# Fannovel16/stylish-tts

Hardware: AMD Instinct MI355X
Metric: utterances_per_sec (higher is better)
Workload: dtype f32

## Files before the change

### include/stylish_hip.h

```cpp
#ifndef STYLISH_HIP_H_
#define STYLISH_HIP_H_

#include <stddef.h>
#include <stdint.h>

#ifdef __cplusplus
extern "C" {
#endif

typedef struct stts_ctx stts_ctx;

typedef struct stts_model_dims {
  int32_t n_fft, win_length, hop_length, sample_rate;
  int32_t style_dim, inter_dim;
  int32_t dec_hidden, dec_residual;
  int32_t gen_input, gen_hidden, gen_inter, gen_io_kernel;
  int32_t tokens, te_hidden, te_filter, te_heads, te_layers, te_kernel;
  int32_t style_layers;
  int32_t dur_layers, dur_classes, dur_max;
  int32_t pe_inter;
} stts_model_dims;

const char* stts_last_error(void);
int stts_version(void);
// ... 113 lines not shown
int stts_rmvpe_finalize(stts_ctx* ctx, const stts_rmvpe_dims* dims);
size_t stts_rmvpe_workspace_bytes(const stts_ctx* ctx, int n_utt, const int32_t* off_host);
int stts_rmvpe_forward(stts_ctx* ctx, void* stream, int n_utt, const int32_t* off_host, const int32_t* off_dev, const float* mel_rows, int ld_mel, float thred,
                       float* hidden_out, float* f0_out, void* ws, size_t ws_bytes);
int stts_rmvpe_forward_taps(stts_ctx* ctx, void* stream, int n_utt, const int32_t* off_host, const int32_t* off_dev, const float* mel_rows, int ld_mel,
                            float thred, float* hidden_out, float* f0_out, float* taps, void* ws, size_t ws_bytes);
int64_t stts_rmvpe_tap_floats(const stts_rmvpe_dims* dims, int n_utt, const int32_t* off_host);
int stts_rmvpe_mel(stts_ctx* ctx, void* stream, int n_utt, const int32_t* sample_off_host, const int32_t* sample_off_dev, const int32_t* mel_off_host,
                   const int32_t* mel_off_dev, const float* wave, const float* mel_basis, const int32_t* band, float* mel_out, int ld_mel, float* mel_lin);
int stts_rmvpe_decode(stts_ctx* ctx, void* stream, int64_t n_rows, const float* salience, int ld, float thred, float* f0_out);
int stts_rmvpe_resample(stts_ctx* ctx, void* stream, int n_utt, const int32_t* off_in_dev, const int32_t* off_out_host, const int32_t* off_out_dev,
                        const float* f0_in, float* f0_out);

typedef struct stts_aligner_dims {
  int32_t n_mels, hidden, classes;
  int32_t n_tdnn, ffn_layers;
  int32_t tdnn_kernel[4];
} stts_aligner_dims;
int stts_aligner_finalize(stts_ctx* ctx, const stts_aligner_dims* dims);
size_t stts_aligner_workspace_bytes(const stts_ctx* ctx, int n_utt, const int32_t* off_host);
int stts_aligner_forward(stts_ctx* ctx, void* stream, int n_utt, const int32_t* off_host, const int32_t* off_dev, const float* mel_rows, int ld_mel,
                         float* log_probs, int ld_out, void* ws, size_t ws_bytes);
int stts_aligner_forward_taps(stts_ctx* ctx, void* stream, int n_utt, const int32_t* off_host, const int32_t* off_dev, const float* mel_rows, int ld_mel,
                              float* log_probs, int ld_out, float* taps, void* ws, size_t ws_bytes);
int64_t stts_aligner_tap_floats(const stts_aligner_dims* dims, int n_utt, const int32_t* off_host);
size_t stts_ctc_align_workspace_bytes(int n_utt, const int32_t* t_off_host, const int32_t* p_off_host);
int stts_ctc_align(void* stream, int n_utt, const int32_t* t_off_host, const int32_t* t_off_dev, const int32_t* p_off_host, const int32_t* p_off_dev,
                   const float* log_probs, int ld, int classes, int blank, const int32_t* targets, int path_given, int32_t* path, float* scores,
                   int32_t* durations, float* left, float* right, void* ws, size_t ws_bytes);

size_t stts_hubert_workspace_bytes(const stts_ctx* ctx, int64_t rows_T, int n_utt, int max_len);
int stts_speaker_style(stts_ctx* ctx, void* stream, int n_utt, const float* spk_emb, int ld, float* style_out, float* pe_style_out, void* ws,
                       size_t ws_bytes);
int stts_hubert_encoder_forward(stts_ctx* ctx, void* stream, int n_utt, const int32_t* off_T_host, const int32_t* off_T_dev, const float* feats,
                                int ld_feats, float* asr_out, int ld_asr, void* ws, size_t ws_bytes);
int stts_hubert_pitch_energy_forward(stts_ctx* ctx, void* stream, int n_utt, const int32_t* off_T_host, const int32_t* off_T_dev, const float* feats,
                                     int ld_feats, const float* pe_style, float* f0_out, float* energy_out, float* prosody_tap, void* ws,
                                     size_t ws_bytes);

size_t stts_mel_style_workspace_bytes(stts_ctx* ctx, int which, int64_t rows_T, int n_utt);
int stts_mel_style_forward(stts_ctx* ctx, void* stream, int which, int n_utt, const int32_t* seg_off_host, const int32_t* seg_off_dev, const float* mel,
                           int ld, float* style_out, void* ws, size_t ws_bytes);
int stts_mel_style_forward_taps(stts_ctx* ctx, void* stream, int which, int n_utt, const int32_t* seg_off_host, const int32_t* seg_off_dev,
                                const float* mel, int ld, float* style_out, float* block_taps, void* ws, size_t ws_bytes);

size_t stts_cfm_pitch_workspace_bytes(stts_ctx* ctx, int64_t rows_T, int n_utt);
int stts_cfm_pitch_forward(stts_ctx* ctx, void* stream, int n_utt, const int32_t* off_T_host, const int32_t* off_T_dev, const float* asr, int ld_asr,
                           const float* spk_style, float* out_normed, float* out_hz, float f0_log2_mean, float f0_log2_std, const float* uv, void* ws,
                           size_t ws_bytes);
int stts_cfm_pitch_forward_taps(stts_ctx* ctx, void* stream, int n_utt, const int32_t* off_T_host, const int32_t* off_T_dev, const float* asr, int ld_asr,
                                const float* spk_style, float* out_normed, float* out_hz, float f0_log2_mean, float f0_log2_std, const float* uv,
                                float* taps, void* ws, size_t ws_bytes);

int stts_log_mel_forward(stts_ctx* ctx, void* stream, int n_utt, const int32_t* sample_off_host, const int32_t* sample_off_dev,
                         const int32_t* row_off_host, const int32_t* row_off_dev, const float* wave, int n_fft, int win_length, int hop_length, int n_mels,
                         int sample_rate, double mean, double std, float* mel_rows, int ld, float* energy, float* raw_rows);
int stts_log_mel_stats(stts_ctx* ctx, void* stream, int n_utt, const int32_t* sample_off_host, const int32_t* sample_off_dev,
                       const int32_t* row_off_host, const int32_t* row_off_dev, const float* wave, int n_fft, int win_length, int hop_length, int n_mels,
                       int sample_rate, double* partials, double* stats);
int stts_log_mel_filters(int n_fft, int n_mels, int sample_rate, int32_t* band, float* weights);

int stts_to_time_major(void* stream, const float* x_bct, int B, int C, int T, float* y, int ldy);
int stts_to_channel_major(void* stream, const float* x, int ldx, int B, int C, int T, float* y_bct);

int stts_conv_stft_transform(stts_ctx* ctx, void* stream, int n_utt, const int32_t* frame_off_host, const int32_t* frame_off_dev,
                             const float* wave, int hop, float* mag, float* x, float* y, int ld);
int stts_conv_stft_inverse(stts_ctx* ctx, void* stream, int n_utt, const int32_t* frame_off_host, const int32_t* frame_off_dev,
                           const float* mag, const float* x, const float* y, int ld, int hop, float* wave_out, void* ws, size_t ws_bytes);

int stts_profile_begin(void);
int stts_profile_end(void* stream, int* launches, double* total_ms, double* total_flops);
int stts_profile_report(void* stream, char* json, size_t json_capacity);

int stts_op_mrf_block(stts_ctx* ctx, void* stream, const char* prefix, int n_utt, const int32_t* seg_off_host,
                      const int32_t* seg_off_dev, const float* x, int ldx, int channels, int kernel, const float* style, float* y,
                      int ldy, void* ws, size_t ws_bytes);

#ifdef STTS_TEST_OPS
int stts_op_conv1d(void* stream, int n_utt, const int32_t* seg_off_host, const int32_t* seg_off_dev, const float* x, int ldx, int cin,
                   const float* w_host, const float* bias_host, int cout, int k, int dil, int act, float* y, int ldy, int force_tile, int precision);
int stts_op_conv1d_x3(void* stream, int n_utt, const int32_t* seg_off_host, const int32_t* seg_off_dev, const float* x, int ldx, int cin,
                      const float* x2, int ldx2, int cin2, const float* w_host, const float* bias_host, int cout, int k, int dil, const float* aff_host,
                      int xaff_mode, float slope, int presplit, float* y, int ldy, int force_tile, int precision);
int stts_op_adain_block(stts_ctx* ctx, void* stream, const char* prefix, int n_utt, const int32_t* seg_off_host,
                        const int32_t* seg_off_dev, const float* x, int ldx, int cin, int cout, const float* style, float* y, int ldy,
                        void* ws, size_t ws_bytes);
int stts_op_attention(void* stream, int n_utt, const int32_t* q_off_host, const int32_t* q_off_dev, const int32_t* k_off_host,
                      const int32_t* k_off_dev, const float* q, const float* k, const float* v, float* o, int heads, int kc,
                      const int32_t* band_centre, int window, int kernel);
int stts_op_stft_geom(void* stream, int n_utt, const int32_t* seg_off_host, const int32_t* seg_off_dev, int n_fft, int win, int h, const float* sig,
                      float* spec, float* phase, int ld, int generic);
int stts_op_istft_geom(void* stream, int n_utt, const int32_t* seg_off_host, const int32_t* seg_off_dev, int n_fft, int win, int h, const float* logamp,
                       const float* phase, int ld, float* audio, int generic);
int stts_bench_gemm(void* stream, int n_utt, int rows_per_utt, int cin, int cout, int k, int tile, int iters, double* avg_ms, int tune);
#endif

#ifdef __cplusplus
}
#endif
#endif
```

### stylish_tts_amd/_lib.py

```python
from __future__ import annotations

import ctypes as C
import os

_HERE = os.path.dirname(os.path.abspath(__file__))
LIB_PATH = os.path.abspath(os.environ["STTS_LIB"]) if os.environ.get("STTS_LIB") else os.path.join(_HERE, "libstylish_hip.so")


class ModelDims(C.Structure):
    _fields_ = [(n, C.c_int32) for n in (
        "n_fft", "win_length", "hop_length", "sample_rate",
        "style_dim", "inter_dim",
        "dec_hidden", "dec_residual",
        "gen_input", "gen_hidden", "gen_inter", "gen_io_kernel",
        "tokens", "te_hidden", "te_filter", "te_heads", "te_layers", "te_kernel",
        "style_layers",
        "dur_layers", "dur_classes", "dur_max",
        "pe_inter",
    )]


class CfmDims(C.Structure):
    _fields_ = [(n, C.c_int32) for n in ("feat_dim", "asr_dim", "spk_dim", "hidden_dim", "emb_dim", "depth", "enc_blocks", "dec_blocks",
                                         "prev_depth", "post_depth", "head_dim")]
# ... 15 lines not shown

_P = C.c_void_p
_I = C.c_int
_SZ = C.c_size_t
_I64 = C.c_int64

SIGNATURES = {
    "stts_last_error": (C.c_char_p, []),
    "stts_version": (_I, []),
    "stts_ctx_create": (_I, [C.POINTER(ModelDims), _I, C.POINTER(_P)]),
    "stts_ctx_destroy": (None, [_P]),
    "stts_load_weight": (_I, [_P, C.c_char_p, _P, C.POINTER(_I64), _I]),
    "stts_finalize_weights": (_I, [_P, _I]),
    "stts_check_status": (_I, [_P, _P]),
    "stts_frame_workspace_bytes": (_SZ, [_P, _I64, _I, _I]),
    "stts_har_ld": (_I, [_P]),
    "stts_decoder_forward": (_I, [_P, _P, _I, _P, _P, _P, _I, _P, _P, _P, _P, _I, _P, _SZ]),
    "stts_prior_flow_forward": (_I, [_P, _P, _I, _P, _P, _P, _I, _P, _P, _P, _I, _P, _P, _P, _SZ]),
    "stts_harmonic_stft": (_I, [_P, _P, _I, _P, _P, _P, _P, _P, _I, _P, _P, _P, _I, _P, _SZ]),
    "stts_vocoder_forward": (_I, [_P, _P, _I, _P, _P, _P, _I, _P, _P, _P, _I, _P, _P, _P, _I, _P, _SZ]),
    "stts_frame_path": (_I, [_P, _P, _I, _P, _P, _P, _I, _P, _P, _P, _P, _P, _P, _I, _P, _P, _SZ, _I]),
    "stts_frame_offsets": (_I, [_P, _P, _I, _P, _P, _P, _P, _P, _P]),
    "stts_phoneme_workspace_bytes": (_SZ, [_P, _I64, _I64, _I]),
    "stts_text_encoder_forward": (_I, [_P, _P, _I, _I, _P, _P, _P, _P, _I, _P, _P, _SZ]),
    "stts_text_style_forward": (_I, [_P, _P, _I, _I, _P, _P, _P, _I, _P, _P, _SZ]),
    "stts_duration_forward": (_I, [_P, _P, _I, _P, _P, _P, _P, _P, _P, _P, _P, _P, _SZ]),
    "stts_pitch_energy_forward": (_I, [_P, _P, _I, _P, _P, _P, _P, _P, _P, _I, _P, _P, _P, _P, _P, _P, _SZ, _I]),
    "stts_duration_decode": (_I, [_P, _P, _I, _I, _P]),
    "stts_duration_to_alignment": (_I, [_P, _P, _I, _I, _P]),
    "stts_length_regulate": (_I, [_P, _P, _I, _P, _P, _P, _I64, _I, _P, _I, _I, _P, _I, _P]),
    "stts_set_precision": (_I, [_P, _I]),
    "stts_upsample4": (_I, [_P, _P, _I, _P, _P, _P, _P, _P]),
    "stts_euler_step": (_I, [_P, _P, _P, C.c_float, C.c_int64]),
    "stts_hubert_workspace_bytes": (_SZ, [_P, C.c_int64, _I, _I]),
    "stts_speaker_style": (_I, [_P, _P, _I, _P, _I, _P, _P, _P, _SZ]),
    "stts_hubert_encoder_forward": (_I, [_P, _P, _I, _P, _P, _P, _I, _P, _I, _P, _SZ]),
    "stts_hubert_pitch_energy_forward": (_I, [_P, _P, _I, _P, _P, _P, _I, _P, _P, _P, _P, _P, _SZ]),
    "stts_mel_style_workspace_bytes": (_SZ, [_P, _I, _I64, _I]),
    "stts_mel_style_forward": (_I, [_P, _P, _I, _I, _P, _P, _P, _I, _P, _P, _SZ]),
    "stts_mel_style_forward_taps": (_I, [_P, _P, _I, _I, _P, _P, _P, _I, _P, _P, _P, _SZ]),
    "stts_cfm_pitch_workspace_bytes": (_SZ, [_P, _I64, _I]),
    "stts_cfm_pitch_forward": (_I, [_P, _P, _I, _P, _P, _P, _I, _P, _P, _P, C.c_float, C.c_float, _P, _P, _SZ]),
    "stts_cfm_pitch_forward_taps": (_I, [_P, _P, _I, _P, _P, _P, _I, _P, _P, _P, C.c_float, C.c_float, _P, _P, _P, _SZ]),
    "stts_ssl_finalize": (_I, [_P, _P]),
    "stts_ssl_frames": (_I64, [_P, _I64]),
    "stts_ssl_workspace_bytes": (_SZ, [_P, _I, _P]),
    "stts_ssl_forward": (_I, [_P, _P, _I, _P, _P, _P, _P, _P, _P, _I, _P, _SZ]),
    "stts_ssl_forward_taps": (_I, [_P, _P, _I, _P, _P, _P, _P, _P, _P, _I, _P, _P, _P, _P, _P, _P, _P, _P, _SZ]),
    "stts_ssl_tap_rows": (_I64, [_P, _I, _P]),
    "stts_rmvpe_finalize": (_I, [_P, _P]),
    "stts_rmvpe_workspace_bytes": (_SZ, [_P, _I, _P]),
    "stts_rmvpe_forward": (_I, [_P, _P, _I, _P, _P, _P, _I, C.c_float, _P, _P, _P, _SZ]),
    "stts_rmvpe_forward_taps": (_I, [_P, _P, _I, _P, _P, _P, _I, C.c_float, _P, _P, _P, _P, _SZ]),
    "stts_rmvpe_tap_floats": (_I64, [_P, _I, _P]),
    "stts_rmvpe_mel": (_I, [_P, _P, _I, _P, _P, _P, _P, _P, _P, _P, _P, _I, _P]),
    "stts_rmvpe_decode": (_I, [_P, _P, _I64, _P, _I, C.c_float, _P]),
    "stts_rmvpe_resample": (_I, [_P, _P, _I, _P, _P, _P, _P, _P]),
    "stts_aligner_finalize": (_I, [_P, _P]),
    "stts_aligner_workspace_bytes": (_SZ, [_P, _I, _P]),
    "stts_aligner_forward": (_I, [_P, _P, _I, _P, _P, _P, _I, _P, _I, _P, _SZ]),
    "stts_aligner_forward_taps": (_I, [_P, _P, _I, _P, _P, _P, _I, _P, _I, _P, _P, _SZ]),
    "stts_aligner_tap_floats": (_I64, [_P, _I, _P]),
    "stts_ctc_align_workspace_bytes": (_SZ, [_I, _P, _P]),
    "stts_ctc_align": (_I, [_P, _I, _P, _P, _P, _P, _P, _I, _I, _I, _P, _I, _P, _P, _P, _P, _P, _P, _SZ]),
    "stts_log_mel_forward": (_I, [_P, _P, _I, _P, _P, _P, _P, _P, _I, _I, _I, _I, _I, C.c_double, C.c_double, _P, _I, _P, _P]),
    "stts_log_mel_stats": (_I, [_P, _P, _I, _P, _P, _P, _P, _P, _I, _I, _I, _I, _I, _P, _P]),
    "stts_log_mel_filters": (_I, [_I, _I, _I, _P, _P]),
    "stts_cfm_finalize": (_I, [_P, _P]),
    "stts_cfm_workspace_bytes": (_SZ, [_P, _I64, _I]),
    "stts_cfm_estimator": (_I, [_P, _P, _I, _P, _P, _P, _I, _P, _I, _P, _P, _P, _P, _P, _P, _P, _P, _I, _P, _SZ]),
    "stts_to_time_major": (_I, [_P, _P, _I, _I, _I, _P, _I]),
    "stts_to_channel_major": (_I, [_P, _P, _I, _I, _I, _I, _P]),
    "stts_conv_stft_transform": (_I, [_P, _P, _I, _P, _P, _P, _I, _P, _P, _P, _I]),
    "stts_conv_stft_inverse": (_I, [_P, _P, _I, _P, _P, _P, _P, _P, _I, _I, _P, _P, _SZ]),
    "stts_profile_begin": (_I, []),
    "stts_profile_end": (_I, [_P, C.POINTER(_I), C.POINTER(C.c_double), C.POINTER(C.c_double)]),
    "stts_profile_report": (_I, [_P, C.c_char_p, _SZ]),
    "stts_op_mrf_block": (_I, [_P, _P, C.c_char_p, _I, _P, _P, _P, _I, _I, _I, _P, _P, _I, _P, _SZ]),
}
TEST_SIGNATURES = {
    "stts_bench_gemm": (_I, [_P, _I, _I, _I, _I, _I, _I, _I, C.POINTER(C.c_double), _I]),
    "stts_op_conv1d": (_I, [_P, _I, _P, _P, _P, _I, _I, _P, _P, _I, _I, _I, _I, _P, _I, _I, _I]),
    "stts_op_conv1d_x3": (_I, [_P, _I, _P, _P, _P, _I, _I, _P, _I, _I, _P, _P, _I, _I, _I, _P, _I, C.c_float, _I, _P, _I, _I, _I]),
    "stts_op_adain_block": (_I, [_P, _P, C.c_char_p, _I, _P, _P, _P, _I, _I, _I, _P, _P, _I, _P, _SZ]),
    "stts_op_attention": (_I, [_P, _I, _P, _P, _P, _P, _P, _P, _P, _P, _I, _I, _P, _I, _I]),
    "stts_op_stft_geom": (_I, [_P, _I, _P, _P, _I, _I, _I, _P, _P, _P, _I, _I]),
    "stts_op_istft_geom": (_I, [_P, _I, _P, _P, _I, _I, _I, _P, _P, _I, _P, _I]),
}

_lib = None


def load() -> C.CDLL:
    global _lib
    if _lib is not None:
        return _lib
    if not os.path.exists(LIB_PATH):
        raise RuntimeError(
            f"{LIB_PATH} not found: build it with `python -c 'import __graft_entry__ as g; g.build()'` "
            "(hipcc --offload-arch=gfx950).  There is no CPU fallback."
        )
    try:
        import torch
    except ImportError:
        pass
    lib = C.CDLL(LIB_PATH)
    for name, (res, args) in SIGNATURES.items():
        fn = getattr(lib, name)
        fn.restype = res
        fn.argtypes = args
    for name, (res, args) in TEST_SIGNATURES.items():
        fn = getattr(lib, name, None)
        if fn is not None:
            fn.restype = res
            fn.argtypes = args
    _lib = lib
    return lib


def check(rc: int) -> None:
    if rc != 0:
        raise RuntimeError("stylish_hip: " + (load().stts_last_error() or b"?").decode("utf-8", "replace"))
```

### stylish_tts_amd/csrc/api.hip

```cpp
#include "model.hip.h"
#include "cfm.hip.h"
#include "hubert.hip.h"
#include "conv2d.hip.h"
#include "mel_style.hip.h"
#include "cfm_pitch.hip.h"
#include "ssl.hip.h"
#include "rmvpe.hip.h"
#include "aligner.hip.h"
#include "log_mel.hip.h"

using namespace stts;

#define API_BEGIN try {
#define API_END                                                         \
  }                                                                     \
  catch (const std::exception& e) { return stts::fail("exception: %s", e.what()); } \
  catch (...) { return stts::fail("unknown exception"); }

extern "C" {

const char* stts_last_error(void) { return stts::last_error().c_str(); }
int stts_version(void) { return 1; }

int stts_ctx_create(const stts_model_dims* dims, int device, stts_ctx** out) {
  API_BEGIN
  STTS_CHECK(dims && out, "null argument");
  int n = 0;
  STTS_HIP(hipGetDeviceCount(&n));
  STTS_CHECK(device >= 0 && device < n, "device %d not available (%d visible)", device, n);
  STTS_HIP(hipSetDevice(device));
  hipDeviceProp_t prop;
  STTS_HIP(hipGetDeviceProperties(&prop, device));
  STTS_CHECK(strncmp(prop.gcnArchName, "gfx950", 6) == 0, "device %d is %s; this library is built for gfx950 only", device, prop.gcnArchName);
  stts_ctx* c = new stts_ctx();
  c->d = *dims;
  c->device = device;
  c->force_generic_signal = getenv("STTS_SIGNAL_GENERIC") && atoi(getenv("STTS_SIGNAL_GENERIC")) != 0;
  PackScope scope(c, engine_mode(c));
  STTS_TRY(dev_upload(c, std::vector<int>(64, 0), &c->d_err));
  *out = c;
  return 0;
  API_END
}

void stts_ctx_destroy(stts_ctx* c) {
  if (!c) return;
  for (void* p : c->allocs) (void)hipFree(p);
  for (auto& kv : c->side_lanes) {
    if (kv.second.fork) (void)hipEventDestroy(kv.second.fork);
    if (kv.second.join) (void)hipEventDestroy(kv.second.join);
    if (kv.second.stream) (void)hipStreamDestroy(kv.second.stream);
    if (kv.second.fork2) (void)hipEventDestroy(kv.second.fork2);
    if (kv.second.join2) (void)hipEventDestroy(kv.second.join2);
    if (kv.second.stream2) (void)hipStreamDestroy(kv.second.stream2);
  }
  delete c;
}

int stts_set_precision(stts_ctx* c, int precision) {
  API_BEGIN
  STTS_CHECK(c, "bad argument");
  STTS_CHECK(precision >= 0 && precision <= 3, "precision must be STTS_PREC_F32, _BF16, _F16 or _F32_NATIVE");
  const int prec = precision == STTS_PREC_F32_NATIVE ? (int)PREC_F32 : precision;
  STTS_CHECK(c->ready == 0 || (prec == c->prec && (precision != STTS_PREC_F32_NATIVE) == c->allow_x3), "precision must be chosen before weights are finalized");
  c->prec = prec;
  c->allow_x3 = precision != STTS_PREC_F32_NATIVE;
  return 0;
  API_END
}

int stts_load_weight(stts_ctx* c, const char* name, const float* data, const int64_t* shape, int ndim) {
  API_BEGIN
  STTS_CHECK(c && name && data && shape && ndim >= 1 && ndim <= 4, "bad argument");
  HostTensor t;
  int64_t n = 1;
  for (int i = 0; i < ndim; ++i) {
    t.shape.push_back(shape[i]);
    n *= shape[i];
  }
  t.data.assign(data, data + n);
  c->host[name] = std::move(t);
  return 0;
  API_END
}

int stts_finalize_weights(stts_ctx* c, int which) {
  API_BEGIN
  STTS_CHECK(c, "null ctx");
  STTS_HIP(hipSetDevice(c->device));
  c->ready &= ~which;
  free_component_allocs(c, which);
  if (which & (STTS_W_DECODER | STTS_W_FLOW | STTS_W_GENERATOR)) {
    PackScope scope(c, {c->prec, true, c->prec != PREC_F32 ? 64 : 32, 0});
    STTS_TRY(finalize_frame(c, which));
  }
  const int ph = which & (STTS_W_SPEECH_TEXT | STTS_W_DURATION | STTS_W_PE_TEXT | STTS_W_PE_STYLE | STTS_W_PITCH_ENERGY);
  if (ph) {
    if (!c->phoneme) c->phoneme = std::make_shared<PhonemeModel>();
    static const bool phoneme_x3 = getenv("STTS_PHONEME_X3") && atoi(getenv("STTS_PHONEME_X3")) != 0;
    PackScope scope(c, {PREC_F32, phoneme_x3, 32, 0});
    STTS_TRY(finalize_phoneme(c, static_cast<PhonemeModel*>(c->phoneme.get()), ph));
    c->ready |= ph;
  }
  const int hb = which & (STTS_W_HUBERT | STTS_W_HUBERT_PE);
  if (hb) {
    if (!c->hubert) c->hubert = std::make_shared<HubertModel>();
    PackScope scope(c, {PREC_F32, false, 32, 0});
    STTS_TRY(finalize_hubert(c, static_cast<HubertModel*>(c->hubert.get()), hb));
    c->ready |= hb;
  }
  const int ms = which & (STTS_W_PE_MEL_STYLE | STTS_W_CFM_PITCH);
  if (ms) {
    if (!c->mel_style) c->mel_style = std::make_shared<MelStyleModel>();
    PackScope scope(c, engine_mode(c));
    STTS_TRY(finalize_mel_style(c, static_cast<MelStyleModel*>(c->mel_style.get()), ms));
    c->ready |= ms;
  }
  if (which & STTS_W_CFM_PITCH_NET) {
    if (!c->cfm_pitch) c->cfm_pitch = std::make_shared<CfmPitchNetW>();
    PackScope scope(c, {PREC_F32, false, 32, STTS_W_CFM_PITCH_NET});
    STTS_TRY(finalize_cfm_pitch_net(c, static_cast<CfmPitchNetW*>(c->cfm_pitch.get())));
    c->ready |= STTS_W_CFM_PITCH_NET;
  }
  STTS_HIP(hipDeviceSynchronize());
  return 0;
  API_END
}

int stts_check_status(stts_ctx* c, void* stream) {
  API_BEGIN
  int e = 0;
  STTS_HIP(hipStreamSynchronize((hipStream_t)stream));
  STTS_HIP(hipMemcpy(&e, c->d_err, sizeof(int), hipMemcpyDeviceToHost));
  if (e) {
    STTS_HIP(hipMemset(c->d_err, 0, sizeof(int)));
    std::string msg;
    if (e & 2) msg += "text encoder: token id outside [0, tokens); ";
    if (e & 4) msg += "harmonic source: an utterance is too short for the STFT's reflect padding (needs more than " + std::to_string(c->d.n_fft / 2) + " samples); ";
    if (e & 1) msg += "harmonic source: a frame is voiced (f0 > 10 Hz) but no f0 exceeds 20 Hz (reference raises: models/generator.py:285); ";
    if (e & ~7) msg += "unknown device error bits " + std::to_string(e & ~7) + "; ";
    msg.resize(msg.size() - 2);
    return stts::fail("%s", msg.c_str());
  }
  return 0;
  API_END
}

int stts_har_ld(const stts_ctx* c) {
  if (!c) return 0;
  if (c->amp_prior.kc) return har_ld(c);
  return round_up(c->d.n_fft / 2 + 1, c->prec != PREC_F32 ? 64 : 32);
}

size_t stts_frame_workspace_bytes(const stts_ctx* c, int64_t rows, int n_utt, int max_len) { return frame_workspace_bytes(c, rows, n_utt, max_len); }

static int seg_ok(int n_utt, const int32_t* h, const int32_t* d, const char* bad = "bad utterance offsets", const char* empty = "utterance %d is empty") {
  STTS_CHECK(n_utt > 0 && h && d && h[0] == 0, "%s", bad);
  for (int u = 0; u < n_utt; ++u) STTS_CHECK(h[u + 1] > h[u], empty, u, h[u + 1] - h[u]);
  return 0;
}

#define READY_CHECK(have, mask)                                                      \
  STTS_CHECK(c && (have) && (c->ready & (mask)) == (mask), "weights for this stage are not finalized (need components 0x%x, have 0x%x)", (mask), c ? c->ready : 0); \
  STTS_HIP(hipSetDevice(c->device));                                                 \
  hipStream_t st = (hipStream_t)stream

#define SEG_CHECK(mask)                                                              \
  READY_CHECK(true, mask);                                                           \
  STTS_TRY(seg_ok(n_utt, seg_off_host, seg_off_dev));                                \
  Seg s{n_utt, seg_off_host, seg_off_dev}

int stts_decoder_forward(stts_ctx* c, void* stream, int n_utt, const int32_t* seg_off_host, const int32_t* seg_off_dev, const float* asr,
                         int ld_asr, const float* pitch, const float* energy, const float* style, float* x_out, int ld_x, void* ws,
                         size_t ws_bytes) {
  API_BEGIN
  SEG_CHECK(STTS_W_DECODER);
  STTS_CHECK(ld_asr >= c->d.inter_dim && ld_asr % 4 == 0 && ld_x >= c->d.dec_hidden, "bad leading dimension");
// ... 912 lines not shown
```

### stylish_tts_amd/csrc/gemm.hip.h

```cpp
#pragma once
#include <type_traits>
#include <mutex>
#include <map>
#include <hip/hip_ext.h>
#include <cmath>
#include <algorithm>
#include <vector>

#include "common.h"

namespace stts {

using f32x16 = __attribute__((ext_vector_type(16))) float;
using f32x4 = __attribute__((ext_vector_type(4))) float;

enum Act { ACT_NONE = 0, ACT_SILU = 1, ACT_GELU = 2, ACT_RELU = 3, ACT_LRELU = 4 };
enum Epi {
  EPI_STORE = 0,
  EPI_GATE = 1,
  EPI_SPLIT_ACC = 2,
  EPI_COUPLE = 3,
  EPI_PRIOR = 4,
};

struct GemmSeg {
  const float* X;
  const float* W;
  const unsigned short* W16;
  long w16_plane;
  long x_plane;
  long w_utt_stride;
  int ldx, xcol0, kc, ntaps, dil, pad;
  int kreal;
};

struct SplitInfo {
  const float* partial;
  int ksplit, slice_rows, ld_part;
};

struct GemmArgs {
  GemmSeg seg[3];
  int nseg;
  const int* seg_off;
  const int* seg_host;
  int n_utt;
  int compact;
  int uniform_len, uniform_lo0;
  int tile0, tiles_y;
  int gemm16_gx;
  int capacity;
  int rows_total, wrows;
  int tune;
  int prec;
  const float* xaff;
  int ld_xaff;
  float xaff_slope;
  bool xaff_scale_only;
  long long* dbg;
  const float* zeros;
  int ksplit;
  float* partial;
  int ld_part;
  SplitInfo* defer;
  int N;
  const float* bias;
  int x16;
  float* Y;
  int ldy, ycol0;
  unsigned short* Y16;
  int ldy16, ycol16;
  const float* R;
  int ldr, rcol0;
  float alpha;
  int act;
  float* sumsq_part;
  int ld_ss, ss_stride;
  float* stat_part;
  int ld_stat, stat_nchunk;
  const float* gate;
  int ld_gate, gcol0, gC;
  float* D0;
  float* D1;
  int ldd0, ldd1, nsplit, acc0, acc1;
  float* Z;
  int ldz, zcol0;
  const float* noise;
  int ldnoise;
};

__device__ __forceinline__ float act_apply(float v, int act) {
  switch (act) {
    case ACT_SILU: return v * __builtin_amdgcn_rcpf(1.0f + __expf(-v));
    case ACT_GELU: return 0.5f * v * (1.0f + erff(v * 0.70710678118654752f));
    case ACT_RELU: return fmaxf(v, 0.0f);
    case ACT_LRELU: return v >= 0.0f ? v : 0.2f * v;
    default: return v;
  }
}

enum { PREC_F32 = 0, PREC_BF16 = 1, PREC_F16 = 2, PREC_X3 = 3 };
typedef __bf16 bf16x8 __attribute__((ext_vector_type(8)));
typedef _Float16 f16x8 __attribute__((ext_vector_type(8)));
typedef unsigned u32x2 __attribute__((ext_vector_type(2)));

template <int PREC>
__device__ __forceinline__ u32x2 pack4_16(const f32x4 v) {
  u32x2 r;
  if constexpr (PREC == PREC_BF16) {
    typedef __bf16 b2 __attribute__((ext_vector_type(2)));
    typedef float f2 __attribute__((ext_vector_type(2)));
    const f2 lo = {v.x, v.y}, hi = {v.z, v.w};
    r.x = __builtin_bit_cast(unsigned, __builtin_convertvector(lo, b2));
    r.y = __builtin_bit_cast(unsigned, __builtin_convertvector(hi, b2));
  } else {
    typedef _Float16 h2 __attribute__((ext_vector_type(2)));
    typedef float f2 __attribute__((ext_vector_type(2)));
    const f2 lo = {v.x, v.y}, hi = {v.z, v.w};
    r.x = __builtin_bit_cast(unsigned, __builtin_convertvector(lo, h2));
    r.y = __builtin_bit_cast(unsigned, __builtin_convertvector(hi, h2));
  }
  return r;
}
__device__ __forceinline__ void split3_bf16(const f32x4 v, u32x2& p0, u32x2& p1, u32x2& p2) {
  typedef __bf16 b2 __attribute__((ext_vector_type(2)));
  typedef float f2 __attribute__((ext_vector_type(2)));
  auto pk = [](float a, float b) { const f2 t = {a, b}; return __builtin_bit_cast(unsigned, __builtin_convertvector(t, b2)); };
  auto lo = [](unsigned u) { return __uint_as_float(u << 16); };
  auto hi = [](unsigned u) { return __uint_as_float(u & 0xffff0000u); };
  const float tmax = __uint_as_float(0x7f7f7fffu);
  bool inf[4];
  float f[4];
#pragma unroll
  for (int e = 0; e < 4; ++e) {
    inf[e] = __builtin_isinf(v[e]);
    f[e] = __builtin_amdgcn_fmed3f(inf[e] ? 0.0f : v[e], -tmax, tmax);
  }
  p0.x = pk(f[0], f[1]); p0.y = pk(f[2], f[3]);
  const float r0 = v.x - lo(p0.x), r1 = v.y - hi(p0.x), r2 = v.z - lo(p0.y), r3 = v.w - hi(p0.y);
  p1.x = pk(inf[0] ? 0.0f : r0, inf[1] ? 0.0f : r1); p1.y = pk(inf[2] ? 0.0f : r2, inf[3] ? 0.0f : r3);
  p2.x = pk(r0 - lo(p1.x), r1 - hi(p1.x)); p2.y = pk(r2 - lo(p1.y), r3 - hi(p1.y));
}
template <int PREC>
__device__ __forceinline__ f32x16 mfma16(const f32x4 a, const f32x4 b, const f32x16 c) {
  if constexpr (PREC == PREC_BF16 || PREC == PREC_X3) return __builtin_amdgcn_mfma_f32_32x32x16_bf16(__builtin_bit_cast(bf16x8, a), __builtin_bit_cast(bf16x8, b), c, 0, 0, 0);
  else return __builtin_amdgcn_mfma_f32_32x32x16_f16(__builtin_bit_cast(f16x8, a), __builtin_bit_cast(f16x8, b), c, 0, 0, 0);
}

template <int BM, int BN, int WARPS_M, int WARPS_N, int EPI, int KSPLIT = 1, bool GLDS = false, int PREC = PREC_F32, int XAFF = 0, bool MSEG = true,
          bool X16 = false>
__global__ void __launch_bounds__(WARPS_M* WARPS_N * 64 * KSPLIT) conv_gemm_f32(const GemmArgs a) {
  static_assert(!(XAFF && GLDS), "the input affine lives on the register staging path");
  static_assert(!X16 || (PREC != PREC_F32 && !XAFF && EPI == EPI_STORE), "16-bit activation rows: 16-bit operand modes, store epilogue");
  constexpr int NT = WARPS_M * WARPS_N * 64 * KSPLIT;
  constexpr bool B16 = PREC != PREC_F32;
  constexpr bool X3 = PREC == PREC_X3;
  constexpr int NPL = X3 ? 3 : 1;
  static_assert(!X3 || !GLDS || X16, "split fp32: fp32 activation rows are split on the register staging path; LDS-DMA needs pre-split planes");
  static_assert(!(B16 && GLDS) || X16, "LDS-DMA staging of 16-bit operands needs 16-bit activation rows (nothing converts on the way)");
  static_assert(KSPLIT == 1 || KSPLIT == 2, "KSPLIT");
  constexpr int WR = BN / WARPS_N, WC = BM / WARPS_M;
  constexpr int TR = WR / 32, TC = WC / 32;
  constexpr int XL = X16 ? (BN * 4 * NPL + NT - 1) / NT : BN * 8 / NT;
  constexpr int WL = B16 ? (BM * 4 * NPL + NT - 1) / NT : BM * 8 / NT;
  static_assert(WR % 32 == 0 && WC % 32 == 0, "wave tile must be a multiple of 32x32");
  static_assert((X16 || (BN * 8) % NT == 0) && (B16 || (BM * 8) % NT == 0), "tile loads must divide over the block");
  static_assert(EPI == EPI_STORE || EPI == EPI_SPLIT_ACC || TC % 2 == 0, "paired epilogues need an even TC");
  constexpr int NSTAGE = (B16 && GLDS) ? (X3 ? 3 : ((BM + BN) <= 256 ? 8 : 3)) : 2;
  constexpr int SLOTS = X3 ? 12 : ((B16 && KSPLIT == 1) ? 4 : 8);
  constexpr int PLANE = (BN + BM) * 4;
  constexpr int STG16 = PLANE * NPL;
  __shared__ f32x4 lds[NSTAGE * (BN + BM) * SLOTS];

  int bx = blockIdx.x, by = blockIdx.y, bz = blockIdx.z;
  {
    unsigned gy = gridDim.y;
    if (a.capacity) {
      const int lane_ = threadIdx.x & 63;
      int tot = 0;
      for (int u0 = 0; u0 < a.n_utt; u0 += 64) {
        const int u = u0 + lane_;
        tot += u < a.n_utt ? (a.seg_off[u + 1] - a.seg_off[u] + BN - 1) / BN : 0;
      }
#pragma unroll
      for (int o = 32; o > 0; o >>= 1) tot += __shfl_xor(tot, o, 64);
      gy = (unsigned)__builtin_amdgcn_readfirstlane(tot);
      if ((unsigned)by >= gy) return;
    }
    const unsigned gx = gridDim.x, nwg = gx * gy * gridDim.z;
    const unsigned orig = bx + gx * (by + gy * bz);
    const unsigned q = nwg >> 3, r = nwg & 7, xcd = orig & 7;
    const unsigned id = (xcd < r ? xcd * (q + 1) : r * (q + 1) + (xcd - r) * q) + (orig >> 3);
    bx = id % gx;
    by = (id / gx) % gy;
    bz = id / (gx * gy);
  }
  const int ksplit = a.ksplit > 1 ? a.ksplit : 1;
  int utt, ks;
  if (a.compact) {
    ks = bz;
    const int t = by + a.tile0, lane_ = threadIdx.x & 63;
    utt = a.n_utt - 1;
    int base = 0, local = 0;
    bool done = false;
    if (a.uniform_len > 0) {
      const int tpu = (a.uniform_len + BN - 1) / BN;
      utt = t / tpu;
      local = t - utt * tpu;
      done = utt < a.n_utt;
    }
    for (int u0 = 0; u0 < a.n_utt && !done && a.uniform_len <= 0; u0 += 64) {
      const int u = u0 + lane_;
      const int tiles = u < a.n_utt ? (a.seg_off[u + 1] - a.seg_off[u] + BN - 1) / BN : 0;
      int incl = tiles;
#pragma unroll
      for (int d = 1; d < 64; d <<= 1) {
        const int v = __shfl_up(incl, d, 64);
        if (lane_ >= d) incl += v;
      }
      const int excl = incl - tiles;
      const unsigned long long hit = __ballot(t >= base + excl && t < base + incl);
      if (hit) {
        const int src = __ffsll((long long)hit) - 1;
        utt = u0 + src;
        local = t - base - __shfl(excl, src, 64);
        done = true;
      }
      base += __shfl(incl, 63, 64);
    }
    if (!done) return;
    utt = __builtin_amdgcn_readfirstlane(utt);
    by = __builtin_amdgcn_readfirstlane(local);
  } else {
    utt = bz / ksplit;
    ks = bz % ksplit;
  }
  const int lo = a.uniform_len > 0 ? a.uniform_lo0 + utt * a.uniform_len : a.seg_off[utt];
  const int hi = a.uniform_len > 0 ? lo + a.uniform_len : a.seg_off[utt + 1];
  const int row0 = lo + by * BN;
  if (row0 >= hi) return;
  const int m0 = bx * BM;
  const int tid = threadIdx.x, lane = tid & 63;
#ifdef STTS_GEMM_TRACE
  const unsigned dbg_blk = blockIdx.x + gridDim.x * (blockIdx.y + gridDim.y * blockIdx.z);
  auto stamp = [&](int i) { if (a.dbg && tid == 0) a.dbg[8 * (long)dbg_blk + i] = wall_clock64(); };
  const long long dbg_c0 = clock64();
  if (a.dbg && tid == 0) { a.dbg[8 * (long)dbg_blk + 5] = __builtin_amdgcn_s_getreg(0xF804); a.dbg[8 * (long)dbg_blk + 6] = __builtin_amdgcn_s_getreg(0xF814); }
  auto stamp_end = [&]() { stamp(3); if (a.dbg && tid == 0) a.dbg[8 * (long)dbg_blk + 7] = clock64() - dbg_c0; };
  auto ablate = [&](int bit) { return (a.tune & bit) != 0; };
#else
  auto stamp = [&](int) {};
  auto stamp_end = [&]() {};
  auto ablate = [](int) { return false; };
#endif
  stamp(0);
  const int kg = (tid >> 6) / (WARPS_M * WARPS_N), wid = (tid >> 6) % (WARPS_M * WARPS_N);
  const int wn = wid / WARPS_M, wm = wid % WARPS_M;
  (void)kg;

  f32x16 acc[TR][TC];
#pragma unroll
  for (int i = 0; i < TR; ++i)
#pragma unroll
    for (int j = 0; j < TC; ++j)
#pragma unroll
      for (int r = 0; r < 16; ++r) acc[i][j][r] = 0.0f;

  int s = 0, tap = 0, chunk = 0;
  auto xbase = [&](const GemmSeg& g) {
    return X16 ? reinterpret_cast<const float*>(reinterpret_cast<const unsigned short*>(g.X) + g.xcol0) : g.X + g.xcol0;
  };
  const float* gX = xbase(a.seg[0]);
  const float* gW = a.seg[0].W + (long)utt * a.seg[0].w_utt_stride + (long)m0 * a.seg[0].ntaps * a.seg[0].kc;
  const unsigned short* gW16 = B16 ? a.seg[0].W16 + (long)utt * a.seg[0].w_utt_stride + (long)m0 * a.seg[0].ntaps * a.seg[0].kc : nullptr;
  int g_ldx = a.seg[0].ldx, g_kc = a.seg[0].kc, g_ntaps = a.seg[0].ntaps, g_dil = a.seg[0].dil, g_pad = a.seg[0].pad;
  const int nseg = a.nseg;

  struct RegSet {
    f32x4 x[XL], w[WL];
    bool ok[XL];
    f32x4 sc, sh;
    bool aff;
  };
  RegSet rsA, rsB;
#ifdef STTS_X3_DEEP
  constexpr bool DEEP = X3 && KSPLIT == 1 && BN <= 128;
#else
  constexpr bool DEEP = false;
#endif
  RegSet rsC, rsD;
  unsigned woff[WL];
  const int len = hi - lo, rel0 = row0 - lo;
  long g_wplane = X3 ? a.seg[0].w16_plane : 0, g_xplane = (X3 && X16) ? a.seg[0].x_plane : 0;
  auto seg_offsets = [&]() {
    const int wrow = g_ntaps * g_kc;
#pragma unroll
    for (int i = 0; i < WL; ++i) {
      const int idx = tid + i * NT;
      if constexpr (X3) {
        const int pl = min(idx / (BM * 4), 2), rem = idx % (BM * 4);
        woff[i] = (unsigned)(((long)pl * g_wplane + (rem >> 2) * wrow + (rem & 3) * 8) * 2);
      } else if constexpr (B16) woff[i] = (unsigned)((min(idx >> 2, BM - 1) * wrow + (idx & 3) * 8) * 2);
      else woff[i] = (unsigned)(((idx >> 3) * wrow + (idx & 7) * 4) * 4);
    }
  };
  seg_offsets();
  auto gload = [&](RegSet& rs) {
    const int shift = (tap - g_pad) * g_dil;
#ifdef STTS_GEMM_TRACE
    const bool hot = a.tune & 16;
#else
    constexpr bool hot = false;
#endif
    const char* xb = X16 ? reinterpret_cast<const char*>(reinterpret_cast<const unsigned short*>(gX) + (long)lo * g_ldx + chunk * 32)
                         : reinterpret_cast<const char*>(gX + (long)lo * g_ldx + (hot ? 0 : chunk * 32));
    const char* wb = B16 ? reinterpret_cast<const char*>(gW16 + tap * g_kc + chunk * 32)
                         : reinterpret_cast<const char*>((hot ? a.seg[0].W : gW) + (hot ? 0 : tap * g_kc + chunk * 32));
#pragma unroll
    for (int i = 0; i < XL; ++i) {
      const int idx = tid + i * NT;
      const int pl = (X16 && X3) ? min(idx / (BN * 4), 2) : 0, idp = (X16 && X3) ? idx % (BN * 4) : idx;
      const int r = X16 ? idp >> 2 : idx >> 3, sl = X16 ? idp & 3 : idx & 7;
      const int rel = (hot ? 0 : rel0) + r + shift;
      const int crel = min(max(rel, 0), len - 1);
      const unsigned rowoff = __umul24((unsigned)crel, (unsigned)g_ldx);
      const unsigned off = X16 ? (rowoff + sl * 8) * 2 : (rowoff + sl * 4) * 4;
      if constexpr (X16 && X3) rs.x[i] = *reinterpret_cast<const f32x4*>(xb + (long)pl * g_xplane * 2 + off);
      else
      rs.x[i] = *reinterpret_cast<const f32x4*>(xb + off);
      rs.ok[i] = rel >= 0 && rel < len;
    }
#pragma unroll
    for (int i = 0; i < WL; ++i) rs.w[i] = *reinterpret_cast<const f32x4*>(wb + woff[i]);
    if constexpr (XAFF) {
      rs.aff = s == 0;
      const float* ap = a.xaff + (long)utt * 2 * a.ld_xaff + (rs.aff ? chunk * 32 + (tid & 7) * 4 : 0);
      rs.sc = *reinterpret_cast<const f32x4*>(ap);
      if constexpr (XAFF == 1) rs.sh = *reinterpret_cast<const f32x4*>(ap + a.ld_xaff);
    }
    const int w1 = tap + 1 >= g_ntaps, wk = (chunk + 1) * 32 >= g_kc;
    const bool wrapt1 = w1 != 0;
    const bool wrapt = (w1 & wk) != 0;
    const bool last = ((w1 & wk) & (MSEG ? (int)(s + 1 >= nseg) : 1)) != 0;
    tap = last ? tap : (wrapt1 ? 0 : tap + 1);
    chunk = last ? chunk : (wrapt ? 0 : chunk + w1);
    if constexpr (MSEG) {
      if (wrapt && !last) {
        ++s;
        const GemmSeg& n = s == 1 ? a.seg[1] : a.seg[2];
        gX = xbase(n);
        gW = n.W + (long)utt * n.w_utt_stride + (long)m0 * n.ntaps * n.kc;
        if constexpr (B16) gW16 = n.W16 + (long)utt * n.w_utt_stride + (long)m0 * n.ntaps * n.kc;
        g_ldx = n.ldx; g_kc = n.kc; g_ntaps = n.ntaps; g_dil = n.dil; g_pad = n.pad;
        if constexpr (X3) { g_wplane = n.w16_plane; g_xplane = n.x_plane; }
        seg_offsets();
      }
    }
  };
  auto xin = [&](const RegSet& rs, int i) {
    const f32x4 z = {0.f, 0.f, 0.f, 0.f};
    f32x4 v = rs.x[i];
    if constexpr (XAFF == 2) {
      static_assert(XAFF != 2 || !MSEG, "the scale-only input affine is instantiated for single-segment launches");
      v = v * rs.sc;
    } else if constexpr (XAFF == 1) {
      f32x4 t;
#pragma unroll
      for (int q = 0; q < 4; ++q) {
        const float y = (rs.sc[q] == 0.0f ? 0.0f : v[q] * rs.sc[q]) + rs.sh[q];
        t[q] = y >= 0.0f ? y : a.xaff_slope * y;
      }
      v = rs.aff ? t : v;
    }
    return rs.ok[i] ? v : z;
// ... 87 lines not shown
    const int slot = 2 * kk + lh;
    f32x4 xa[TR], wb[TC];
#pragma unroll
    for (int i = 0; i < TR; ++i) {
      const int r = wn * WR + i * 32 + l31;
      xa[i] = Xs[r * 8 + (slot ^ ((r >> 1) & 7))];
    }
#pragma unroll
    for (int j = 0; j < TC; ++j) {
      const int c = wm * WC + j * 32 + l31;
      wb[j] = Ws[c * 8 + (slot ^ ((c >> 1) & 7))];
    }
#pragma unroll
    for (int i = 0; i < TR; ++i)
#pragma unroll
      for (int j = 0; j < TC; ++j) {
        acc[i][j] = __builtin_amdgcn_mfma_f32_32x32x2f32(xa[i].x, wb[j].x, acc[i][j], 0, 0, 0);
        acc[i][j] = __builtin_amdgcn_mfma_f32_32x32x2f32(xa[i].y, wb[j].y, acc[i][j], 0, 0, 0);
        acc[i][j] = __builtin_amdgcn_mfma_f32_32x32x2f32(xa[i].z, wb[j].z, acc[i][j], 0, 0, 0);
        acc[i][j] = __builtin_amdgcn_mfma_f32_32x32x2f32(xa[i].w, wb[j].w, acc[i][j], 0, 0, 0);
      }
  };

  auto mma_step16 = [&](int b, int kk) {
    const f32x4* Xs = lds + b * STG16;
    const f32x4* Ws = Xs + BN * 4;
    const int slot = 2 * kk + lh;
    if constexpr (X3) {
      f32x4 xa[TR][3], wb[TC][3];
      const bool nord = ablate(32);
#pragma unroll
      for (int i = 0; i < TR; ++i) {
        const int r = wn * WR + i * 32 + l31;
        const int o = r * 4 + (slot ^ ((r >> 2) & 3));
#pragma unroll
        for (int p = 0; p < 3; ++p) {
          if (!nord) xa[i][p] = Xs[o + p * PLANE];
          else xa[i][p] = f32x4{(float)r, (float)kk, (float)p, 0.f};
        }
      }
#pragma unroll
      for (int j = 0; j < TC; ++j) {
        const int c = wm * WC + j * 32 + l31;
        const int o = c * 4 + (slot ^ ((c >> 2) & 3));
#pragma unroll
        for (int p = 0; p < 3; ++p) {
          if (!nord) wb[j][p] = Ws[o + p * PLANE];
          else wb[j][p] = f32x4{(float)c, (float)kk, (float)p, 0.f};
        }
      }
      if (ablate(1)) return;
#pragma unroll
      for (int i = 0; i < TR; ++i)
#pragma unroll
        for (int j = 0; j < TC; ++j) {
          acc[i][j] = mfma16<PREC>(xa[i][2], wb[j][0], acc[i][j]);
          acc[i][j] = mfma16<PREC>(xa[i][0], wb[j][2], acc[i][j]);
          acc[i][j] = mfma16<PREC>(xa[i][1], wb[j][1], acc[i][j]);
          acc[i][j] = mfma16<PREC>(xa[i][1], wb[j][0], acc[i][j]);
          acc[i][j] = mfma16<PREC>(xa[i][0], wb[j][1], acc[i][j]);
          acc[i][j] = mfma16<PREC>(xa[i][0], wb[j][0], acc[i][j]);
        }
      return;
    }
    f32x4 xa[TR], wb[TC];
    const bool nord = ablate(32);
#pragma unroll
    for (int i = 0; i < TR; ++i) {
      const int r = wn * WR + i * 32 + l31;
      if (!nord) xa[i] = Xs[r * 4 + (slot ^ ((r >> 2) & 3))];
      else xa[i] = f32x4{(float)r, (float)kk, 0.f, 0.f};
    }
#pragma unroll
    for (int j = 0; j < TC; ++j) {
      const int c = wm * WC + j * 32 + l31;
      if (!nord) wb[j] = Ws[c * 4 + (slot ^ ((c >> 2) & 3))];
      else wb[j] = f32x4{(float)c, (float)kk, 0.f, 0.f};
    }
#pragma unroll
    for (int i = 0; i < TR; ++i)
#pragma unroll
      for (int j = 0; j < TC; ++j) acc[i][j] = mfma16<PREC>(xa[i], wb[j], acc[i][j]);
  };

  if constexpr (GLDS) {
    static_assert(KSPLIT == 1, "GLDS path is single K-group");
    if constexpr (B16) {
      constexpr int NW = NT / 64, NI1 = (BN + BM) / 16, NI = NI1 * NPL, PER = NI / NW;
      static_assert((NI % NW == 0 || X3) && BN % 16 == 0, "tile rows must divide over the waves");
      constexpr int PERC = (NI + NW - 1) / NW;
      const int wv = tid >> 6;
      auto issue = [&](int b) {
        const int shift = (tap - g_pad) * g_dil;
        const char* xb = reinterpret_cast<const char*>(reinterpret_cast<const unsigned short*>(gX) + (long)lo * g_ldx + chunk * 32);
        const char* wb = reinterpret_cast<const char*>(gW16 + tap * g_kc + chunk * 32);
        const int wrow = g_ntaps * g_kc;
#pragma unroll
        for (int q = 0; q < PERC; ++q) {
          const int instq = min(wv + q * NW, NI - 1);
          const int pl = instq / NI1, inst = instq % NI1;
          const int trow = inst * 16 + (lane >> 2);
          const char* src;
          if (inst < BN / 16) {
            const int r = trow;
            const int sslot = (lane & 3) ^ ((r >> 2) & 3);
            const int rel = rel0 + r + shift;
            const bool ok = rel >= 0 && rel < len;
            src = ok ? xb + (long)pl * g_xplane * 2 + (unsigned)((rel * g_ldx + sslot * 8) * 2) : reinterpret_cast<const char*>(a.zeros);
          } else {
            const int n = trow - BN;
            const int sslot = (lane & 3) ^ ((n >> 2) & 3);
            src = wb + (long)pl * g_wplane * 2 + (unsigned)((n * wrow + sslot * 8) * 2);
          }
          __builtin_amdgcn_global_load_lds((const __attribute__((address_space(1))) void*)src,
                                           (__attribute__((address_space(3))) void*)(lds + b * STG16 + pl * PLANE + inst * 64), 16, 0, 0);
        }
        const int w1 = tap + 1 >= g_ntaps, wk = (chunk + 1) * 32 >= g_kc;
        const bool wrapt1 = w1 != 0;
        const bool wrapt = (w1 & wk) != 0;
        const bool last = ((w1 & wk) & (MSEG ? (int)(s + 1 >= nseg) : 1)) != 0;
        tap = last ? tap : (wrapt1 ? 0 : tap + 1);
        chunk = last ? chunk : (wrapt ? 0 : chunk + w1);
        if constexpr (MSEG) {
          if (wrapt && !last) {
            ++s;
            const GemmSeg& n = s == 1 ? a.seg[1] : a.seg[2];
            gX = xbase(n);
            gW16 = n.W16 + (long)utt * n.w_utt_stride + (long)m0 * n.ntaps * n.kc;
            g_ldx = n.ldx; g_kc = n.kc; g_ntaps = n.ntaps; g_dil = n.dil; g_pad = n.pad;
            if constexpr (X3) { g_wplane = n.w16_plane; g_xplane = n.x_plane; }
          }
        }
      };
      (void)PER;
      constexpr int INFLIGHT = (NSTAGE - 2) * PERC;
      static_assert(INFLIGHT >= 1 && INFLIGHT <= 63, "vmcnt immediate");
      auto wait_next_tile = [&]() {
        asm volatile("" ::: "memory");
        __builtin_amdgcn_s_waitcnt((INFLIGHT & 15) | (7 << 4) | (15 << 8) | ((INFLIGHT >> 4) << 14));
        asm volatile("" ::: "memory");
      };
#pragma unroll
      for (int q = 0; q < NSTAGE - 1; ++q) issue(q);
      wait_next_tile();
      __syncthreads();
      stamp(1);
      int cur = 0, nxt = NSTAGE - 1;
      for (int it = 0; it < total; ++it) {
        if (!ablate(8)) issue(nxt);
        mma_step16(cur, 0);
        mma_step16(cur, 1);
        wait_next_tile();
        if (!ablate(2)) __syncthreads();
        cur = cur == NSTAGE - 1 ? 0 : cur + 1;
        nxt = nxt == NSTAGE - 1 ? 0 : nxt + 1;
      }
      asm volatile("s_waitcnt vmcnt(0)" ::: "memory");
      __syncthreads();
      stamp(2);
    } else {
        static_assert(KSPLIT == 1, "GLDS path is single K-group");
      constexpr int NW = NT / 64, NI = (BN + BM) / 8;
      static_assert(NI % NW == 0, "tile rows must divide over the waves");
      const int wv = tid >> 6;
      auto issue = [&](int b) {
        const int shift = (tap - g_pad) * g_dil;
        const char* xb = reinterpret_cast<const char*>(gX + (long)lo * g_ldx + chunk * 32);
        const char* wb = reinterpret_cast<const char*>(gW + tap * g_kc + chunk * 32);
        const int wrow = g_ntaps * g_kc;
  #pragma unroll
        for (int q = 0; q < NI / NW; ++q) {
          const int inst = wv + q * NW;
          const int trow = inst * 8 + (lane >> 3);
          const char* src;
          if (inst < BN / 8) {
            const int r = trow;
            const int sslot = (lane & 7) ^ ((r >> 1) & 7);
            const int rel = rel0 + r + shift;
            const bool ok = rel >= 0 && rel < len;
            src = ok ? xb + (unsigned)((rel * g_ldx + sslot * 4) * 4) : reinterpret_cast<const char*>(a.zeros);
          } else {
            const int n = trow - BN;
            const int sslot = (lane & 7) ^ ((n >> 1) & 7);
            src = wb + (unsigned)((n * wrow + sslot * 4) * 4);
          }
          __builtin_amdgcn_global_load_lds((const __attribute__((address_space(1))) void*)src,
                                           (__attribute__((address_space(3))) void*)(lds + b * (BN + BM) * 8 + inst * 64), 16, 0, 0);
        }
        const int w1 = tap + 1 >= g_ntaps, wk = (chunk + 1) * 32 >= g_kc;
        const bool wrapt1 = w1 != 0;
        const bool wrapt = (w1 & wk) != 0;
        const bool last = ((w1 & wk) & (int)(s + 1 >= nseg)) != 0;
        tap = last ? tap : (wrapt1 ? 0 : tap + 1);
        chunk = last ? chunk : (wrapt ? 0 : chunk + w1);
        if (wrapt && !last) {
          ++s;
          const GemmSeg& n = s == 1 ? a.seg[1] : a.seg[2];
          gX = xbase(n);
          gW = n.W + (long)utt * n.w_utt_stride + (long)m0 * n.ntaps * n.kc;
          if constexpr (B16) gW16 = n.W16 + (long)utt * n.w_utt_stride + (long)m0 * n.ntaps * n.kc;
          g_ldx = n.ldx; g_kc = n.kc; g_ntaps = n.ntaps; g_dil = n.dil; g_pad = n.pad;
        }
      };
      issue(0);
      asm volatile("s_waitcnt vmcnt(0)" ::: "memory");
      __syncthreads();
      for (int it = 0; it < total; ++it) {
        issue((it + 1) & 1);
        const f32x4* Xs = lds + (it & 1) * (BN + BM) * 8;
        const f32x4* Ws = Xs + BN * 8;
        mma_step(Xs, Ws, 0);
        mma_step(Xs, Ws, 1);
        mma_step(Xs, Ws, 2);
        mma_step(Xs, Ws, 3);
        asm volatile("s_waitcnt vmcnt(0)" ::: "memory");
        __syncthreads();
      }
    }
  } else {
  gload(rsA);
  lstore(rsA, 0);
  gload(rsB);
  if constexpr (DEEP) {
    gload(rsC);
    gload(rsD);
  }
  gload(rsA);
  __syncthreads();
  stamp(1);

  int return_guard = 0;
  (void)return_guard;
  constexpr bool FPIPE = X3 && KSPLIT == 1 && BN == 128 && BM == 128 && WARPS_M * WARPS_N == 8 && !GLDS;
  struct Frag {
    f32x4 xa[TR][3], wb[TC][3];
  };
  Frag fA, fB;
  auto frag_read = [&](int b, int kk, Frag& f) {
    const f32x4* Xs = lds + b * STG16;
    const f32x4* Ws = Xs + BN * 4;
    const int slot = 2 * kk + lh;
    const bool nord = ablate(32);
#pragma unroll
    for (int i = 0; i < TR; ++i) {
      const int r = wn * WR + i * 32 + l31;
      const int o = r * 4 + (slot ^ ((r >> 2) & 3));
#pragma unroll
      for (int p = 0; p < 3; ++p) {
        if (!nord) f.xa[i][p] = Xs[o + p * PLANE];
        else f.xa[i][p] = f32x4{(float)r, (float)kk, (float)p, 0.f};
      }
    }
#pragma unroll
    for (int j = 0; j < TC; ++j) {
      const int c = wm * WC + j * 32 + l31;
      const int o = c * 4 + (slot ^ ((c >> 2) & 3));
#pragma unroll
      for (int p = 0; p < 3; ++p) {
        if (!nord) f.wb[j][p] = Ws[o + p * PLANE];
        else f.wb[j][p] = f32x4{(float)c, (float)kk, (float)p, 0.f};
      }
    }
  };
  auto frag_mma = [&](const Frag& f) {
    if (ablate(1)) return;
#pragma unroll
    for (int i = 0; i < TR; ++i)
#pragma unroll
      for (int j = 0; j < TC; ++j) {
        acc[i][j] = mfma16<PREC>(f.xa[i][2], f.wb[j][0], acc[i][j]);
        acc[i][j] = mfma16<PREC>(f.xa[i][0], f.wb[j][2], acc[i][j]);
        acc[i][j] = mfma16<PREC>(f.xa[i][1], f.wb[j][1], acc[i][j]);
        acc[i][j] = mfma16<PREC>(f.xa[i][1], f.wb[j][0], acc[i][j]);
        acc[i][j] = mfma16<PREC>(f.xa[i][0], f.wb[j][1], acc[i][j]);
        acc[i][j] = mfma16<PREC>(f.xa[i][0], f.wb[j][0], acc[i][j]);
      }
  };
  if constexpr (FPIPE) frag_read(0, 0, fA);
  auto iter = [&](int it, RegSet& nset) {
    const f32x4* Xs = lds + (it & 1) * (BN + BM) * 8;
    const f32x4* Ws = Xs + BN * 8;
    if constexpr (FPIPE) {
      frag_read(it & 1, 1, fB);
      frag_mma(fA);
      if (!ablate(4)) lstore(nset, (it + 1) & 1);
      if (!ablate(8)) gload(nset);
#ifndef STTS_X3_NO_SGB
#pragma unroll
      for (int g = 0; g < 6 * TR * TC; ++g) {
        __builtin_amdgcn_sched_group_barrier(0x008, 1, 0);
        __builtin_amdgcn_sched_group_barrier(0x002, 7, 0);
      }
#endif
      if (!ablate(2)) __syncthreads();
      frag_read((it + 1) & 1, 0, fA);
      frag_mma(fB);
      return;
    }
    if constexpr (B16) {
      if constexpr (KSPLIT == 1) {
        mma_step16(it & 1, 0);
// ... 29 lines not shown
      mma_step(Xs, Ws, 2 * kg + 1);
    }
    if (!ablate(2)) __syncthreads();
  };
  if constexpr (DEEP) {
    int it = 0;
    for (; it + 3 < total; it += 4) {
      iter(it, rsB);
      iter(it + 1, rsC);
      iter(it + 2, rsD);
      iter(it + 3, rsA);
    }
    if (it < total) iter(it, rsB);
    if (it + 1 < total) iter(it + 1, rsC);
    if (it + 2 < total) iter(it + 2, rsD);
  } else {
    int it = 0;
    for (; it + 1 < total; it += 2) {
      iter(it, rsB);
      iter(it + 1, rsA);
    }
    if (it < total) iter(it, rsB);
  }
  stamp(2);
#ifdef STTS_GEMM_TRACE
  if (a.dbg && tid == 0) a.dbg[8 * (long)dbg_blk + 4] = total;
#endif
  }

  if constexpr (KSPLIT == 2) {
    static_assert(WARPS_M * WARPS_N * TR * TC * 16 * 64 * 4 <= NSTAGE * (BN + BM) * SLOTS * 16, "reduction buffer must fit in the staging LDS");
    float* red = reinterpret_cast<float*>(lds);
    if (kg == 1) {
#pragma unroll
      for (int i = 0; i < TR; ++i)
#pragma unroll
        for (int j = 0; j < TC; ++j)
#pragma unroll
          for (int r = 0; r < 16; ++r) red[(((wid * TR + i) * TC + j) * 16 + r) * 64 + lane] = acc[i][j][r];
    }
    __syncthreads();
    if (kg == 1) return;
#pragma unroll
    for (int i = 0; i < TR; ++i)
#pragma unroll
      for (int j = 0; j < TC; ++j)
#pragma unroll
        for (int r = 0; r < 16; ++r) acc[i][j][r] += red[(((wid * TR + i) * TC + j) * 16 + r) * 64 + lane];
  }
  const int nvalid = hi - row0;
  if constexpr (EPI == EPI_STORE) {
    if (ksplit > 1) {
      float* P = a.partial + (long)ks * a.rows_total * a.ld_part;
#pragma unroll
      for (int j = 0; j < TC; ++j) {
        const int n = m0 + wm * WC + j * 32 + l31;
#pragma unroll
        for (int i = 0; i < TR; ++i)
#pragma unroll
          for (int r = 0; r < 16; ++r) {
            const int rl = wn * WR + i * 32 + (r & 3) + 8 * (r >> 2) + 4 * lh;
            if (rl < nvalid) P[(long)(row0 + rl) * a.ld_part + n] = acc[i][j][r];
          }
      }
      stamp_end();
      return;
    }
    const bool hasR = a.R != nullptr, hasY = a.Y != nullptr, hasSS = a.sumsq_part != nullptr;
    bool hasY16 = false;
    if constexpr (B16) hasY16 = a.Y16 != nullptr;
    const int act = a.act;
    const float alpha = a.alpha;
    float* const Yb = hasY ? a.Y + (long)row0 * a.ldy + a.ycol0 + m0 : nullptr;
    const float* const Rb = hasR ? a.R + (long)row0 * a.ldr + a.rcol0 + m0 : nullptr;
    unsigned short* const Y16b = hasY16 ? a.Y16 + (long)row0 * a.ldy16 + a.ycol16 + m0 : nullptr;
    const int rlane = wn * WR + 4 * lh, clane = wm * WC + l31;
    unsigned oy = (unsigned)(rlane * a.ldy + clane), orr = (unsigned)(rlane * a.ldr + clane), o16 = (unsigned)(rlane * a.ldy16 + clane);
    const unsigned sy1 = (unsigned)a.ldy, sy5 = 5u * sy1, sr1 = (unsigned)a.ldr, sr5 = 5u * sr1, s161 = (unsigned)a.ldy16, s165 = 5u * s161;
    float bv[TC];
    bool nok[TC];
#pragma unroll
    for (int j = 0; j < TC; ++j) {
      const int n = m0 + clane + j * 32;
      bv[j] = a.bias ? a.bias[n] : 0.0f;
      nok[j] = n < a.N;
    }
#pragma unroll
    for (int i = 0; i < TR; ++i) {
      float ss[TC];
#pragma unroll
      for (int j = 0; j < TC; ++j) ss[j] = 0.0f;
#pragma unroll
      for (int r = 0; r < 16; ++r) {
        const int dr = i * 32 + (r & 3) + 8 * (r >> 2);
        const bool rok = rlane + dr < nvalid;
#pragma unroll
        for (int j = 0; j < TC; ++j) {
          float v = act_apply(acc[i][j][r] + bv[j], act);
          if (rok && nok[j]) {
            if (hasR) v += Rb[orr + j * 32];
            v *= alpha;
            if (hasY) Yb[oy + j * 32] = v;
            if constexpr (B16) {
              if (hasY16) {
                if constexpr (PREC == PREC_BF16) reinterpret_cast<__bf16*>(Y16b)[o16 + j * 32] = (__bf16)v;
                else reinterpret_cast<_Float16*>(Y16b)[o16 + j * 32] = (_Float16)v;
              }
            }
            ss[j] += v * v;
          }
        }
        const bool big = (r & 3) == 3;
        oy += big ? sy5 : sy1;
        orr += big ? sr5 : sr1;
        o16 += big ? s165 : s161;
      }
      if (hasSS) {
#pragma unroll
        for (int j = 0; j < TC; ++j) {
          float t2 = ss[j] + __shfl_xor(ss[j], 32, 64);
          const int sub = by * (BN / 32) + (wn * TR + i);
          if (lh == 0 && nok[j] && sub * 32 < hi - lo) {
            const long t = (long)utt * a.ss_stride + sub;
            a.sumsq_part[t * a.ld_ss + m0 + clane + j * 32] = t2;
          }
        }
      }
      __builtin_amdgcn_sched_barrier(0);
    }
  } else if constexpr (EPI == EPI_SPLIT_ACC) {
#pragma unroll
    for (int j = 0; j < TC; ++j) {
      const int n = m0 + wm * WC + j * 32 + l31;
      const float bv = a.bias ? a.bias[n] : 0.0f;
      if (n < a.N) {
        float* D;
        int ld, col, accum;
        if (n < a.nsplit) {
          D = a.D0; ld = a.ldd0; col = n; accum = a.acc0;
        } else {
          D = a.D1; ld = a.ldd1; col = n - a.nsplit; accum = a.acc1;
        }
#pragma unroll
        for (int i = 0; i < TR; ++i)
#pragma unroll
          for (int r = 0; r < 16; ++r) {
            const int rl = wn * WR + i * 32 + (r & 3) + 8 * (r >> 2) + 4 * lh;
            if (rl < nvalid) {
              float* p = D + (long)(row0 + rl) * ld + col;
              const float v = acc[i][j][r] + bv;
              *p = accum ? *p + v : v;
            }
          }
      }
    }
  } else {
#pragma unroll
    for (int jp = 0; jp < TC / 2; ++jp) {
      const int npk = m0 + wm * WC + jp * 64 + l31;
      const int c = (npk >> 6) * 32 + (npk & 31);
      const float ba = a.bias ? a.bias[npk] : 0.0f;
      const float bb = a.bias ? a.bias[npk + 32] : 0.0f;
      if (c < a.N) {
        float ga = 0.f, gb = 0.f;
        if constexpr (EPI == EPI_GATE) {
          ga = a.gate[(long)utt * a.ld_gate + a.gcol0 + c];
          gb = a.gate[(long)utt * a.ld_gate + a.gcol0 + a.gC + c];
// ... 120 lines not shown
}
inline double gemm_algorithmic_flops(const GemmArgs& a) {
  double k = 0;
  for (int i = 0; i < a.nseg; ++i) k += (double)a.seg[i].kreal * a.seg[i].ntaps;
  return 2.0 * (double)a.rows_total * (double)a.wrows * k;
}

#define STTS_LAUNCH_TIMED(kernel, grid, block, st, e0, e1, ...)                                   \
  do {                                                                                            \
    if (e0) hipExtLaunchKernelGGL(kernel, grid, block, 0, st, e0, e1, 0, __VA_ARGS__);            \
    else hipLaunchKernelGGL(kernel, grid, block, 0, st, __VA_ARGS__);                             \
  } while (0)

#define STTS_LAUNCH_PROF(name, bytes, kernel, grid, block, st, ...)                                \
  do {                                                                                            \
    stts::GemmProfiler& _p = stts::gemm_profiler();                                               \
    if (_p.on) {                                                                                  \
      hipEvent_t _e0 = _p.next(), _e1 = _p.next();                                                \
      _p.add(name, 1, 0.0, 0.0, (double)(bytes));                                                 \
      hipExtLaunchKernelGGL(kernel, grid, block, 0, st, _e0, _e1, 0, __VA_ARGS__);                \
    } else {                                                                                      \
      hipLaunchKernelGGL(kernel, grid, block, 0, st, __VA_ARGS__);                                \
    }                                                                                             \
  } while (0)

template <int ABL>
inline int launch_conv_gemm16(hipStream_t st, const GemmArgs& a, int npad, int n_utt);

void gemm_dispatch_f32(hipStream_t st, const GemmArgs& as, int tile, int epi, int npad, int n_utt, int max_rows, hipEvent_t e0, hipEvent_t e1);
void gemm_dispatch_bf16(hipStream_t st, const GemmArgs& as, int tile, int epi, int npad, int n_utt, int max_rows, hipEvent_t e0, hipEvent_t e1);
void gemm_dispatch_f16(hipStream_t st, const GemmArgs& as, int tile, int epi, int npad, int n_utt, int max_rows, hipEvent_t e0, hipEvent_t e1);
void gemm_dispatch_x3(hipStream_t st, const GemmArgs& as, int tile, int epi, int npad, int n_utt, int max_rows, hipEvent_t e0, hipEvent_t e1);
int launch_conv_gemm16_main(hipStream_t st, const GemmArgs& a, int npad, int n_utt);

}

#include "gemm_plan.hip.h"

namespace stts {

#ifndef STTS_GEMM_NO_LAUNCHER
template <int BM, int BN, int WM, int WN, int KS = 1, bool GL = false, int PR = PREC_F32>
inline void launch_cfg(hipStream_t st, const GemmArgs& a, int epi, int npad, int n_utt, int max_rows, hipEvent_t e0 = nullptr, hipEvent_t e1 = nullptr) {
  dim3 grid(npad / BM, ceil_div(max_rows, BN), n_utt * (a.ksplit > 1 ? a.ksplit : 1)), block(WM * WN * 64 * KS);
  if (a.compact) grid = dim3(npad / BM, a.tiles_y, a.ksplit > 1 ? a.ksplit : 1);
  if constexpr (GL && PR != PREC_F32) {
    if (a.nseg == 1) STTS_LAUNCH_TIMED((conv_gemm_f32<BM, BN, WM, WN, EPI_STORE, KS, true, PR, false, false, true>), grid, block, st, e0, e1, a);
    else STTS_LAUNCH_TIMED((conv_gemm_f32<BM, BN, WM, WN, EPI_STORE, KS, true, PR, false, true, true>), grid, block, st, e0, e1, a);
    return;
  } else
  switch (epi) {
    case EPI_STORE:
      if constexpr (!GL && PR != PREC_F32 && KS == 1) {
        if (a.x16) {
          if (a.nseg == 1) STTS_LAUNCH_TIMED((conv_gemm_f32<BM, BN, WM, WN, EPI_STORE, KS, GL, PR, false, false, true>), grid, block, st, e0, e1, a);
          else STTS_LAUNCH_TIMED((conv_gemm_f32<BM, BN, WM, WN, EPI_STORE, KS, GL, PR, false, true, true>), grid, block, st, e0, e1, a);
          break;
        }
      }
      if constexpr (!GL) {
        if (a.xaff) {
          if (a.nseg == 1) STTS_LAUNCH_TIMED((conv_gemm_f32<BM, BN, WM, WN, EPI_STORE, KS, GL, PR, 1, false>), grid, block, st, e0, e1, a);
          else STTS_LAUNCH_TIMED((conv_gemm_f32<BM, BN, WM, WN, EPI_STORE, KS, GL, PR, 1, true>), grid, block, st, e0, e1, a);
          break;
        }
        if (a.nseg == 1) {
          STTS_LAUNCH_TIMED((conv_gemm_f32<BM, BN, WM, WN, EPI_STORE, KS, GL, PR, false, false>), grid, block, st, e0, e1, a);
          break;
        }
      }
      STTS_LAUNCH_TIMED((conv_gemm_f32<BM, BN, WM, WN, EPI_STORE, KS, GL, PR>), grid, block, st, e0, e1, a);
      break;
    case EPI_SPLIT_ACC: STTS_LAUNCH_TIMED((conv_gemm_f32<BM, BN, WM, WN, EPI_SPLIT_ACC, KS, GL, PR>), grid, block, st, e0, e1, a); break;
    default:
      if constexpr (BM / WM >= 64) {
        if (epi == EPI_GATE) STTS_LAUNCH_TIMED((conv_gemm_f32<BM, BN, WM, WN, EPI_GATE, KS, GL, PR>), grid, block, st, e0, e1, a);
        else if (epi == EPI_COUPLE) STTS_LAUNCH_TIMED((conv_gemm_f32<BM, BN, WM, WN, EPI_COUPLE, KS, GL, PR>), grid, block, st, e0, e1, a);
        else STTS_LAUNCH_TIMED((conv_gemm_f32<BM, BN, WM, WN, EPI_PRIOR, KS, GL, PR>), grid, block, st, e0, e1, a);
      }
      break;
  }
}

template <int BM, int BN, int WM, int WN, int KS = 1, int X16MODE = 0>
inline void launch_cfg_x3(hipStream_t st, const GemmArgs& a, int epi, int npad, int n_utt, int max_rows, hipEvent_t e0 = nullptr, hipEvent_t e1 = nullptr) {
  dim3 grid(npad / BM, ceil_div(max_rows, BN), n_utt * (a.ksplit > 1 ? a.ksplit : 1)), block(WM * WN * 64 * KS);
  if (a.compact) grid = dim3(npad / BM, a.tiles_y, a.ksplit > 1 ? a.ksplit : 1);
  if constexpr (X16MODE != 0) {
    if (a.nseg == 1) STTS_LAUNCH_TIMED((conv_gemm_f32<BM, BN, WM, WN, EPI_STORE, KS, X16MODE == 2, PREC_X3, false, false, true>), grid, block, st, e0, e1, a);
    else STTS_LAUNCH_TIMED((conv_gemm_f32<BM, BN, WM, WN, EPI_STORE, KS, X16MODE == 2, PREC_X3, false, true, true>), grid, block, st, e0, e1, a);
    return;
  } else
  if (epi == EPI_PRIOR) {
    if constexpr (BM / WM >= 64) STTS_LAUNCH_TIMED((conv_gemm_f32<BM, BN, WM, WN, EPI_PRIOR, KS, false, PREC_X3>), grid, block, st, e0, e1, a);
  } else if (a.xaff) {
    if (a.nseg == 1 && a.xaff_scale_only) STTS_LAUNCH_TIMED((conv_gemm_f32<BM, BN, WM, WN, EPI_STORE, KS, false, PREC_X3, 2, false>), grid, block, st, e0, e1, a);
    else if (a.nseg == 1) STTS_LAUNCH_TIMED((conv_gemm_f32<BM, BN, WM, WN, EPI_STORE, KS, false, PREC_X3, 1, false>), grid, block, st, e0, e1, a);
    else STTS_LAUNCH_TIMED((conv_gemm_f32<BM, BN, WM, WN, EPI_STORE, KS, false, PREC_X3, 1, true>), grid, block, st, e0, e1, a);
  } else if (a.nseg == 1) {
    STTS_LAUNCH_TIMED((conv_gemm_f32<BM, BN, WM, WN, EPI_STORE, KS, false, PREC_X3, false, false>), grid, block, st, e0, e1, a);
  } else {
    STTS_LAUNCH_TIMED((conv_gemm_f32<BM, BN, WM, WN, EPI_STORE, KS, false, PREC_X3>), grid, block, st, e0, e1, a);
  }
}
template <int T, int PR>
inline void launch_tile(hipStream_t st, const GemmArgs& as, int epi, int npad, int n_utt, int max_rows, hipEvent_t e0, hipEvent_t e1) {
  constexpr TileRow r = tile_row(T);
  if constexpr ((r.forms & (PR == PREC_F32 ? FORM_F32 : FORM_16)) != 0) launch_cfg<r.BM, r.BN, r.WM, r.WN, r.KS, r.glds, PR>(st, as, epi, npad, n_utt, max_rows, e0, e1);
}
template <int T>
inline void launch_tile_x3(hipStream_t st, const GemmArgs& as, int epi, int npad, int n_utt, int max_rows, hipEvent_t e0, hipEvent_t e1) {
  constexpr TileRow r = tile_row(T);
  static_assert((r.forms & FORM_X3) != 0, "not a split-fp32 tile");
  launch_cfg_x3<r.BM, r.BN, r.WM, r.WN, r.KS, r.x16 != X16_MUST ? 0 : r.glds ? 2 : 1>(st, as, epi, npad, n_utt, max_rows, e0, e1);
}
#define STTS_TILE_CASE(T) case T: launch_tile<T, PR>(st, as, epi, npad, n_utt, max_rows, e0, e1); break;
template <int PR>
inline void gemm_dispatch_tile(hipStream_t st, const GemmArgs& as, int tile, int epi, int npad, int n_utt, int max_rows, hipEvent_t e0, hipEvent_t e1) {
  switch (tile) {
    STTS_TILE_CASE(2) STTS_TILE_CASE(4) STTS_TILE_CASE(5) STTS_TILE_CASE(6) STTS_TILE_CASE(8)
    STTS_TILE_CASE(14) STTS_TILE_CASE(15) STTS_TILE_CASE(16) STTS_TILE_CASE(17) STTS_TILE_CASE(18)
    STTS_TILE_CASE(11) STTS_TILE_CASE(13)
    default: launch_tile<3, PR>(st, as, epi, npad, n_utt, max_rows, e0, e1); break;
  }
}
#undef STTS_TILE_CASE
#define STTS_TILE_CASE(T) case T: launch_tile_x3<T>(st, as, epi, npad, n_utt, max_rows, e0, e1); break;
inline void gemm_dispatch_tile_x3(hipStream_t st, const GemmArgs& as, int tile, int epi, int npad, int n_utt, int max_rows, hipEvent_t e0, hipEvent_t e1) {
  switch (tile) {
    STTS_TILE_CASE(2) STTS_TILE_CASE(4) STTS_TILE_CASE(5) STTS_TILE_CASE(6) STTS_TILE_CASE(8)
    STTS_TILE_CASE(20) STTS_TILE_CASE(21) STTS_TILE_CASE(22)
    STTS_TILE_CASE(25) STTS_TILE_CASE(26) STTS_TILE_CASE(27) STTS_TILE_CASE(28)
    default: launch_tile_x3<3>(st, as, epi, npad, n_utt, max_rows, e0, e1); break;
  }
}
#undef STTS_TILE_CASE

inline int launch_conv_gemm(hipStream_t st, const GemmArgs& a, int epi, int npad, int n_utt, int max_rows, int force_tile = 0) {
  STTS_CHECK(npad % 128 == 0, "conv_gemm: padded cout %d not a multiple of 128", npad);
  for (int i = 0; i < a.nseg; ++i) {
    STTS_CHECK(a.seg[i].kc % 32 == 0 && a.seg[i].ldx % 4 == 0 && a.seg[i].xcol0 % 4 == 0, "conv_gemm: segment %d misaligned (kc %d ldx %d xcol0 %d)", i,
               a.seg[i].kc, a.seg[i].ldx, a.seg[i].xcol0);
  }
  if (a.x16 && a.prec != PREC_F32)
    for (int i = 0; i < a.nseg; ++i)
      STTS_CHECK(a.seg[i].ldx % 8 == 0 && a.seg[i].xcol0 % 8 == 0, "conv_gemm: 16-bit activation rows need ldx / xcol0 multiples of 8 (segment %d)", i);
  GemmPlan plan = plan_conv_gemm(a, epi, npad, n_utt, max_rows, force_tile, gemm_switches());
  STTS_CHECK(plan.ok(), "%s", plan.err);
  if (plan.route == ROUTE_GEMM16) return launch_conv_gemm16_main(st, a, npad, n_utt);
  if (a.prec != PREC_F32)
    for (int i = 0; i < a.nseg; ++i) STTS_CHECK(a.seg[i].W16 != nullptr, "conv_gemm: 16-bit operand mode without 16-bit weights (segment %d)", i);
  const int tile = plan.tile, bn = plan.bn();
  GemmArgs as = a;
  as.n_utt = n_utt;
  if (!as.zeros) as.zeros = zero_page();
  as.compact = a.seg_host != nullptr;
  float* part = nullptr;
  if (plan.main_ksp > 1 || plan.rem_rt > 0) {
    part = splitk_scratch(st, (size_t)std::max(plan.main_ksp, plan.rem_ksp) * a.rows_total * npad * sizeof(float));
    if (!part) {
      plan.main_ksp = 1;
      plan.full_rt += plan.rem_rt;
      plan.rem_rt = 0;
    }
  }
  GemmProfiler& prof = gemm_profiler();
  const double flops = gemm_algorithmic_flops(a);
  const long all_rt = plan.full_rt + plan.rem_rt;
  auto launch_range = [&](long tile0, long ntiles, int ksp) {
    as.tile0 = (int)tile0;
    as.tiles_y = (int)ntiles;
    as.ksplit = ksp;
    as.partial = ksp > 1 ? part : nullptr;
    as.ld_part = npad;
    hipEvent_t e0 = nullptr, e1 = nullptr;
    if (prof.on) {
      e0 = prof.next();
      e1 = prof.next();
      prof.add(plan.route == ROUTE_X3 ? "conv_gemm_f32_x3" : "conv_gemm_f32", 0, flops * (double)ntiles / (double)all_rt, flops * (double)ntiles / (double)all_rt, 0.0);
    }
    if (plan.route == ROUTE_X3) gemm_dispatch_x3(st, as, tile, epi, npad, n_utt, max_rows, e0, e1);
    else if (plan.route == ROUTE_BF16) gemm_dispatch_bf16(st, as, tile, epi, npad, n_utt, max_rows, e0, e1);
    else if (plan.route == ROUTE_F16) gemm_dispatch_f16(st, as, tile, epi, npad, n_utt, max_rows, e0, e1);
    else gemm_dispatch_f32(st, as, tile, epi, npad, n_utt, max_rows, e0, e1);
    if (ksp > 1 && a.defer && tile0 == 0 && ntiles == all_rt) {
      *a.defer = SplitInfo{part, ksp, a.rows_total, npad};
    } else if (ksp > 1) {
      int row_first = 0;
      if (tile0 > 0) {
        long t = tile0;
        for (int u = 0; u < n_utt; ++u) {
          const long tu = ceil_div(a.seg_host[u + 1] - a.seg_host[u], bn);
          if (t < tu) {
            row_first = a.seg_host[u] + (int)t * bn;
            break;
          }
          t -= tu;
        }
      }
      const long work = (long)(a.rows_total - row_first) * ((a.N + 3) / 4);
      STTS_LAUNCH_PROF("splitk_reduce_kernel", (size_t)work * 4 * 4 * (ksp + 1), splitk_reduce_kernel, dim3((unsigned)std::min<long>(2048, (work + 255) / 256)), dim3(256), st, part, ksp, a.rows_total,
                         row_first, npad, a.N, a.bias, a.act, a.R, a.ldr, a.rcol0, a.alpha, a.Y, a.ldy, a.ycol0);
    }
  };
  if (a.defer) *a.defer = SplitInfo{nullptr, 1, 0, 0};
  if (plan.full_rt > 0) launch_range(0, plan.full_rt, plan.main_ksp);
  if (plan.rem_rt > 0) launch_range(plan.full_rt, plan.rem_rt, plan.rem_ksp);
  STTS_HIP(hipGetLastError());
  return 0;
}
#ifdef STTS_GEMM_TU_FORM
#if STTS_GEMM_TU_FORM == 0
void gemm_dispatch_f32(hipStream_t st, const GemmArgs& as, int tile, int epi, int npad, int n_utt, int max_rows, hipEvent_t e0, hipEvent_t e1) {
  gemm_dispatch_tile<PREC_F32>(st, as, tile, epi, npad, n_utt, max_rows, e0, e1);
}
// ... 18 lines not shown
```

### stylish_tts_amd/csrc/gemm_plan.hip.h

```cpp
#pragma once
#include <climits>
#include <cstdio>

namespace stts {

enum : unsigned { FORM_F32 = 1, FORM_16 = 2, FORM_X3 = 4 };
enum TileX16 { X16_NEVER, X16_MAY, X16_MUST };
struct TileRow {
  int id, BM, BN, WM, WN, KS;
  bool glds;
  unsigned forms;
  TileX16 x16;
  bool store_only;
  bool paired;
  bool xaff;
  bool splitk;
};
constexpr unsigned kAllForms = FORM_F32 | FORM_16 | FORM_X3;
constexpr TileRow kTiles[] = {
    {2, 128, 64, 2, 2, 1, false, kAllForms, X16_MAY, false, true, true, true},
    {3, 128, 32, 2, 1, 1, false, kAllForms, X16_MAY, false, true, true, true},
    {4, 128, 32, 4, 1, 1, false, kAllForms, X16_MAY, false, false, true, true},
    {5, 128, 128, 4, 2, 1, false, kAllForms, X16_MAY, false, false, true, true},
    {6, 128, 64, 4, 2, 1, false, kAllForms, X16_MAY, false, false, true, true},
    {8, 128, 128, 4, 2, 2, false, kAllForms, X16_NEVER, false, false, true, false},
    {11, 128, 128, 4, 2, 1, true, FORM_F32, X16_NEVER, false, false, false, true},
    {13, 128, 64, 4, 2, 1, true, FORM_F32, X16_NEVER, false, false, false, true},
    {14, 256, 256, 4, 2, 1, false, FORM_16, X16_MAY, true, false, true, true},
    {15, 128, 256, 4, 2, 1, false, FORM_16, X16_MAY, true, false, true, true},
    {16, 256, 256, 4, 2, 1, true, FORM_16, X16_MUST, true, false, false, true},
    {17, 128, 256, 4, 2, 1, true, FORM_16, X16_MUST, true, false, false, true},
    {18, 128, 128, 4, 2, 1, true, FORM_16, X16_MUST, true, false, false, true},
    {20, 128, 128, 2, 2, 1, false, FORM_X3, X16_MAY, false, true, true, true},
    {21, 128, 128, 2, 2, 2, false, FORM_X3, X16_MAY, false, true, true, false},
    {22, 128, 256, 2, 4, 1, false, FORM_X3, X16_MAY, false, true, true, true},
    {25, 128, 128, 4, 2, 1, false, FORM_X3, X16_MUST, true, false, false, false},
    {26, 128, 64, 4, 2, 1, false, FORM_X3, X16_MUST, true, false, false, false},
    {27, 128, 128, 4, 2, 1, true, FORM_X3, X16_MUST, true, false, false, false},
    {28, 128, 64, 4, 2, 1, true, FORM_X3, X16_MUST, true, false, false, false},
};
constexpr const TileRow* find_tile(int id) {
  for (const TileRow& r : kTiles)
    if (r.id == id) return &r;
  return nullptr;
}
constexpr TileRow tile_row(int id) { return *find_tile(id); }
constexpr int presplit_tile(int bn, bool glds) {
  for (const TileRow& r : kTiles)
    if ((r.forms & FORM_X3) && r.x16 == X16_MUST && r.glds == glds && r.BN == (bn >= 128 ? 128 : 64)) return r.id;
  return 0;
}
struct GemmSwitches {
  static constexpr int kUnset = INT_MIN;
  bool no_x3;
  bool x3_rem;
  int x3_tile;
  bool x3p_glds;
  int tile16;
  int splitk_min_iters;
  long gemm16_min_tiles;
};
inline const GemmSwitches& gemm_switches() {
  static const GemmSwitches sw = [] {
    auto num = [](const char* name, int unset) { return getenv(name) ? atoi(getenv(name)) : unset; };
    GemmSwitches s;
    s.no_x3 = num("STTS_NO_X3", 0) != 0;
    s.x3_rem = num("STTS_X3_REM", 0) != 0;
    s.x3_tile = num("STTS_X3_TILE", GemmSwitches::kUnset);
    s.x3p_glds = num("STTS_X3P_GLDS", 1) != 0;
    s.tile16 = num("STTS_TILE16", GemmSwitches::kUnset);
    s.splitk_min_iters = getenv("STTS_SPLITK_MIN_ITERS") ? std::max(1, atoi(getenv("STTS_SPLITK_MIN_ITERS"))) : 0;
    s.gemm16_min_tiles = getenv("STTS_GEMM16_MIN_TILES") ? atol(getenv("STTS_GEMM16_MIN_TILES")) : 192;
    return s;
  }();
  return sw;
}
inline bool x3_enabled() { return !gemm_switches().no_x3; }

enum GemmRoute { ROUTE_GEMM16, ROUTE_X3, ROUTE_BF16, ROUTE_F16, ROUTE_F32 };
struct GemmPlan {
  GemmRoute route = ROUTE_F32;
  int tile = 0;
  long full_rt = 0, rem_rt = 0;
  int rem_ksp = 1, main_ksp = 1;
  char err[256] = "";
  bool ok() const { return err[0] == 0; }
  int bn() const { return find_tile(tile)->BN; }
};
#define STTS_PLAN_CHECK(cond, ...)                    \
  do {                                                \
    if (!(cond)) {                                    \
      snprintf(p.err, sizeof(p.err), __VA_ARGS__);    \
      return p;                                       \
    }                                                 \
  } while (0)

constexpr int kG16Tile = 256;
constexpr int kG16K = 64;
inline bool gemm16_eligible(const GemmArgs& a, int epi, int npad) {
  if (epi != EPI_STORE || a.prec == PREC_F32 || !a.x16 || !a.seg_host || a.xaff || npad % kG16Tile != 0 || a.N % 4 != 0) return false;
  if (a.ldy % 4 || a.ycol0 % 4 || a.ldr % 4 || a.rcol0 % 4 || a.ldy16 % 4 || a.ycol16 % 4 || a.ld_ss % 4 || a.ld_stat % 4) return false;
  for (int i = 0; i < a.nseg; ++i)
    if (a.seg[i].kc % kG16K != 0 || a.seg[i].ldx % 8 != 0 || a.seg[i].xcol0 % 8 != 0 || !a.seg[i].W16 || a.seg[i].ldx - a.seg[i].xcol0 < a.seg[i].kc) return false;
  return true;
}

inline long gemm16_tiles(const GemmArgs& a, int npad, int n_utt) {
  long rt = 0;
  for (int u = 0; u < n_utt; ++u) rt += ceil_div(a.seg_host[u + 1] - a.seg_host[u], kG16Tile);
  return rt * (npad / kG16Tile);
}

inline bool gemm16_route(const GemmArgs& a, int epi, int npad, int n_utt, int force_tile, const GemmSwitches& sw) {
  if (force_tile != 0 && force_tile != 19) return false;
  return gemm16_eligible(a, epi, npad) && (force_tile == 19 || gemm16_tiles(a, npad, n_utt) >= sw.gemm16_min_tiles);
}
inline bool gemm16_will_run(const GemmArgs& a, int epi, int npad, int n_utt) { return gemm16_route(a, epi, npad, n_utt, 0, gemm_switches()); }

constexpr int kCUs = 256;
inline long gemm_row_tiles(const GemmArgs& a, int n_utt, int max_rows, int bn) {
  if (!a.seg_host) return (long)n_utt * ceil_div(max_rows, bn);
  long t = 0;
  for (int u = 0; u < n_utt; ++u) t += ceil_div(a.seg_host[u + 1] - a.seg_host[u], bn);
  return t;
}
struct RowPlan {
  long full_rt = 0, rem_rt = 0;
  int rem_ksp = 1;
  double cost = 0;
};
inline RowPlan plan_rows(long rt, int mt, int iters, bool may_split_rem, int bn, double penalty) {
  RowPlan p;
  const long blocks = rt * mt, whole = blocks / kCUs;
  p.full_rt = rt;
  p.cost = std::ceil((double)blocks / kCUs);
  if (may_split_rem && whole >= 1 && blocks % kCUs != 0) {
    const long full_rt = whole * kCUs / mt, rem_blocks = (rt - full_rt) * mt;
    const int ksp = (int)std::min<long>(8, std::min<long>(iters / 4, kCUs / std::max<long>(rem_blocks, 1)));
    if (ksp >= 2 && full_rt > 0) {
      const double hybrid = (double)(full_rt * mt) / kCUs + std::max((double)rem_blocks / kCUs, 1.0 / ksp) * 1.15 + 0.1;
      if (hybrid < p.cost) {
        p.full_rt = full_rt;
        p.rem_rt = rt - full_rt;
        p.rem_ksp = ksp;
        p.cost = hybrid;
      }
    }
  }
  p.cost *= bn * penalty;
  return p;
}
inline bool tile_fits(GemmPlan& p, int tile, const GemmArgs& a, int epi, int npad, unsigned form) {
  const TileRow* r = find_tile(tile);
  const bool paired = epi != EPI_STORE && epi != EPI_SPLIT_ACC;
  if (!r) snprintf(p.err, sizeof(p.err), "conv_gemm: no tile %d", tile);
  else if (!(r->forms & form) || (a.x16 ? r->x16 == X16_NEVER || a.xaff : r->x16 == X16_MUST) || (a.xaff && !r->xaff) || (epi != EPI_STORE && r->store_only) ||
           (paired && !r->paired) || npad % r->BM != 0)
    snprintf(p.err, sizeof(p.err), "conv_gemm: tile %d does not take this launch (operand form %u, 16-bit rows / pre-split planes %d, input affine %d, epilogue %d, cout padded to %d): see kTiles", tile, form,
              a.x16, a.xaff != nullptr, epi, npad);
  return p.ok();
}

inline GemmPlan plan_conv_gemm(const GemmArgs& a, int epi, int npad, int n_utt, int max_rows, int force_tile, const GemmSwitches& sw) {
  GemmPlan p;
  if (gemm16_route(a, epi, npad, n_utt, force_tile, sw)) {
    p.route = ROUTE_GEMM16;
    p.tile = 19;
    return p;
  }
  STTS_PLAN_CHECK(!a.stat_part, "conv_gemm: output statistics (stat_part) exist only in conv_gemm16_kernel's epilogue: ask gemm16_will_run first");
  STTS_PLAN_CHECK(force_tile != 19, "conv_gemm: tile 19 (conv_gemm16_kernel) needs 16-bit activation rows, a store epilogue, channels in multiples of 64 and cout padded to 256");
  const int mt = npad / 128;
  int iters = 0;
  for (int i = 0; i < a.nseg; ++i) iters += a.seg[i].ntaps * (a.seg[i].kc / 32);
  const bool splittable = force_tile == 0 && epi == EPI_STORE && !a.sumsq_part && a.Y && !a.Y16;
  const long blocks128 = mt * gemm_row_tiles(a, n_utt, max_rows, 128);
  bool x3 = a.prec == PREC_F32 && !sw.no_x3 && (epi == EPI_STORE || epi == EPI_PRIOR);
  for (int i = 0; i < a.nseg; ++i) x3 = x3 && a.seg[i].W16 != nullptr && a.seg[i].w16_plane > 0 && 6 * a.seg[i].w16_plane + 2L * 128 * a.seg[i].ntaps * a.seg[i].kc < (1L << 32);
  if (a.x16 && a.prec == PREC_F32) {
    STTS_PLAN_CHECK(x3 && epi == EPI_STORE && !a.xaff && !a.sumsq_part, "conv_gemm: pre-split activation planes need the split-fp32 store contraction");
    for (int i = 0; i < a.nseg; ++i) STTS_PLAN_CHECK(a.seg[i].x_plane > 0 && a.seg[i].ldx % 8 == 0 && a.seg[i].xcol0 % 8 == 0, "conv_gemm: pre-split activation planes: segment %d misaligned", i);
  }
  if (force_tile >= 100) {
    x3 = false;
    force_tile -= 100;
  }
  if (force_tile != 0) {
    const TileRow* f = find_tile(force_tile);
    STTS_PLAN_CHECK(f, "conv_gemm: no tile %d", force_tile);
    if (!(f->forms & FORM_X3) || (f->x16 == X16_MUST && !a.x16)) x3 = false;
  }
  const bool may_split_rem = (!x3 || sw.x3_rem) && splittable && a.seg_host && !a.capacity;
  int tile = force_tile;
  const bool paired = epi != EPI_STORE && epi != EPI_SPLIT_ACC;
  RowPlan rows;
  if (tile == 0) {
    if (blocks128 < 24) tile = paired ? 3 : 4;
    else if (paired) tile = 2;
    else {
      const RowPlan p5 = plan_rows(gemm_row_tiles(a, n_utt, max_rows, 128), mt, iters, may_split_rem, 128, 1.0);
      const RowPlan p6 = plan_rows(gemm_row_tiles(a, n_utt, max_rows, 64), mt, iters, may_split_rem, 64, 1.03);
      tile = p5.cost <= p6.cost ? 5 : 6;
      if (x3 && iters <= 24 && !a.xaff) tile = 6;
      rows = tile == 5 ? p5 : p6;
      if (tile == 5 && blocks128 <= kCUs && a.prec == PREC_F32 && !x3) tile = 8;
    }
  }
  const long rt256 = gemm_row_tiles(a, n_utt, max_rows, 256);
  if (force_tile == 0 && a.prec != PREC_F32 && a.x16 && epi == EPI_STORE) {
    if (npad % 256 == 0 && iters >= 128 && rt256 * (npad / 256) >= 3 * kCUs / 2) tile = 14;
    else if (rt256 * (npad / 128) >= 3 * kCUs / 2) tile = 15;
    if (tile == 14 || tile == 15) rows = RowPlan();
    if (sw.tile16 != GemmSwitches::kUnset) {
      tile = sw.tile16;
      rows = RowPlan();
    }
  }
  const unsigned form = x3 ? FORM_X3 : a.prec == PREC_F32 ? FORM_F32 : FORM_16;
  if (!tile_fits(p, tile, a, epi, npad, form)) return p;
  const bool x3_large = x3 && !a.x16 && force_tile == 0 && (tile == 5 || tile == 6);
  if (x3_large && (sw.x3_tile == 5 || sw.x3_tile == 6 || sw.x3_tile == 22)) {
    tile = sw.x3_tile;
    rows = RowPlan();
  }
  const long blocks22 = rt256 * mt;
  const bool fills22 = blocks22 >= 640 || (blocks22 >= 440 && (blocks22 % kCUs == 0 || blocks22 % kCUs >= kCUs * 4 / 5));
  if (x3_large && fills22 && sw.x3_tile == GemmSwitches::kUnset) {
    tile = 22;
    rows = RowPlan();
  }
  if (x3 && a.x16) {
    if (find_tile(tile)->x16 != X16_MUST) tile = presplit_tile(find_tile(tile)->BN, sw.x3p_glds);
    rows = RowPlan();
  }
  if (!tile_fits(p, tile, a, epi, npad, form)) return p;
  const TileRow& row = *find_tile(tile);
  if ((rows.full_rt == 0 && rows.rem_rt == 0) || !row.splitk) rows = RowPlan{gemm_row_tiles(a, n_utt, max_rows, row.BN), 0, 1, 0};
  p.route = x3 ? ROUTE_X3 : a.prec == PREC_BF16 ? ROUTE_BF16 : a.prec == PREC_F16 ? ROUTE_F16 : ROUTE_F32;
  p.tile = tile;
  p.full_rt = rows.full_rt;
  p.rem_rt = rows.rem_rt;
  p.rem_ksp = rows.rem_ksp;
  if (splittable && row.splitk && p.rem_rt == 0) {
    const long blocks = p.full_rt * mt;
    const int min_it = sw.splitk_min_iters ? sw.splitk_min_iters : (blocks >= 128 ? 8 : 4);
    p.main_ksp = (int)std::min<long>(8, std::min<long>(iters / min_it, ((a.prec == PREC_F32 && !x3) ? 512 : 255) / std::max<long>(blocks, 1)));
    if (p.main_ksp < 2) p.main_ksp = 1;
  }
  return p;
}

}
```

### stylish_tts_amd/csrc/model.hip.h

```cpp
#pragma once
#include <math.h>

#include <array>
#include <map>
#include <memory>
#include <mutex>
#include <string>
#include <vector>

#include "../../include/stylish_hip.h"
#include "common.h"
#include "elementwise.hip.h"
#include "gemm.hip.h"
#include "gemm16.hip.h"
#include "signal.hip.h"
#include "signal_geom.hip.h"
#include "phoneme.hip.h"
#include "wn_layer.hip.h"
#include "wn_layer_small.hip.h"
#include "wn_fused.hip.h"
#include "wn_fused16.hip.h"
#include "wn_block16.hip.h"
#include "wn_fused_x3.hip.h"
#include "wn_block_x3.hip.h"
#include "winograd.hip.h"

namespace stts {

struct HostTensor {
  std::vector<int64_t> shape;
  std::vector<float> data;
  int64_t dim(int i) const { return shape[i]; }
};

struct PackedConv {
  float* W = nullptr;
  unsigned short* W16 = nullptr;
  long w16_plane = 0;
  int prec = 0;
  float* bias = nullptr;
  int npad = 0, N = 0, kc = 0, ntaps = 1;
  int cin_real = 0, rows_real = 0;
};

struct WinoConv {
  PackedConv planes;
  WinoMats mats;
  int pad = 0;
  bool ready = false;
};

struct StyleSlot {
  int col0 = 0, C = 0;
};

struct StyleTable {
  std::vector<float> hW, hb;
  float* W = nullptr;
  float* b = nullptr;
  int J = 0, K = 64;
  int add(const HostTensor& w, const HostTensor& bias) {
    while (J % 4) {
      hW.insert(hW.end(), K, 0.f);
      hb.push_back(0.f);
      ++J;
    }
    const int c0 = J;
    hW.insert(hW.end(), w.data.begin(), w.data.end());
    hb.insert(hb.end(), bias.data.begin(), bias.data.end());
    J += (int)bias.data.size();
    return c0;
  }
  int ld() const { return round_up(J, 4); }
};

struct AdainBlockW {
  int cin = 0, cout = 0, kcin = 0;
  PackedConv conv1, conv2, sc;
  WinoConv w1, w2;
  StyleSlot n1, n2;
};

struct WnFusedW {
  float* W1[3][4] = {};
  float* b1[4] = {};
  float* W2[4] = {};
  float* b2[4] = {};
  float* W3 = nullptr;
  float* b3m = nullptr;
  float* b3s = nullptr;
  float* W4 = nullptr;
  float* b4 = nullptr;
  unsigned short* H1[4] = {};
  unsigned short* H2[4] = {};
  unsigned short* H2b[4] = {};
  unsigned short* H3 = nullptr;
  unsigned short* H4 = nullptr;
  unsigned short* X1[4] = {};
  unsigned short* X2[4] = {};
  unsigned short* X2b[4] = {};
  unsigned short* X3 = nullptr;
  unsigned short* X4 = nullptr;
  long xp1 = 0, xp2[4] = {}, xp3 = 0, xp4 = 0;
  bool ready = false;
  bool ready16 = false;
  bool ready_x3 = false;
};

struct FlowLayerW {
  PackedConv pre, in[4], rs[4], proj;
  WnFusedW fused;
  int cond_col0 = 0;
};

struct ConvNextW {
  float* dw_wt = nullptr;
  float* dw_b = nullptr;
  int K = 0;
  StyleSlot norm;
  PackedConv pw1, pw2;
  float* grn_gamma = nullptr;
};

struct MrfW {
  PackedConv c1[3], c2[3];
  StyleSlot a1[3], a2[3];
  float* alpha1[3];
  float* alpha2[3];
  int dil[3] = {1, 3, 5};
  int channels = 0, kernel = 0;
  StyleTable table;
};

struct PackMode {
  int prec;
  bool x3;
  int kc_align;
  int tag;
};

}

struct stts_ctx {
  stts_model_dims d;
  int device = 0;
  std::map<std::string, stts::HostTensor> host;
  std::vector<void*> allocs;
  std::vector<int> alloc_tag;
  int* d_err = nullptr;
  struct SideLane {
    hipStream_t stream = nullptr;
    hipEvent_t fork = nullptr, join = nullptr;
    hipStream_t stream2 = nullptr;
    hipEvent_t fork2 = nullptr, join2 = nullptr;
  };
  std::map<hipStream_t, SideLane> side_lanes;
  std::mutex side_mu;
  int ready = 0;
  int prec = 0;
  bool allow_x3 = true;
  stts::PackMode pack{-1, true, 32, 0};
  stts::SignalGeom geom;
  bool force_generic_signal = false;
  float* hann = nullptr;
  float2* twiddle = nullptr;
  double2* twiddle64 = nullptr;
  float front_wf[3], front_bf, front_wn[3], front_bn;
  stts::PackedConv asr_res;
  stts::AdainBlockW dec[5];
  stts::StyleTable dec_style;
  stts::PackedConv prior, post_flow;
  stts::FlowLayerW flow[8];
  stts::StyleTable flow_style;
  stts::PackedConv amp_prior, phase_prior, proj_mel, proj_la, proj_ph, amp_out, phase_out;
  stts::WinoConv wino_prior[2], wino_out[2];
  float* nyq_w[2] = {nullptr, nullptr};
  float nyq_b[2] = {0.f, 0.f};
  stts::ConvNextW cnx[4];
  stts::StyleSlot head_amp, head_phase;
  stts::StyleTable gen_style;
  std::map<std::string, std::unique_ptr<stts::AdainBlockW>> op_blocks;
  std::map<std::string, std::unique_ptr<stts::StyleTable>> op_tables;
  std::map<std::string, std::unique_ptr<stts::MrfW>> op_mrf;
  std::shared_ptr<void> phoneme;
  std::shared_ptr<void> cfm;
  std::shared_ptr<void> hubert;
  std::shared_ptr<void> mel_style;
  std::shared_ptr<void> cfm_pitch;
  std::shared_ptr<void> ssl;
  std::shared_ptr<void> rmvpe;
  std::shared_ptr<void> aligner;
  std::map<std::array<int, 4>, std::shared_ptr<void>> log_mel;
  std::mutex log_mel_mu;
};

namespace stts {

struct PackScope {
  stts_ctx* c;
  PackMode saved;
  PackScope(stts_ctx* ctx, const PackMode& m) : c(ctx), saved(ctx->pack) { c->pack = m; }
  ~PackScope() { c->pack = saved; }
  PackScope(const PackScope&) = delete;
  PackScope& operator=(const PackScope&) = delete;
};
inline PackMode engine_mode(const stts_ctx* c) { return {c->prec, true, 32, 0}; }
inline bool packs_x3(const stts_ctx* c) { return c->allow_x3 && c->pack.x3 && x3_enabled(); }

template <typename T>
inline int dev_upload(stts_ctx* c, const std::vector<T>& h, T** out) {
  STTS_CHECK(c->pack.prec >= 0, "dev_upload outside a PackScope");
  void* p = nullptr;
  STTS_HIP(hipMalloc(&p, std::max<size_t>(h.size(), 1) * sizeof(T)));
  c->allocs.push_back(p);
  c->alloc_tag.push_back(c->pack.tag);
  if (!h.empty()) STTS_HIP(hipMemcpy(p, h.data(), h.size() * sizeof(T), hipMemcpyHostToDevice));
  *out = (T*)p;
  return 0;
}

inline void free_component_allocs(stts_ctx* c, int mask) {
// ... 4 lines not shown
  size_t k = 0;
  for (size_t i = 0; i < c->allocs.size(); ++i) {
    if (c->alloc_tag[i] & mask) {
      (void)hipFree(c->allocs[i]);
    } else {
      c->allocs[k] = c->allocs[i];
      c->alloc_tag[k++] = c->alloc_tag[i];
    }
  }
  c->allocs.resize(k);
  c->alloc_tag.resize(k);
}

inline const HostTensor* find(stts_ctx* c, const std::string& name) {
  auto it = c->host.find(name);
  return it == c->host.end() ? nullptr : &it->second;
}
#define STTS_GET(var, name)                                   \
  const stts::HostTensor* var = stts::find(c, (name));        \
  if (!var) return stts::fail("missing weight '%s'", std::string(name).c_str())

inline HostTensor fold_weight_norm(const HostTensor& g, const HostTensor& v) {
  HostTensor w;
  w.shape = v.shape;
  w.data.resize(v.data.size());
  const int64_t rows = v.shape[0], per = (int64_t)v.data.size() / rows;
  for (int64_t r = 0; r < rows; ++r) {
    double s = 0;
    for (int64_t i = 0; i < per; ++i) s += (double)v.data[r * per + i] * v.data[r * per + i];
    const float scale = g.data[r] / (float)sqrt(s);
    for (int64_t i = 0; i < per; ++i) w.data[r * per + i] = v.data[r * per + i] * scale;
  }
  return w;
}

inline int get_weight(stts_ctx* c, const std::string& p, HostTensor* w) {
  if (const HostTensor* g = find(c, p + ".parametrizations.weight.original0")) {
    STTS_GET(v, p + ".parametrizations.weight.original1");
    *w = fold_weight_norm(*g, *v);
  } else if (const HostTensor* g2 = find(c, p + ".weight_g")) {
    STTS_GET(v, p + ".weight_v");
    *w = fold_weight_norm(*g2, *v);
  } else {
    STTS_GET(v, p + ".weight");
    *w = *v;
  }
  if (w->shape.size() == 2) w->shape.push_back(1);
  return 0;
}

inline unsigned short f32_to_bf16(float f) {
  unsigned u;
  memcpy(&u, &f, 4);
  if ((u & 0x7fffffffu) > 0x7f800000u) return (unsigned short)((u >> 16) | 0x40);
  return (unsigned short)((u + 0x7fffu + ((u >> 16) & 1u)) >> 16);
}
inline float bf16_to_f32(unsigned short h) {
  const unsigned u = (unsigned)h << 16;
  float f;
  memcpy(&f, &u, 4);
  return f;
}
inline void split3_host(float f, unsigned short* p0, unsigned short* p1, unsigned short* p2) {
  if (std::isinf(f)) {
    *p0 = *p1 = 0;
    *p2 = f32_to_bf16(f);
    return;
  }
  const unsigned tbits = 0x7f7f7fffu;
  float tmax;
  memcpy(&tmax, &tbits, 4);
  *p0 = f32_to_bf16(f != f ? f : std::fmin(std::fmax(f, -tmax), tmax));
  const float r1 = f - bf16_to_f32(*p0);
  *p1 = f32_to_bf16(r1);
  *p2 = f32_to_bf16(r1 - bf16_to_f32(*p1));
}
inline unsigned short f32_to_f16(float f) {
  const _Float16 h = (_Float16)f;
  unsigned short r;
  memcpy(&r, &h, 2);
  return r;
}

inline int pack_rows(stts_ctx* c, const HostTensor& w, const HostTensor* bias, const std::vector<int>& row_of, int cin_lo, int cin_n,
                     int kc, int N, PackedConv* out, float scale = 1.0f) {
  STTS_CHECK(c->pack.prec >= 0, "pack_rows outside a PackScope");
  const int prec = c->pack.prec;
  const int cin = (int)w.shape[1], k = (int)w.shape[2];
  const int npad = (int)row_of.size();
  std::vector<float> pw((size_t)npad * k * kc, 0.f), pb(npad, 0.f);
  for (int n = 0; n < npad; ++n) {
    const int r = row_of[n];
    if (r < 0) continue;
    for (int t = 0; t < k; ++t)
      for (int ci = 0; ci < cin_n; ++ci) pw[((size_t)n * k + t) * kc + ci] = w.data[((size_t)r * cin + cin_lo + ci) * k + t] * scale;
    if (bias) pb[n] = bias->data[r] * scale;
  }
  STTS_TRY(dev_upload(c, pw, &out->W));
  STTS_TRY(dev_upload(c, pb, &out->bias));
  out->prec = prec;
  out->W16 = nullptr;
  out->w16_plane = 0;
  if (prec != PREC_F32 || packs_x3(c)) {
    const bool split = prec == PREC_F32;
    std::vector<unsigned short> h(pw.size() * (split ? 3 : 1));
    if (split) {
      out->w16_plane = (long)pw.size();
      for (size_t i = 0; i < pw.size(); ++i) split3_host(pw[i], &h[i], &h[pw.size() + i], &h[2 * pw.size() + i]);
    } else
    for (size_t i = 0; i < pw.size(); ++i) h[i] = prec == PREC_BF16 ? f32_to_bf16(pw[i]) : f32_to_f16(pw[i]);
    STTS_TRY(dev_upload(c, h, &out->W16));
  }
  out->npad = npad;
  out->N = N;
  out->kc = kc;
  out->ntaps = k;
  out->cin_real = cin_n;
  out->rows_real = 0;
  for (int r : row_of) out->rows_real += r >= 0;
  return 0;
}

inline std::vector<int> plain_rows(int cout) {
  std::vector<int> r(round_up(cout, 128), -1);
  for (int i = 0; i < cout; ++i) r[i] = i;
  return r;
}
inline std::vector<int> paired_rows(int nres, int a_lo, int b_lo) {
  std::vector<int> r(round_up(2 * nres, 128), -1);
  for (int ch = 0; ch < nres; ++ch) {
    const int g = ch / 32, q = ch % 32;
    r[g * 64 + q] = a_lo + ch;
    r[g * 64 + 32 + q] = b_lo + ch;
  }
  return r;
}

inline int pack_plain(stts_ctx* c, const std::string& p, bool has_bias, int cin_lo, int cin_n, PackedConv* out, float scale = 1.0f) {
  HostTensor w;
  STTS_TRY(get_weight(c, p, &w));
  const HostTensor* b = has_bias ? find(c, p + ".bias") : nullptr;
  if (has_bias && !b) return fail("missing weight '%s.bias'", p.c_str());
  if (cin_n < 0) cin_n = (int)w.shape[1] - cin_lo;
  return pack_rows(c, w, b, plain_rows((int)w.shape[0]), cin_lo, cin_n, round_up(cin_n, c->pack.kc_align), (int)w.shape[0], out, scale);
}

inline int upload_table(stts_ctx* c, StyleTable* t) {
  while (t->J % 4) {
    t->hW.insert(t->hW.end(), t->K, 0.f);
    t->hb.push_back(0.f);
    ++t->J;
  }
  STTS_TRY(dev_upload(c, t->hW, &t->W));
  STTS_TRY(dev_upload(c, t->hb, &t->b));
  return 0;
}

inline int add_style(stts_ctx* c, StyleTable* t, const std::string& p, int C, StyleSlot* slot) {
  STTS_GET(w, p + ".fc.weight");
  STTS_GET(b, p + ".fc.bias");
  STTS_CHECK((int)b->data.size() == 2 * C, "%s.fc has %zu outputs, expected %d", p.c_str(), b->data.size(), 2 * C);
  slot->col0 = t->add(*w, *b);
  slot->C = C;
  return 0;
}

inline int pack_winograd(stts_ctx* c, const HostTensor& w, const HostTensor* bias, int cin_lo, int cin_n, int cout_used, WinoConv* out) {
  static const bool disabled = getenv("STTS_NO_WINOGRAD") != nullptr;
  if (disabled) return 0;
  STTS_CHECK(c->pack.prec >= 0, "pack_winograd outside a PackScope");
  const int cin = (int)w.shape[1], r = (int)w.shape[2];
  STTS_CHECK(wino_matrices(r, &out->mats), "winograd: unsupported kernel size %d (or self-check failed)", r);
  const int n = out->mats.n, npad = round_up(cout_used, 128), kc = round_up(cin_n, 32);
  HostTensor wp;
  wp.shape = {(int64_t)n * cout_used, cin, 1};
  wp.data.assign((size_t)n * cout_used * cin, 0.f);
  for (int j = 0; j < n; ++j)
    for (int co = 0; co < cout_used; ++co)
      for (int ci = 0; ci < cin; ++ci) {
        double acc = 0;
        for (int k = 0; k < r; ++k) acc += out->mats.G[j][k] * (double)w.data[((size_t)co * cin + ci) * r + k];
        wp.data[((size_t)j * cout_used + co) * cin + ci] = (float)acc;
      }
  std::vector<int> row_of((size_t)n * npad, -1);
  for (int j = 0; j < n; ++j)
    for (int co = 0; co < cout_used; ++co) row_of[(size_t)j * npad + co] = j * cout_used + co;
  {
    PackMode f32 = c->pack;
    f32.prec = PREC_F32;
    PackScope scope(c, f32);
    STTS_TRY(pack_rows(c, wp, nullptr, row_of, cin_lo, cin_n, kc, cout_used, &out->planes));
  }
  out->planes.npad = npad;
  out->planes.cin_real = cin_n;
// ... 331 lines not shown
    for (int i = 0; i < 4; ++i) STTS_TRY(pack_convnext_block(c, g + "convnext." + std::to_string(i) + ".", h, ks[i], &c->gen_style, &c->cnx[i]));
    STTS_TRY(add_style(c, &c->gen_style, g + "amp_final_layer_norm", h, &c->head_amp));
    STTS_TRY(add_style(c, &c->gen_style, g + "phase_final_layer_norm", h, &c->head_phase));
    STTS_TRY(upload_table(c, &c->gen_style));
  }
  c->ready |= which & (STTS_W_DECODER | STTS_W_FLOW | STTS_W_GENERATOR);
  return 0;
}

struct DryRun {
  bool on = false;
  size_t peak = 0;
};
inline DryRun& dry_run() {
  static thread_local DryRun d;
  return d;
}
#define STTS_DRY_RETURN(arena)                                                   \
  do {                                                                            \
    if (stts::dry_run().on) {                                                     \
      stts::dry_run().peak = std::max(stts::dry_run().peak, (arena).offset0 + (arena).used); \
      return 0;                                                                   \
    }                                                                             \
  } while (0)

struct Arena {
  char* base;
  size_t cap, used = 0;
  size_t offset0 = 0;
  bool ok = true;
  Arena(void* p, size_t n, size_t off0 = 0) : base((char*)p), cap(n), offset0(off0) {}
  template <typename T>
  T* get(size_t count) {
    const size_t bytes = (count * sizeof(T) + 255) / 256 * 256;
    if (used + bytes > cap) {
      ok = false;
      return nullptr;
    }
    T* p = (T*)(base + used);
    used += bytes;
    return p;
  }
};

struct Seg {
  int n_utt;
  const int* host;
  const int* dev;
  bool cap = false;
  const int* rows_dev() const { return cap ? dev + n_utt : nullptr; }
  int rows() const { return host[n_utt]; }
  int max_len() const {
    int m = 0;
    for (int i = 0; i < n_utt; ++i) m = std::max(m, host[i + 1] - host[i]);
    return m;
  }
};

inline GemmArgs gemm_args(const Seg& s) {
  GemmArgs a;
  memset(&a, 0, sizeof(a));
  a.seg_off = s.dev;
  a.seg_host = s.host;
  a.n_utt = s.n_utt;
  a.rows_total = s.rows();
  a.capacity = s.cap;
  if (!s.cap && s.host && s.n_utt > 0) {
    const int len = s.host[1] - s.host[0];
    bool same = len > 0;
    for (int u = 1; u < s.n_utt && same; ++u) same = s.host[u + 1] - s.host[u] == len;
    if (same) { a.uniform_len = len; a.uniform_lo0 = s.host[0]; }
  }
  a.alpha = 1.0f;
  a.xaff_slope = 0.2f;
  a.zeros = zero_page();
  return a;
}
inline void set_seg(GemmArgs& a, int i, const float* X, int ldx, int xcol0, const PackedConv& w, int pad = -1, int dil = 1) {
  GemmSeg& g = a.seg[i];
  g.X = X;
  g.W = w.W;
  g.W16 = w.W16;
  g.w16_plane = w.w16_plane;
  if (i == 0) a.prec = w.prec;
  g.w_utt_stride = 0;
  g.ldx = ldx;
  g.xcol0 = xcol0;
  g.kc = w.kc;
  g.ntaps = w.ntaps;
  g.dil = dil;
  g.pad = pad >= 0 ? pad : (w.ntaps - 1) / 2;
  g.kreal = w.cin_real;
  if (i == 0) a.wrows = w.rows_real;
  if (a.nseg < i + 1) a.nseg = i + 1;
}

struct WinoScratch {
  float* p = nullptr;
  bool setup = false;
  explicit operator bool() const { return p != nullptr; }
};
inline size_t wino_scratch_floats(const Seg& s, const WinoConv& wc) {
  const long pr = wino_plane_rows(s.rows(), s.n_utt);
  return (size_t)wc.mats.n * pr * (wc.planes.kc * 3 / 2 + round_up(wc.planes.N, 32)) + round_up(s.n_utt + 1 + 16, 32) + 32;
}
template <int N>
inline int run_winograd_n(hipStream_t st, const Seg& s, const float* X, int ldx, const WinoConv& wc, float* Y, int ldy, int act, const float* R, int ldr,
                          float alpha, WinoScratch& scratch, const float* aff = nullptr, int ld_aff = 0, float* stat = nullptr, int ld_stat = 0) {
  const int n = wc.mats.n, kc = wc.planes.kc, ldm = round_up(wc.planes.N, 32), ml = s.max_len();
  long pr = 0;
  for (int u = 0; u < s.n_utt; ++u) pr += ceil_div(s.host[u + 1] - s.host[u], kWinoM);
  const long pr_cap = wino_plane_rows(s.rows(), s.n_utt);
  int* segp = reinterpret_cast<int*>(scratch.p);
  int* goff = segp + 16;
  float* Xp = scratch.p + round_up(s.n_utt + 1 + 16, 32);
  static const bool presplit_env = getenv("STTS_X3_PRESPLIT") && atoi(getenv("STTS_X3_PRESPLIT")) != 0;
  const bool presplit = presplit_env && x3_enabled() && wc.planes.w16_plane > 0 && wc.planes.prec == PREC_F32 && kc % 8 == 0;
  const long xplane = (long)n * pr_cap * kc;
  float* Mp = Xp + (size_t)n * pr_cap * kc * 3 / 2;
  WinoIn ti;
  WinoOut to;
  memcpy(ti.Bt, wc.mats.Bt, sizeof(ti.Bt));
  memcpy(to.At, wc.mats.At, sizeof(to.At));
  const int groups = ceil_div(ml, kWinoM);
  GemmProfiler& prof = gemm_profiler();
  const bool timed = prof.on;
  if (timed) {
    (void)hipEventRecord(prof.next(), st);
    prof.on = false;
  }
  if (!scratch.setup) {
    hipLaunchKernelGGL(wino_setup_kernel, dim3(1), dim3(64), 0, st, s.dev, s.n_utt, kWinoMaxN, goff, segp);
    scratch.setup = true;
  }
  if (presplit)
    hipLaunchKernelGGL((winograd_input_kernel<N, true>), dim3(ceil_div(groups, 4), ceil_div(kc / 4, 64), s.n_utt), dim3(64, 4), 0, st, X, ldx,
                       wc.planes.cin_real, s.dev, wc.pad, ti, Xp, kc, goff, aff, ld_aff, xplane);
  else
  hipLaunchKernelGGL((winograd_input_kernel<N>), dim3(ceil_div(groups, 4), ceil_div(kc / 4, 64), s.n_utt), dim3(64, 4), 0, st, X, ldx,
                     wc.planes.cin_real, s.dev, wc.pad, ti, Xp, kc, goff, aff, ld_aff, 0L);
  std::vector<int> seg_h(n + 1);
  for (int j = 0; j <= n; ++j) seg_h[j] = (int)(j * pr);
  Seg sp{n, seg_h.data(), segp};
  sp.cap = s.cap;
  GemmArgs a = gemm_args(sp);
  set_seg(a, 0, Xp, kc, 0, wc.planes, 0);
  a.seg[0].w_utt_stride = (long)wc.planes.npad * kc;
  if (presplit) {
    a.x16 = 1;
    a.seg[0].x_plane = xplane;
  }
  a.N = wc.planes.N; a.bias = nullptr; a.Y = Mp; a.ldy = ldm;
  {
    const int rc = launch_conv_gemm(st, a, EPI_STORE, wc.planes.npad, n, (int)pr);
    if (rc) {
      prof.on = timed;
      return rc;
    }
  }
  if (stat)
    hipLaunchKernelGGL((winograd_output_kernel<N, true>), dim3(ceil_div(groups, 4), ceil_div(ceil_div(wc.planes.N, 4), 64), s.n_utt), dim3(64, 4), 0, st, Mp, ldm, goff,
                       s.dev, to, wc.planes.bias, act, R, ldr, alpha, Y, ldy, wc.planes.N, stat, ld_stat, ceil_div(groups, 4));
  else
    hipLaunchKernelGGL((winograd_output_kernel<N, false>), dim3(ceil_div(groups, 4), ceil_div(ceil_div(wc.planes.N, 4), 64), s.n_utt), dim3(64, 4), 0, st, Mp, ldm, goff,
                       s.dev, to, wc.planes.bias, act, R, ldr, alpha, Y, ldy, wc.planes.N, nullptr, 0, 0);
  if (timed) {
    prof.on = true;
    (void)hipEventRecord(prof.next(), st);
    prof.add((x3_enabled() && wc.planes.w16_plane > 0) ? "winograd_conv_x3" : "winograd_conv", 0, 2.0 * (double)s.rows() * wc.planes.rows_real * wc.planes.cin_real * wc.mats.r,
             2.0 * (double)n * (double)pr * wc.planes.rows_real * wc.planes.cin_real, 0.0);
  }
  STTS_HIP(hipGetLastError());
  return 0;
}
inline int wino_stat_chunks(const Seg& s) { return ceil_div(ceil_div(s.max_len(), kWinoM), 4); }
inline int run_winograd(hipStream_t st, const Seg& s, const float* X, int ldx, const WinoConv& wc, float* Y, int ldy, int act, const float* R, int ldr,
                        float alpha, WinoScratch& scratch, const float* aff = nullptr, int ld_aff = 0, float* stat = nullptr, int ld_stat = 0) {
  STTS_CHECK(wc.ready && (wc.mats.n == 8 || wc.mats.n == 12), "winograd conv not packed");
  STTS_CHECK(ldx % 4 == 0 && ldy % 4 == 0 && (!R || ldr % 4 == 0), "winograd conv: leading dimensions must be multiples of 4");
  STTS_CHECK(!stat || (ld_stat % 4 == 0 && ld_stat >= round_up(wc.planes.N, 4)), "winograd conv: statistics rows of %d floats do not cover %d channels", ld_stat, wc.planes.N);
  return wc.mats.n == 8 ? run_winograd_n<8>(st, s, X, ldx, wc, Y, ldy, act, R, ldr, alpha, scratch, aff, ld_aff, stat, ld_stat)
                        : run_winograd_n<12>(st, s, X, ldx, wc, Y, ldy, act, R, ldr, alpha, scratch, aff, ld_aff, stat, ld_stat);
}

inline int run_style(hipStream_t st, const StyleTable& t, const float* style, int n_utt, float* out) {
  if (n_utt >= 16 && t.K % 4 == 0 && t.K <= 128) {
    STTS_LAUNCH_PROF("style_fc_batch_kernel", (size_t)t.J * (t.K + n_utt) * 4, style_fc_batch_kernel, dim3(ceil_div(t.J, 4)), dim3(256), st, t.W, t.b, style, out,
                     t.J, t.K, n_utt, t.K, t.ld());
    STTS_HIP(hipGetLastError());
    return 0;
  }
  STTS_LAUNCH_PROF("style_fc_kernel", (size_t)t.J * (t.K + n_utt) * 4, style_fc_kernel, dim3(ceil_div(t.J, 4)), dim3(256), st, t.W, t.b, style, out, t.J, t.K, n_utt, t.K, t.ld());
  STTS_HIP(hipGetLastError());
  return 0;
}

inline dim3 rows_grid(const Seg& s, int per_row_work) {
  const long total = (long)s.max_len() * per_row_work;
  return dim3((unsigned)std::min<long>(std::max<long>(1, ceil_div((int)std::min<long>(total, 1 << 30), 256)), 512), s.n_utt);
}

inline long rows16_threshold() {
  static const long v = getenv("STTS_ROWS16") ? atol(getenv("STTS_ROWS16")) : 3840;
  return v;
}

inline size_t adain_part_floats(const Seg& s, int C, int chunk_rows = kStatChunk) { return (size_t)s.n_utt * ceil_div(s.max_len(), chunk_rows) * 2 * round_up(C, 32); }
inline int run_adain(hipStream_t st, const Seg& s, const float* X, int ldx, int C, float* Y, int ldy, const float* style_out, int ld_style,
                     int gcol0, int act, const float* alpha, float* part, int out16 = 0, bool have_stats = false) {
  const int nchunk = ceil_div(s.max_len(), kStatChunk), ldp = round_up(C, 32);
  if (!have_stats)
    STTS_LAUNCH_PROF("adain_partial_kernel", (size_t)s.rows() * C * 4, adain_partial_kernel, dim3(ceil_div(C, 32), nchunk, s.n_utt), dim3(256), st, X, ldx, C, s.dev, part, ldp, nchunk, kStatChunk);
  const int rb = (long)ceil_div(ldy, 64) * ceil_div(s.rows(), 64) >= 4096 ? 256 : 64;
  STTS_LAUNCH_PROF("adain_apply_kernel", (size_t)s.rows() * (C * 4 + ldy * (out16 ? 2 : 4)), adain_apply_kernel, dim3(ceil_div(ldy, 64), ceil_div(s.max_len(), rb), s.n_utt), dim3(256), st, X, ldx, Y, ldy, C, s.dev,
                     part, ldp, nchunk, style_out, ld_style, gcol0, 1e-5f, act, alpha, out16, rb);
  STTS_HIP(hipGetLastError());
  return 0;
}

struct PendingReduce {
  SplitSrc src{};
  float* Y = nullptr;
  int ldy = 0;
};
inline void pending_from(PendingReduce* p, const SplitInfo& info, const GemmArgs& a) {
  p->src = SplitSrc{};
  if (info.ksplit > 1) {
    p->src = SplitSrc{info.partial, info.ksplit, info.slice_rows, info.ld_part, a.N, a.bias, a.act, a.R, a.ldr, a.rcol0, a.alpha};
    p->Y = a.Y + a.ycol0;
    p->ldy = a.ldy;
  }
}
inline int pending_finish(hipStream_t st, PendingReduce* p) {
  if (!p || !p->src.partial) return 0;
  const SplitSrc& r = p->src;
  const long work = (long)r.slice_rows * ((r.N + 3) / 4);
  STTS_LAUNCH_PROF("splitk_reduce_kernel", (size_t)work * 4 * 4 * (r.ksplit + 1), splitk_reduce_kernel, dim3((unsigned)std::min<long>(2048, (work + 255) / 256)), dim3(256), st, r.partial,
                   r.ksplit, r.slice_rows, 0, r.ld_part, r.N, r.bias, r.act, r.R, r.ldr, r.rcol0, r.alpha, p->Y, p->ldy, 0);
  p->src = SplitSrc{};
  STTS_HIP(hipGetLastError());
  return 0;
}
inline long fold_rows() {
  static const long v = getenv("STTS_FOLD_ROWS") ? atol(getenv("STTS_FOLD_ROWS")) : 2500;
  return v;
}
struct SideWork {
  hipStream_t stream = nullptr;
  hipEvent_t fork = nullptr, join = nullptr;
  float* out = nullptr;
};
struct AdainStats {
  float* in = nullptr;
  bool in_ready = false;
  float* mid = nullptr;
  float* out = nullptr;
  int out_ld = 0;
  bool out_ready = false;
  int chunk_rows = kStatChunk;
};
inline int run_adain_block(hipStream_t st, const Seg& s, const AdainBlockW& B, const float* style_out, int ld_style, const float* x, int ldx,
                           float* y, int ldy, float* act1, float* hbuf, float* act2, float* ss, int force_tile = 0, WinoScratch* wino = nullptr,
                           unsigned short* xs16 = nullptr, bool xs16_ready = false, unsigned short* y16 = nullptr, int ldy16 = 0,
                           AdainStats* stats = nullptr, PendingReduce* pend_in = nullptr, PendingReduce* pend_out = nullptr, const SideWork* side = nullptr) {
  const int ml = s.max_len();
// ... 264 lines not shown
  STTS_CHECK(ws.ok, "harmonic_stft: workspace too small");
  if (g.generic) STTS_CHECK(ld >= g.bins, "harmonic_stft: row stride %d < %d bins", ld, g.bins);
  else STTS_CHECK(ld >= kBins && ld <= 64 * ((kBins + 63) / 64), "harmonic_stft: row stride %d outside [%d, %d]", ld, kBins, 64 * ((kBins + 63) / 64));
  STTS_DRY_RETURN(ws);
  if (!s.cap)
    for (int u = 0; u < s.n_utt; ++u)
      STTS_CHECK((long)(s.host[u + 1] - s.host[u]) * g.h > g.n_fft / 2, "utterance %d too short for reflect padding (%d frames; need > %d samples)", u,
                 s.host[u + 1] - s.host[u], g.n_fft / 2);
  if (g.generic) {
    STTS_TRY(launch_pcph_geom(st, g, s.n_utt, s.dev, R, s.max_len(), pitch, noise, init_phase, batch_scope, prefix, stats, sig, c->d_err));
    STTS_TRY(launch_stft_geom(st, g, s.n_utt, s.dev, R, s.max_len(), sig, c->hann, c->twiddle64, har_spec, har_phase, ld, out16));
    STTS_HIP(hipGetLastError());
    return 0;
  }
  STTS_LAUNCH_PROF("pcph_prep_kernel", (size_t)R * 12, pcph_prep_kernel, dim3(s.n_utt), dim3(256), st, pitch, s.dev, prefix, stats);
  STTS_LAUNCH_PROF("pcph_kernel", (size_t)R * kHop * 8, pcph_kernel, dim3(std::min(1024, ceil_div(s.max_len() * kHop, 256)), s.n_utt), dim3(256), st, pitch, s.dev, s.n_utt,
                     prefix, stats, noise, init_phase, batch_scope, sig, c->d_err);
  STTS_LAUNCH_PROF("stft_kernel", (size_t)R * (kHop + 2 * kBins) * 4, stft_kernel, dim3((s.max_len() + kFftWaves - 1) / kFftWaves, s.n_utt), dim3(64 * kFftWaves), st, sig, s.dev, c->hann, c->twiddle64, har_spec, har_phase, ld, out16);
  STTS_HIP(hipGetLastError());
  return 0;
}

inline int ln_launch(hipStream_t st, const float* X, int ldx, int C, long n_rows, const int* row_utt, float eps, int adaptive, int nout,
                     const LnOut& o0, const LnOut& o1, int act, const LnIn& in = LnIn{}, const int* n_rows_dev = nullptr) {
  STTS_LAUNCH_PROF("row_layernorm_kernel", (size_t)n_rows * C * (1 + nout) * 4, row_layernorm_kernel, dim3((unsigned)ceil_div((int)n_rows, 4)), dim3(256), st, X, ldx, C, (int)n_rows, row_utt, eps,
                     adaptive, nout, o0, o1, act, in, n_rows_dev);
  STTS_HIP(hipGetLastError());
  return 0;
}

struct ConvNextScratch {
  float *dw, *nrm, *U, *part;
  int ss_stride;
  float *gscale, *w2u;
  const int* row_utt;
};

inline int convnext_block_forward(hipStream_t st, const Seg& s, const ConvNextW& B, int h, int inter, const float* sty, int lds, int p16, const float* cur,
                                  float* nxt, const ConvNextScratch& sc) {
  const long R = s.rows();
  const int ml = s.max_len();
  float *dw = sc.dw, *nrm = sc.nrm, *U = sc.U, *part = sc.part, *gscale = sc.gscale, *w2u = sc.w2u;
  const int ss_stride = sc.ss_stride;
  const int* row_utt = sc.row_utt;
  if (h <= kDwLnMaxC && h % 4 == 0 && (B.K == 3 || B.K == 7 || B.K == 15 || B.K == 31)) {
    const dim3 fg(ceil_div(ml, 16), s.n_utt);
    const size_t fb = (size_t)R * h * (4 + (p16 ? 2 : 4));
#define STTS_DWLN(KK) STTS_LAUNCH_PROF("dwconv_ln_kernel", fb, (dwconv_ln_kernel<KK, 16>), fg, dim3(256), st, cur, h, h, s.dev, B.dw_wt, B.dw_b, 1e-6f, sty, lds, B.norm.col0, nrm, h, p16)
    if (B.K == 3) STTS_DWLN(3);
    else if (B.K == 7) STTS_DWLN(7);
    else if (B.K == 15) STTS_DWLN(15);
    else STTS_DWLN(31);
#undef STTS_DWLN
  } else {
    STTS_CHECK(row_utt, "convnext_block_forward: this block needs the row -> utterance table");
    STTS_LAUNCH_PROF("dwconv_kernel", (size_t)R * h * 2 * 4, (dwconv_kernel<31>), dim3(ceil_div(h, 64), ceil_div(ml, 64), s.n_utt), dim3(256), st, cur, h, dw, h, h, s.dev, B.dw_wt,
                       B.dw_b, B.K, (int)ACT_NONE);
    LnOut o0{nrm, h, 0, sty, nullptr, lds, B.norm.col0, p16}, o1{};
    STTS_TRY(ln_launch(st, dw, h, h, R, row_utt, 1e-6f, 1, 1, o0, o1, ACT_NONE, LnIn{}, s.rows_dev()));
  }
  GemmArgs a = gemm_args(s);
  set_seg(a, 0, nrm, h, 0, B.pw1);
  a.N = inter; a.bias = B.pw1.bias; a.act = ACT_SILU;
  a.x16 = p16 != 0;
  if (p16) { a.Y = nullptr; a.Y16 = reinterpret_cast<unsigned short*>(U); a.ldy16 = inter; }
  else { a.Y = U; a.ldy = inter; }
  a.sumsq_part = part; a.ld_ss = inter; a.ss_stride = ss_stride;
  STTS_TRY(launch_conv_gemm(st, a, EPI_STORE, B.pw1.npad, s.n_utt, ml));
  STTS_LAUNCH_PROF("grn_gx_kernel", (size_t)s.n_utt * ss_stride * inter * 4, grn_gx_kernel, dim3(ceil_div(inter, 32), s.n_utt), dim3(256), st, part, inter, ss_stride, s.dev, inter, gscale, inter);
  GemmArgs b = gemm_args(s);
  set_seg(b, 0, U, inter, 0, B.pw2);
  if (B.pw2.prec == PREC_F32 && B.pw2.w16_plane > 0 && x3_enabled()) {
    hipLaunchKernelGGL(grn_xaff_kernel, dim3(s.n_utt), dim3(256), 0, st, gscale, inter, B.grn_gamma, w2u, B.pw2.kc, inter);
    b.xaff = w2u;
    b.ld_xaff = B.pw2.kc;
    b.xaff_slope = 1.0f;
    static const bool no_scale_only = getenv("STTS_XAFF_GENERAL") != nullptr;
    b.xaff_scale_only = B.pw2.kc == inter && !no_scale_only;
  } else {
    launch_scale_weight(st, dim3(128, s.n_utt), B.pw2.prec, B.pw2.W, gscale, inter, B.grn_gamma, w2u, B.pw2.npad, B.pw2.kc);
    b.seg[0].W = w2u;
    b.seg[0].W16 = reinterpret_cast<const unsigned short*>(w2u);
    b.seg[0].w16_plane = 0;
    b.seg[0].w_utt_stride = (long)B.pw2.npad * B.pw2.kc;
  }
  b.x16 = p16 != 0;
  b.N = h; b.bias = B.pw2.bias; b.Y = nxt; b.ldy = h; b.R = cur; b.ldr = h;
  STTS_TRY(launch_conv_gemm(st, b, EPI_STORE, B.pw2.npad, s.n_utt, ml));
  return 0;
}

inline bool vocoder_rows16(const stts_ctx* c, long rows) { return c->prec != PREC_F32 && rows >= rows16_threshold(); }

inline int prior_conv(stts_ctx* c, hipStream_t st, const Seg& s, int which, const float* har, int ld_har, float* head, WinoScratch* wino = nullptr,
                      unsigned short* har16 = nullptr, bool har_is16 = false) {
  const int h = c->d.gen_hidden, hp = h / 2, hc = h + hp;
  const PackedConv& w = which == 0 ? c->amp_prior : c->phase_prior;
  if (wino && *wino && c->wino_prior[which].ready)
    return run_winograd(st, s, har, ld_har, c->wino_prior[which], head + h, hc, ACT_NONE, nullptr, 0, 1.0f, *wino);
  GemmArgs a = gemm_args(s);
  set_seg(a, 0, har, ld_har, 0, w);
  a.N = hp; a.bias = w.bias;
  if (vocoder_rows16(c, s.rows())) {
    STTS_CHECK((har16 || har_is16) && ld_har % 8 == 0, "prior_conv: 16-bit mode needs the rounded-copy scratch");
    if (!har_is16) launch_cast_rows(st, c->prec, har, ld_har, c->geom.bins, har16, ld_har, s.rows());
    a.seg[0].X = har_is16 ? har : reinterpret_cast<const float*>(har16);
    a.x16 = 1;
    a.Y = nullptr; a.Y16 = reinterpret_cast<unsigned short*>(head); a.ldy16 = hc; a.ycol16 = h;
  } else {
    a.Y = head; a.ldy = hc; a.ycol0 = h;
  }
  return launch_conv_gemm(st, a, EPI_STORE, w.npad, s.n_utt, s.max_len());
}

inline int vocoder_body(stts_ctx* c, hipStream_t st, const Seg& s, const float* mel, int ld_mel, const float* style, float* headA, float* headP,
                        float* audio, float* logamp_out, float* phase_out, int ld_lp, Arena& ws, const unsigned short* mel16_in = nullptr) {
  const stts_model_dims& d = c->d;
  const long R = s.rows();
  const int h = d.gen_hidden, hp = h / 2, hc = h + hp, inter = d.gen_inter, ml = s.max_len();
  const SignalGeom& geo = c->geom;
  const int ldlp = round_up(geo.bins, 32);
  float* xa = ws.get<float>(R * h);
  float* xb = ws.get<float>(R * h);
  float* dw = ws.get<float>(R * h);
  float* nrm = ws.get<float>(R * h);
  float* U = ws.get<float>(R * inter);
  const int ss_stride = ceil_div(ml, 128) * 4;
  float* part = ws.get<float>((size_t)s.n_utt * ss_stride * inter);
  float* gscale = ws.get<float>((size_t)s.n_utt * inter);
  float* w2u = ws.get<float>((size_t)s.n_utt * c->cnx[0].pw2.npad * inter);
  float* sty = ws.get<float>((size_t)s.n_utt * c->gen_style.ld());
  int* row_utt = ws.get<int>(R);
  float* la = logamp_out ? logamp_out : ws.get<float>(R * ldlp);
  float* ph = phase_out ? phase_out : ws.get<float>(R * ldlp);
  const int ldl = logamp_out ? ld_lp : ldlp;
  const int p16 = (c->prec != PREC_F32 && vocoder_rows16(c, R)) ? c->prec : 0;
  unsigned short* mel16 = (p16 && !mel16_in) ? ws.get<unsigned short>(R * round_up(d.gen_input, 32)) : nullptr;
  float* yw = ws.get<float>((R + s.n_utt) * geo.win);
  WinoScratch wino;
  if (c->wino_out[0].ready && c->wino_out[1].ready) wino.p = ws.get<float>(wino_scratch_floats(s, c->wino_out[0]));
  STTS_CHECK(ws.ok, "vocoder: workspace too small");
  STTS_DRY_RETURN(ws);
  STTS_CHECK(!logamp_out == !phase_out, "logamp_out and phase_out must be given together");
  const int lds = c->gen_style.ld();
  STTS_TRY(run_style(st, c->gen_style, style, s.n_utt, sty));
  STTS_LAUNCH_PROF("row_utt_kernel", (size_t)R * 4, row_utt_kernel, dim3(ceil_div(ml, 256), s.n_utt), dim3(256), st, s.dev, s.n_utt, row_utt);
  {
    GemmArgs a = gemm_args(s);
    if (p16) {
      const int ldm16 = round_up(d.gen_input, 32);
      if (!mel16_in) launch_cast_rows(st, p16, mel, ld_mel, d.gen_input, mel16, ldm16, R);
      set_seg(a, 0, reinterpret_cast<const float*>(mel16_in ? mel16_in : mel16), ldm16, 0, c->proj_mel);
      a.x16 = 1;
    } else {
      set_seg(a, 0, mel, ld_mel, 0, c->proj_mel);
    }
    set_seg(a, 1, headA, hc, h, c->proj_la);
    set_seg(a, 2, headP, hc, h, c->proj_ph);
    a.N = h; a.bias = c->proj_mel.bias; a.Y = xa; a.ldy = h;
    STTS_TRY(launch_conv_gemm(st, a, EPI_STORE, c->proj_mel.npad, s.n_utt, ml));
  }
  float* cur = xa;
  float* nxt = xb;
  const ConvNextScratch cs{dw, nrm, U, part, ss_stride, gscale, w2u, row_utt};
  for (int i = 0; i < 4; ++i) {
    STTS_TRY(convnext_block_forward(st, s, c->cnx[i], h, inter, sty, lds, p16, cur, nxt, cs));
// ... 188 lines not shown
```

### stylish_tts_amd/csrc/phoneme_model.hip.h

```cpp
#pragma once

namespace stts {

struct TextEncW {
  bool ready = false;
  float* emb = nullptr;
  int C = 0, inter = 0, heads = 0, n_layers = 0, ffk = 0, filter = 0, tokens = 0;
  PackedConv pre[3], pre_proj, proj_m;
  float* pre_g[3];
  float* pre_b[3];
  struct Layer {
    PackedConv qkv, o, f1, f2;
    float *g1, *b1, *g2, *b2;
  } layer[16];
};

struct StyleEncW {
  bool ready = false;
  int inter = 0, sd = 0, n = 0;
  PackedConv conv_in;
  struct Blk {
    float *dw_wt, *dw_b, *ln_g, *ln_b, *grn_gamma;
    PackedConv pw1, pw2;
  } blk[8];
// ... 278 lines not shown
  STTS_HIP(hipGetLastError());
  return 0;
}
inline void run_rope(hipStream_t st, const Seg& s, float* X, int ldx, int col0, int heads, int kc, int col1 = -1) {
  const int d = (int)(kc * 0.5);
  hipLaunchKernelGGL(rope_kernel, dim3(std::max(1, ceil_div(s.max_len() * heads * (d / 2) * (col1 >= 0 ? 2 : 1), 256)), s.n_utt), dim3(256), 0, st, X,
                     ldx, col0, col1, heads, kc, d, s.dev);
}

inline int encoder_layers_forward(hipStream_t st, const TextEncW& W, const Seg& s, float* x, float* t, float* qkv, float* att, float* ff) {
  const int C = W.C;
  const int kc = C / W.heads;
  for (int i = 0; i < W.n_layers; ++i) {
    const TextEncW::Layer& L = W.layer[i];
    STTS_TRY(gemm_store(st, s, x, C, 0, L.qkv, qkv, 3 * C, 0));
    run_rope(st, s, qkv, 3 * C, 0, W.heads, kc, C);
    STTS_TRY(run_attention(st, s, s, qkv, 3 * C, 0, qkv, 3 * C, C, qkv, 3 * C, 2 * C, att, C, W.heads, kc, nullptr, 0));
    STTS_TRY(gemm_ln(st, s, att, C, L.o, t, C, x, C, C, 1e-4f, 0, nullptr, LnOut{x, C, 0, L.g1, L.b1, 0, 0}, ACT_NONE));
    STTS_TRY(gemm_store(st, s, x, C, 0, L.f1, ff, W.filter, 0, ACT_RELU));
    STTS_TRY(gemm_ln(st, s, ff, W.filter, L.f2, t, C, x, C, C, 1e-4f, 0, nullptr, LnOut{x, C, 0, L.g2, L.b2, 0, 0}, ACT_NONE));
  }
  return 0;
}

inline int text_encoder_forward(stts_ctx* c, hipStream_t st, const TextEncW& W, const Seg& s, const long* tokens, float* mu, int ld_mu, float* x_out,
                                Arena& ws) {
  const long R = s.rows();
  const int C = W.C;
  float* x = ws.get<float>(R * C);
  float* h = ws.get<float>(R * C);
  float* t = ws.get<float>(R * C);
  float* qkv = ws.get<float>(R * 3 * C);
  float* att = ws.get<float>(R * C);
  float* ff = ws.get<float>(R * W.filter);
  STTS_CHECK(ws.ok, "text_encoder_forward: workspace too small");
  hipLaunchKernelGGL(embed_kernel, dim3((unsigned)std::min<long>(1024, ceil_div((int)(R * C / 4), 256))), dim3(256), 0, st, tokens, W.emb, C, W.tokens,
                     sqrtf((float)C), x, C, (int)R, c->d_err);
  const float* cur = x;
  for (int i = 0; i < 3; ++i) {
    STTS_TRY(gemm_ln(st, s, cur, C, W.pre[i], t, C, nullptr, 0, C, 1e-4f, 0, nullptr, LnOut{h, C, 0, W.pre_g[i], W.pre_b[i], 0, 0}, ACT_RELU));
    cur = h;
  }
  STTS_TRY(gemm_store(st, s, h, C, 0, W.pre_proj, t, C, 0, ACT_NONE, x, C));
  std::swap(x, t);
  STTS_TRY(encoder_layers_forward(st, W, s, x, t, qkv, att, ff));
  if (x_out) STTS_HIP(hipMemcpyAsync(x_out, x, R * C * sizeof(float), hipMemcpyDeviceToDevice, st));
  STTS_TRY(gemm_store(st, s, x, C, 0, W.proj_m, mu, ld_mu, 0));
  return 0;
}

inline int text_style_forward(stts_ctx* c, hipStream_t st, const StyleEncW& W, const Seg& s, const float* x, int ldx, float* style, int ld_style,
                              Arena& ws) {
  (void)c;
  const long R = s.rows();
  const int sd = W.sd, inter4 = 4 * sd, ml = s.max_len();
  float* h = ws.get<float>(R * sd);
  float* h2 = ws.get<float>(R * sd);
  float* dw = ws.get<float>(R * sd);
  float* nrm = ws.get<float>(R * sd);
  float* U = ws.get<float>(R * inter4);
  const int ss_stride = ceil_div(ml, 128) * 4;
  float* part = ws.get<float>((size_t)s.n_utt * ss_stride * inter4);
  float* gx = ws.get<float>((size_t)s.n_utt * inter4);
  float* w2u = ws.get<float>((size_t)s.n_utt * W.blk[0].pw2.npad * inter4);
  STTS_CHECK(ws.ok, "text_style_forward: workspace too small");
  STTS_TRY(gemm_store(st, s, x, ldx, 0, W.conv_in, h, sd, 0));
  for (int i = 0; i < W.n; ++i) {
    const StyleEncW::Blk& B = W.blk[i];
    hipLaunchKernelGGL((dwconv_kernel<31>), dim3(ceil_div(sd, 64), ceil_div(ml, 64), s.n_utt), dim3(256), 0, st, h, sd, dw, sd, sd, s.dev, B.dw_wt, B.dw_b,
                       7, (int)ACT_NONE);
    STTS_TRY(static_ln(st, dw, sd, sd, R, 1e-6f, B.ln_g, B.ln_b, nrm, sd, ACT_NONE));
    GemmArgs a = gemm_args(s);
    set_seg(a, 0, nrm, sd, 0, B.pw1);
    a.N = inter4; a.bias = B.pw1.bias; a.Y = U; a.ldy = inter4; a.act = ACT_GELU;
    a.sumsq_part = part; a.ld_ss = inter4; a.ss_stride = ss_stride;
    STTS_TRY(launch_conv_gemm(st, a, EPI_STORE, B.pw1.npad, s.n_utt, ml));
    hipLaunchKernelGGL(grn_gx_kernel, dim3(ceil_div(inter4, 32), s.n_utt), dim3(256), 0, st, part, inter4, ss_stride, s.dev, inter4, gx, inter4);
    launch_scale_weight(st, dim3(8, s.n_utt), B.pw2.prec, B.pw2.W, gx, inter4, B.grn_gamma, w2u, B.pw2.npad, B.pw2.kc);
    GemmArgs b = gemm_args(s);
    set_seg(b, 0, U, inter4, 0, B.pw2);
    b.seg[0].W = w2u;
    b.seg[0].W16 = reinterpret_cast<const unsigned short*>(w2u);
    b.seg[0].w16_plane = 0;
    b.seg[0].w_utt_stride = (long)B.pw2.npad * B.pw2.kc;
    b.N = sd; b.bias = B.pw2.bias; b.Y = h2; b.ldy = sd; b.R = h; b.ldr = sd;
    STTS_TRY(launch_conv_gemm(st, b, EPI_STORE, B.pw2.npad, s.n_utt, ml));
    std::swap(h, h2);
  }
  hipLaunchKernelGGL(mean_rows_kernel, dim3(s.n_utt), dim3(256), 0, st, h, sd, sd, s.dev, style, ld_style);
  STTS_HIP(hipGetLastError());
  return 0;
}

inline int prosody_forward(hipStream_t st, const ProsodyW& W, const Seg& s, const float* enc, int ld_enc, const float* style, const float* sty,
                           int ld_sty, const int* row_utt, float* out, Arena& ws) {
  const long R = s.rows();
  const int C = W.C, d = W.d, sd = C - d, kc = C / W.heads;
  float* x = out;
  float* t = ws.get<float>(R * C);
  float* y = ws.get<float>(R * C);
  float* qkv = ws.get<float>(R * 3 * C);
  float* att = ws.get<float>(R * C);
  float* ff = ws.get<float>(R * 2 * C);
  STTS_CHECK(ws.ok, "prosody_forward: workspace too small");
  STTS_HIP(hipMemcpy2DAsync(x, C * sizeof(float), enc, ld_enc * sizeof(float), d * sizeof(float), R, hipMemcpyDeviceToDevice, st));
  hipLaunchKernelGGL(broadcast_style_kernel, dim3(std::max(1, ceil_div(s.max_len() * sd, 256)), s.n_utt), dim3(256), 0, st, style, sd, sd, x, C, d, s.dev);
  for (int i = 0; i < W.n_layers; ++i) {
    const ProsodyW::L& L = W.l[i];
    STTS_TRY(gemm_store(st, s, x, C, 0, L.qkv, qkv, 3 * C, 0));
    run_rope(st, s, qkv, 3 * C, 0, W.heads, kc, C);
    STTS_TRY(run_attention(st, s, s, qkv, 3 * C, 0, qkv, 3 * C, C, qkv, 3 * C, 2 * C, att, C, W.heads, kc, nullptr, 0));
    STTS_TRY(gemm_ln(st, s, att, C, L.o, t, C, x, C, C, 1e-5f, 1, row_utt, LnOut{y, C, 0, sty, nullptr, ld_sty, L.n1.col0}, ACT_NONE));
    STTS_TRY(gemm_store(st, s, y, C, 0, L.f1, ff, 2 * C, 0, ACT_RELU));
    STTS_TRY(gemm_ln(st, s, ff, 2 * C, L.f2, t, C, y, C, C, 1e-5f, 1, row_utt, LnOut{y, C, 0, sty, nullptr, ld_sty, L.n2.col0}, ACT_NONE));
    STTS_TRY(gemm_store(st, s, y, C, 0, L.proj, x, C, 0));
  }
  return 0;
}

inline size_t phoneme_workspace_bytes(const stts_ctx* c, int64_t n_tok, int64_t n_frames, int n_utt) {
  const stts_model_dims& d = c->d;
  const size_t C = d.te_hidden, Cp = d.pe_inter + d.style_dim;
  const size_t tok = (size_t)n_tok * (C * 8 + d.te_filter + Cp * 12 + d.style_dim * 12 + 64) * sizeof(float);
  const size_t frm = (size_t)n_frames * (Cp * 12 + 16) * sizeof(float) + ((size_t)n_frames / kWinoM + n_utt + 1) * 8 * 2 * Cp * sizeof(float);
  const size_t per = (size_t)n_utt * ((size_t)(n_tok / std::max(1, n_utt) / 32 + 16) * 4 * d.style_dim * 8 + 128 * 256 + 8192) * sizeof(float);
  return tok + frm + per + ((size_t)4 << 20);
}

inline int duration_forward(stts_ctx* c, PhonemeModel& M, hipStream_t st, const Seg& s, const long* tokens, float* logits, int ld_logits, int* dur_out,
                            float* mu_out, float* style_out, float* prosody_out, Arena& ws) {
  const long R = s.rows();
  const DurationW& D = M.dur;
  const int d = c->d.inter_dim, C = D.pros.C;
  float* mu = mu_out ? mu_out : ws.get<float>(R * d);
  float* style = style_out ? style_out : ws.get<float>((size_t)s.n_utt * c->d.style_dim);
  float* pros = prosody_out ? prosody_out : ws.get<float>(R * C);
  float* sty = ws.get<float>((size_t)s.n_utt * D.table.ld());
  int* row_utt = ws.get<int>(R);
  STTS_CHECK(ws.ok, "duration_forward: workspace too small");
  hipLaunchKernelGGL(row_utt_kernel, dim3(ceil_div(s.max_len(), 256), s.n_utt), dim3(256), 0, st, s.dev, s.n_utt, row_utt);
  { Arena a(ws.base + ws.used, ws.cap - ws.used); STTS_TRY(text_encoder_forward(c, st, M.te[0], s, tokens, mu, d, nullptr, a)); }
  { Arena a(ws.base + ws.used, ws.cap - ws.used); STTS_TRY(text_style_forward(c, st, M.se[0], s, mu, d, style, c->d.style_dim, a)); }
  STTS_TRY(run_style(st, D.table, style, s.n_utt, sty));
  { Arena a(ws.base + ws.used, ws.cap - ws.used); STTS_TRY(prosody_forward(st, D.pros, s, mu, d, style, sty, D.table.ld(), row_utt, pros, a)); }
  STTS_TRY(gemm_store(st, s, pros, C, 0, D.proj, logits, ld_logits, 0));
  if (dur_out) hipLaunchKernelGGL(duration_decode_kernel, dim3(ceil_div((int)R, 256)), dim3(256), 0, st, logits, ld_logits, 16, (int)R, dur_out);
  STTS_HIP(hipGetLastError());
  return 0;
}

inline int pitch_energy_forward(stts_ctx* c, PhonemeModel& M, hipStream_t st, const Seg& sp, const Seg& sf, const int* dur, const float* pe_enc, int ld_enc,
                                const float* pe_style, float* f0, float* nrg, float* prosody_out, float* cross_out, Arena& ws) {
  const PitchEnergyW& P = M.pe;
  const long Rp = sp.rows(), Rf = sf.rows();
  const int C = P.C, heads = 8, kc = C / heads;
  float* pros = prosody_out ? prosody_out : ws.get<float>(Rp * C);
  float* sty = ws.get<float>((size_t)sp.n_utt * P.table.ld());
  int* row_utt_p = ws.get<int>(Rp);
  int* row_utt_f = ws.get<int>(Rf);
  int* src_row = ws.get<int>(Rf);
  int* centre = ws.get<int>(Rf);
  float* base = ws.get<float>(Rf * C);
  float* qn = ws.get<float>(Rf * C);
  float* kn = ws.get<float>(Rp * C);
  float* q = ws.get<float>(Rf * C);
  float* kv = ws.get<float>(Rp * 2 * C);
// ... 66 lines not shown
```

### stylish_tts_amd/runtime.py

```python
from __future__ import annotations

import ctypes as C
import threading
from typing import Dict, Mapping, Optional, Sequence

import numpy as np
import torch

from . import _lib
from .config import geometry, load_model_config

N_BINS_LD = 1056


def _ptr(t: Optional[torch.Tensor]):
    return C.c_void_p(0 if t is None else t.data_ptr())


def _stream():
    return C.c_void_p(torch.cuda.current_stream().cuda_stream)


class Segments:

# ... 117 lines not shown

    def decoder(self, seg: Segments, asr, pitch, energy, style):
        dh = self.cfg.decoder.hidden_dim
        x = self._f32(seg.rows, dh)
        ws = self.workspace(seg)
        _lib.check(self.lib.stts_decoder_forward(self.ctx, _stream(), seg.n, seg.host_ptr, _ptr(seg.dev), _ptr(asr), asr.shape[1], _ptr(pitch),
                                                 _ptr(energy), _ptr(style), _ptr(x), dh, _ptr(ws), ws.numel()))
        return x

    def prior_flow(self, seg: Segments, x, style, prior_noise, return_z=False):
        dh = self.cfg.decoder.hidden_dim
        mel = self._f32(seg.rows, dh)
        zp = self._f32(seg.rows, dh // 4) if return_z else None
        zf = self._f32(seg.rows, dh // 4) if return_z else None
        ws = self.workspace(seg)
        _lib.check(self.lib.stts_prior_flow_forward(self.ctx, _stream(), seg.n, seg.host_ptr, _ptr(seg.dev), _ptr(x), x.shape[1], _ptr(style),
                                                    _ptr(prior_noise), _ptr(mel), dh, _ptr(zp), _ptr(zf), _ptr(ws), ws.numel()))
        return (mel, zp, zf) if return_z else mel

    def harmonic_stft(self, seg: Segments, pitch, src_noise, init_phase, batch_scope=True, return_signal=False):
        spec = self._f32(seg.rows, self.har_ld)
        phase = self._f32(seg.rows, self.har_ld)
        sig = self._f32(seg.rows * self.hop4) if return_signal else None
        ws = self.workspace(seg)
        _lib.check(self.lib.stts_harmonic_stft(self.ctx, _stream(), seg.n, seg.host_ptr, _ptr(seg.dev), _ptr(pitch), _ptr(src_noise),
                                               _ptr(init_phase), int(batch_scope), _ptr(sig), _ptr(spec), _ptr(phase), self.har_ld, _ptr(ws),
                                               ws.numel()))
        return (spec, phase, sig) if return_signal else (spec, phase)

    def vocoder(self, seg: Segments, mel, style, har_spec, har_phase, return_spec=False):
        audio = self._f32(seg.rows * self.hop4)
        la = self._f32(seg.rows, self.ld_lp) if return_spec else None
        ph = self._f32(seg.rows, self.ld_lp) if return_spec else None
        ws = self.workspace(seg)
        _lib.check(self.lib.stts_vocoder_forward(self.ctx, _stream(), seg.n, seg.host_ptr, _ptr(seg.dev), _ptr(mel), mel.shape[1], _ptr(style),
                                                 _ptr(har_spec), _ptr(har_phase), har_spec.shape[1], _ptr(audio), _ptr(la), _ptr(ph), self.ld_lp,
                                                 _ptr(ws), ws.numel()))
        return (audio, la, ph) if return_spec else audio

    def frame_path(self, seg: Segments, asr, pitch, energy, style, prior_noise, src_noise, init_phase, batch_scope=True, out=None):
        audio = out if out is not None else self._f32(seg.rows * self.hop4)
        ws = self.workspace(seg)
        _lib.check(self.lib.stts_frame_path(self.ctx, _stream(), seg.n, seg.host_ptr, _ptr(seg.dev), _ptr(asr), asr.shape[1], _ptr(pitch),
                                            _ptr(energy), _ptr(style), _ptr(prior_noise), _ptr(src_noise), _ptr(init_phase), int(batch_scope),
                                            _ptr(audio), _ptr(ws), ws.numel(), seg.flags))
        return audio

    def to_time_major(self, x_bct: torch.Tensor, ld: Optional[int] = None) -> torch.Tensor:
        B, Cc, T = x_bct.shape
        ld = ld or ((Cc + 31) // 32 * 32)
        y = self._f32(B * T, ld)
        _lib.check(self.lib.stts_to_time_major(_stream(), _ptr(x_bct.contiguous()), B, Cc, T, _ptr(y), ld))
        return y

    def to_channel_major(self, x: torch.Tensor, B: int, Cc: int, T: int) -> torch.Tensor:
        y = self._f32(B, Cc, T)
        _lib.check(self.lib.stts_to_channel_major(_stream(), _ptr(x), x.shape[1], B, Cc, T, _ptr(y)))
        return y

    def op_conv1d(self, seg: Segments, x, cin, w: np.ndarray, bias: Optional[np.ndarray], dil=1, act=0, force_tile=0, precision: Optional[str] = None):
        cout, _, k = w.shape
        ldy = (cout + 31) // 32 * 32
        y = torch.zeros(seg.rows, ldy, dtype=torch.float32, device=self.device)
        w = np.ascontiguousarray(w, np.float32)
        b = None if bias is None else np.ascontiguousarray(bias, np.float32)
        _lib.check(self.lib.stts_op_conv1d(_stream(), seg.n, seg.host_ptr, _ptr(seg.dev), _ptr(x), x.shape[1], cin, w.ctypes.data_as(C.c_void_p),
                                           None if b is None else b.ctypes.data_as(C.c_void_p), cout, k, dil, act, _ptr(y), ldy, force_tile,
                                           self.PRECISIONS[precision or self.precision]))
        return y

    def op_conv1d_x3(self, seg: Segments, x, cin, w: np.ndarray, bias: Optional[np.ndarray], dil=1, x2=None, cin2=0, aff: Optional[np.ndarray] = None,
                     xaff_mode=0, slope=1.0, presplit=False, force_tile=0, precision: Optional[str] = None):
        cout, _, k = w.shape
        ldy = (cout + 31) // 32 * 32
        y = torch.zeros(seg.rows, ldy, dtype=torch.float32, device=self.device)
        w = np.ascontiguousarray(w, np.float32)
        b = None if bias is None else np.ascontiguousarray(bias, np.float32)
        a = None if aff is None else np.ascontiguousarray(aff, np.float32)
        _lib.check(self.lib.stts_op_conv1d_x3(_stream(), seg.n, seg.host_ptr, _ptr(seg.dev), _ptr(x), x.shape[1], cin,
                                              None if x2 is None else _ptr(x2), 0 if x2 is None else x2.shape[1], cin2, w.ctypes.data_as(C.c_void_p),
                                              None if b is None else b.ctypes.data_as(C.c_void_p), cout, k, dil,
                                              None if a is None else a.ctypes.data_as(C.c_void_p), xaff_mode, slope, int(presplit), _ptr(y), ldy,
                                              force_tile, self.PRECISIONS[precision or self.precision]))
        return y

    def op_adain_block(self, prefix: str, seg: Segments, x, cin, cout, style):
        y = self._f32(seg.rows, cout)
        ws = self.workspace(seg)
        _lib.check(self.lib.stts_op_adain_block(self.ctx, _stream(), prefix.encode(), seg.n, seg.host_ptr, _ptr(seg.dev), _ptr(x), x.shape[1], cin,
                                                cout, _ptr(style), _ptr(y), cout, _ptr(ws), ws.numel()))
        return y

    def op_attention(self, seg_q: Segments, seg_k: Segments, q, k, v, heads: int, kc: int, band_centre=None, window: int = 0, kernel: int = 0):
        o = self._f32(seg_q.rows, heads * kc)
        _lib.check(self.lib.stts_op_attention(_stream(), seg_q.n, seg_q.host_ptr, _ptr(seg_q.dev), seg_k.host_ptr, _ptr(seg_k.dev), _ptr(q), _ptr(k), _ptr(v),
                                              _ptr(o), heads, kc, None if band_centre is None else _ptr(band_centre), window, kernel))
        return o

    def op_mrf_block(self, prefix: str, seg: Segments, x, channels, kernel, style):
        y = self._f32(seg.rows, channels)
        ws = self.workspace(seg)
        _lib.check(self.lib.stts_op_mrf_block(self.ctx, _stream(), prefix.encode(), seg.n, seg.host_ptr, _ptr(seg.dev), _ptr(x), x.shape[1], channels,
                                              kernel, _ptr(style), _ptr(y), channels, _ptr(ws), ws.numel()))
        return y

    def op_stft_geom(self, seg: Segments, sig: torch.Tensor, n_fft: int, win: int, h: int, generic: bool = True):
        ld = (n_fft // 2 + 1 + 31) // 32 * 32
        spec, phase = self._f32(seg.rows, ld), self._f32(seg.rows, ld)
        _lib.check(self.lib.stts_op_stft_geom(_stream(), seg.n, seg.host_ptr, _ptr(seg.dev), n_fft, win, h, _ptr(sig), _ptr(spec), _ptr(phase), ld,
                                              int(generic)))
        return spec, phase

    def op_istft_geom(self, seg: Segments, logamp: torch.Tensor, phase: torch.Tensor, n_fft: int, win: int, h: int, generic: bool = True):
        audio = self._f32(seg.rows * h)
        _lib.check(self.lib.stts_op_istft_geom(_stream(), seg.n, seg.host_ptr, _ptr(seg.dev), n_fft, win, h, _ptr(logamp), _ptr(phase), logamp.shape[1],
                                               _ptr(audio), int(generic)))
        return audio

    def conv_stft_transform(self, seg_frames: Segments, wave: torch.Tensor, hop: int):
        mag, x, y = (self._f32(seg_frames.rows, N_BINS_LD) for _ in range(3))
        _lib.check(self.lib.stts_conv_stft_transform(self.ctx, _stream(), seg_frames.n, seg_frames.host_ptr, _ptr(seg_frames.dev), _ptr(wave), hop,
                                                     _ptr(mag), _ptr(x), _ptr(y), N_BINS_LD))
        return mag, x, y

    def conv_stft_inverse(self, seg_frames: Segments, mag, x, y, hop: int):
        out = self._f32((seg_frames.rows - seg_frames.n) * hop)
        ws = self._f32(seg_frames.rows * 1200)
        _lib.check(self.lib.stts_conv_stft_inverse(self.ctx, _stream(), seg_frames.n, seg_frames.host_ptr, _ptr(seg_frames.dev), _ptr(mag), _ptr(x), _ptr(y),
                                                   mag.shape[1], hop, _ptr(out), _ptr(ws), ws.numel() * 4))
        return out

    def _ph_ws(self, n_tok: int, n_frames: int, n_utt: int) -> torch.Tensor:
        return self._grow(self._pws, int(self.lib.stts_phoneme_workspace_bytes(self.ctx, n_tok, n_frames, n_utt)))

    def text_encoder(self, which: int, seg: Segments, tokens: torch.Tensor, return_hidden=False):
        inter = self.cfg.pitch_energy_predictor.inter_dim if which == 2 else self.cfg.inter_dim
        mu = self._f32(seg.rows, inter)
        xh = self._f32(seg.rows, self.cfg.text_encoder.hidden_dim) if return_hidden else None
        ws = self._ph_ws(seg.rows, 0, seg.n)
        _lib.check(self.lib.stts_text_encoder_forward(self.ctx, _stream(), which, seg.n, seg.host_ptr, _ptr(seg.dev), _ptr(tokens), _ptr(mu), inter,
                                                      _ptr(xh), _ptr(ws), ws.numel()))
        return (mu, xh) if return_hidden else mu

    def text_style(self, which: int, seg: Segments, x: torch.Tensor):
        style = self._f32(seg.n, self.cfg.style_dim)
        ws = self._ph_ws(seg.rows, 0, seg.n)
        _lib.check(self.lib.stts_text_style_forward(self.ctx, _stream(), which, seg.n, seg.host_ptr, _ptr(seg.dev), _ptr(x), x.shape[1], _ptr(style),
                                                    _ptr(ws), ws.numel()))
        return style

    def duration(self, seg: Segments, tokens: torch.Tensor, taps=False):
        logits = self._f32(seg.rows, 16)
        dur = torch.empty(seg.rows, dtype=torch.int32, device=self.device)
        t = None
        if taps:
            t = dict(text_mu=self._f32(seg.rows, self.cfg.inter_dim), style=self._f32(seg.n, self.cfg.style_dim),
                     prosody=self._f32(seg.rows, self.cfg.inter_dim + self.cfg.style_dim))
        ws = self._ph_ws(seg.rows, 0, seg.n)
        _lib.check(self.lib.stts_duration_forward(self.ctx, _stream(), seg.n, seg.host_ptr, _ptr(seg.dev), _ptr(tokens), _ptr(logits), _ptr(dur),
                                                  _ptr(t["text_mu"]) if t else None, _ptr(t["style"]) if t else None,
                                                  _ptr(t["prosody"]) if t else None, _ptr(ws), ws.numel()))
        return (logits, dur, t) if taps else (logits, dur)

    def pitch_energy(self, seg_p: Segments, seg_t: Segments, dur: torch.Tensor, pe_enc: torch.Tensor, pe_style: torch.Tensor, taps=False):
        f0 = self._f32(seg_t.rows)
        en = self._f32(seg_t.rows)
# ... 271 lines not shown
```

Baseline: 2465.

## Add weights-from-registers split-fp32 GEMM tile with fragment-ordered weight packing

Adds a new split-fp32 (x3) conv GEMM variant that streams pre-packed, fragment-ordered weight planes straight from global memory into registers, skipping LDS staging for the weight operand. LDS then holds only activation tiles, and weight loads are interleaved with MFMA work in a software-pipelined loop. The planner picks the new tile by default for large x3 store-epilogue launches with enough blocks and packed weights. The cost is extra device memory for a second weight copy and higher register pressure per wave.

```diff
diff --git a/include/stylish_hip.h b/include/stylish_hip.h
--- a/include/stylish_hip.h
+++ b/include/stylish_hip.h
@@ -219,6 +219,9 @@
 int stts_op_conv1d_x3(void* stream, int n_utt, const int32_t* seg_off_host, const int32_t* seg_off_dev, const float* x, int ldx, int cin,
                       const float* x2, int ldx2, int cin2, const float* w_host, const float* bias_host, int cout, int k, int dil, const float* aff_host,
                       int xaff_mode, float slope, int presplit, float* y, int ldy, int force_tile, int precision);
+int stts_op_conv1d_wreg(void* stream, int n_utt, const int32_t* seg_off_host, const int32_t* seg_off_dev, int capacity, const float* x, int ldx,
+                        const int32_t* cins, int nseg, const float* w_host, const float* bias_host, int cout, int k, int wino, float* y, int ldy,
+                        int force_tile);
 int stts_op_adain_block(stts_ctx* ctx, void* stream, const char* prefix, int n_utt, const int32_t* seg_off_host,
                         const int32_t* seg_off_dev, const float* x, int ldx, int cin, int cout, const float* style, float* y, int ldy,
                         void* ws, size_t ws_bytes);
diff --git a/stylish_tts_amd/_lib.py b/stylish_tts_amd/_lib.py
--- a/stylish_tts_amd/_lib.py
+++ b/stylish_tts_amd/_lib.py
@@ -121,6 +121,7 @@
     "stts_bench_gemm": (_I, [_P, _I, _I, _I, _I, _I, _I, _I, C.POINTER(C.c_double), _I]),
     "stts_op_conv1d": (_I, [_P, _I, _P, _P, _P, _I, _I, _P, _P, _I, _I, _I, _I, _P, _I, _I, _I]),
     "stts_op_conv1d_x3": (_I, [_P, _I, _P, _P, _P, _I, _I, _P, _I, _I, _P, _P, _I, _I, _I, _P, _I, C.c_float, _I, _P, _I, _I, _I]),
+    "stts_op_conv1d_wreg": (_I, [_P, _I, _P, _P, _I, _P, _I, _P, _I, _P, _P, _I, _I, _I, _P, _I, _I]),
     "stts_op_adain_block": (_I, [_P, _P, C.c_char_p, _I, _P, _P, _P, _I, _I, _I, _P, _P, _I, _P, _SZ]),
     "stts_op_attention": (_I, [_P, _I, _P, _P, _P, _P, _P, _P, _P, _P, _I, _I, _P, _I, _I]),
     "stts_op_stft_geom": (_I, [_P, _I, _P, _P, _I, _I, _I, _P, _P, _P, _I, _I]),
diff --git a/stylish_tts_amd/csrc/api.hip b/stylish_tts_amd/csrc/api.hip
--- a/stylish_tts_amd/csrc/api.hip
+++ b/stylish_tts_amd/csrc/api.hip
@@ -93,6 +93,7 @@
   if (which & (STTS_W_DECODER | STTS_W_FLOW | STTS_W_GENERATOR)) {
     PackScope scope(c, {c->prec, true, c->prec != PREC_F32 ? 64 : 32, 0});
     STTS_TRY(finalize_frame(c, which));
+    if (getenv("STTS_PACK_STATS")) fprintf(stderr, "[pack] fragment-order split planes (weights-from-registers tiles): %.2f MB so far in this process\n", 1e-6 * (double)x3_wreg_bytes());
   }
   const int ph = which & (STTS_W_SPEECH_TEXT | STTS_W_DURATION | STTS_W_PE_TEXT | STTS_W_PE_STYLE | STTS_W_PITCH_ENERGY);
   if (ph) {
diff --git a/stylish_tts_amd/csrc/gemm.hip.h b/stylish_tts_amd/csrc/gemm.hip.h
--- a/stylish_tts_amd/csrc/gemm.hip.h
+++ b/stylish_tts_amd/csrc/gemm.hip.h
@@ -28,6 +28,7 @@
   const float* W;
   const unsigned short* W16;
   long w16_plane;
+  const unsigned short* WF;
   long x_plane;
   long w_utt_stride;
   int ldx, xcol0, kc, ntaps, dil, pad;
@@ -148,8 +149,9 @@
 }
 
 template <int BM, int BN, int WARPS_M, int WARPS_N, int EPI, int KSPLIT = 1, bool GLDS = false, int PREC = PREC_F32, int XAFF = 0, bool MSEG = true,
-          bool X16 = false>
+          bool X16 = false, bool WREG = false>
 __global__ void __launch_bounds__(WARPS_M* WARPS_N * 64 * KSPLIT) conv_gemm_f32(const GemmArgs a) {
+  static_assert(!WREG || (PREC == PREC_X3 && !X16 && !GLDS && KSPLIT == 1 && BM / WARPS_M == 32 && EPI == EPI_STORE), "weights from registers: split fp32, register staging, 32 output channels per wave");
   static_assert(!(XAFF && GLDS), "the input affine lives on the register staging path");
   static_assert(!X16 || (PREC != PREC_F32 && !XAFF && EPI == EPI_STORE), "16-bit activation rows: 16-bit operand modes, store epilogue");
   constexpr int NT = WARPS_M * WARPS_N * 64 * KSPLIT;
@@ -162,15 +164,16 @@
   constexpr int WR = BN / WARPS_N, WC = BM / WARPS_M;
   constexpr int TR = WR / 32, TC = WC / 32;
   constexpr int XL = X16 ? (BN * 4 * NPL + NT - 1) / NT : BN * 8 / NT;
-  constexpr int WL = B16 ? (BM * 4 * NPL + NT - 1) / NT : BM * 8 / NT;
+  constexpr int WL = WREG ? 0 : B16 ? (BM * 4 * NPL + NT - 1) / NT : BM * 8 / NT;
+  constexpr int WLA = WL > 0 ? WL : 1;
   static_assert(WR % 32 == 0 && WC % 32 == 0, "wave tile must be a multiple of 32x32");
   static_assert((X16 || (BN * 8) % NT == 0) && (B16 || (BM * 8) % NT == 0), "tile loads must divide over the block");
   static_assert(EPI == EPI_STORE || EPI == EPI_SPLIT_ACC || TC % 2 == 0, "paired epilogues need an even TC");
   constexpr int NSTAGE = (B16 && GLDS) ? (X3 ? 3 : ((BM + BN) <= 256 ? 8 : 3)) : 2;
   constexpr int SLOTS = X3 ? 12 : ((B16 && KSPLIT == 1) ? 4 : 8);
-  constexpr int PLANE = (BN + BM) * 4;
+  constexpr int PLANE = (BN + (WREG ? 0 : BM)) * 4;
   constexpr int STG16 = PLANE * NPL;
-  __shared__ f32x4 lds[NSTAGE * (BN + BM) * SLOTS];
+  __shared__ f32x4 lds[WREG ? 4 * STG16 : NSTAGE * (BN + BM) * SLOTS];
 
   int bx = blockIdx.x, by = blockIdx.y, bz = blockIdx.z;
   {
@@ -277,7 +280,7 @@
   const int nseg = a.nseg;
 
   struct RegSet {
-    f32x4 x[XL], w[WL];
+    f32x4 x[XL], w[WLA];
     bool ok[XL];
     f32x4 sc, sh;
     bool aff;
@@ -289,7 +292,7 @@
   constexpr bool DEEP = false;
 #endif
   RegSet rsC, rsD;
-  unsigned woff[WL];
+  unsigned woff[WLA];
   const int len = hi - lo, rel0 = row0 - lo;
   long g_wplane = X3 ? a.seg[0].w16_plane : 0, g_xplane = (X3 && X16) ? a.seg[0].x_plane : 0;
   auto seg_offsets = [&]() {
@@ -543,6 +546,9 @@
 #pragma unroll
       for (int j = 0; j < TC; ++j) acc[i][j] = mfma16<PREC>(xa[i], wb[j], acc[i][j]);
   };
+
+  float bias_early = 0.0f;
+  if constexpr (WREG) bias_early = a.bias ? a.bias[m0 + wm * WC + l31] : 0.0f;
 
   if constexpr (GLDS) {
     static_assert(KSPLIT == 1, "GLDS path is single K-group");
@@ -678,6 +684,128 @@
         __syncthreads();
       }
     }
+  } else if constexpr (WREG) {
+    static_assert(TC == 1, "one 32-channel block of output channels per wave");
+    struct XFrag {
+      f32x4 xa[TR][3];
+    };
+    struct WSet {
+      f32x4 w[3];
+    };
+    XFrag xA, xB;
+    WSet w0, w1, w2, w3;
+    const int wmu = __builtin_amdgcn_readfirstlane(wm);
+    auto wf_base = [&](const GemmSeg& g) {
+      return reinterpret_cast<const char*>(g.WF + 3 * (long)utt * g.w_utt_stride) + (long)((m0 >> 5) + wmu) * g.ntaps * g.kc * (96 * 2);
+    };
+    const char* wfp = wf_base(a.seg[0]);
+    int wf_left = a.seg[0].ntaps * (a.seg[0].kc / 32) - 1;
+    int wf_s = 0;
+    auto wf_next = [&]() {
+      const char* p = wfp;
+      const bool endseg = wf_left == 0;
+      bool moved = false;
+      if constexpr (MSEG) {
+        if (endseg && wf_s + 1 < nseg) {
+          ++wf_s;
+          const GemmSeg& n = wf_s == 1 ? a.seg[1] : a.seg[2];
+          wfp = wf_base(n);
+          wf_left = n.ntaps * (n.kc / 32) - 1;
+          moved = true;
+        }
+      }
+      if (!moved) {
+        wfp += endseg ? 0 : 6 * 1024;
+        wf_left -= endseg ? 0 : 1;
+      }
+      return p;
+    };
+    auto wload = [&](const char* p, int kk, WSet& w) {
+#pragma unroll
+      for (int pl = 0; pl < 3; ++pl) w.w[pl] = *reinterpret_cast<const f32x4*>(p + ((kk * 3 + pl) * 64 + lane) * 16);
+    };
+    auto xread = [&](int sub, int kk, XFrag& f) {
+      const f32x4* Xs = lds + sub * STG16;
+      const int slot = 2 * kk + lh;
+#pragma unroll
+      for (int i = 0; i < TR; ++i) {
+        const int r = wn * WR + i * 32 + l31;
+        const int o = r * 4 + (slot ^ ((r >> 2) & 3));
+#pragma unroll
+        for (int p = 0; p < 3; ++p) f.xa[i][p] = Xs[o + p * PLANE];
+      }
+    };
+    auto xw_mma = [&](const XFrag& f, const WSet& w) {
+#pragma unroll
+      for (int i = 0; i < TR; ++i) {
+        acc[i][0] = mfma16<PREC>(f.xa[i][2], w.w[0], acc[i][0]);
+        acc[i][0] = mfma16<PREC>(f.xa[i][0], w.w[2], acc[i][0]);
+        acc[i][0] = mfma16<PREC>(f.xa[i][1], w.w[1], acc[i][0]);
+        acc[i][0] = mfma16<PREC>(f.xa[i][1], w.w[0], acc[i][0]);
+        acc[i][0] = mfma16<PREC>(f.xa[i][0], w.w[1], acc[i][0]);
+        acc[i][0] = mfma16<PREC>(f.xa[i][0], w.w[0], acc[i][0]);
+      }
+    };
+    gload(rsA);
+    gload(rsB);
+    {
+      const char* p = wf_next();
+      wload(p, 0, w0);
+      wload(p, 1, w1);
+      p = wf_next();
+      wload(p, 0, w2);
+      wload(p, 1, w3);
+    }
+    lstore(rsA, 0);
+    gload(rsA);
+    lstore(rsB, 1);
+    gload(rsB);
+    __syncthreads();
+    stamp(1);
+    xread(0, 0, xA);
+    auto pair = [&](int b) {
+      const int s0 = 2 * b, s1 = s0 + 1, n0 = 2 * (b ^ 1), n1 = n0 + 1;
+      xread(s0, 1, xB);
+      xw_mma(xA, w0);
+      const char* p = wf_next();
+      wload(p, 0, w0);
+      lstore(rsA, n0);
+      gload(rsA);
+      xread(s1, 0, xA);
+      xw_mma(xB, w1);
+      wload(p, 1, w1);
+      xread(s1, 1, xB);
+      xw_mma(xA, w2);
+      p = wf_next();
+      wload(p, 0, w2);
+      lstore(rsB, n1);
+      gload(rsB);
+#ifndef STTS_X3_NO_SGB
+      constexpr int NM = 18 * TR * TC, NV = (2 * (25 + 30 * XL) + NM - 1) / NM;
+#pragma unroll
+      for (int g = 0; g < NM; ++g) {
+        __builtin_amdgcn_sched_group_barrier(0x008, 1, 0);
+        __builtin_amdgcn_sched_group_barrier(0x002, NV, 0);
+      }
+#endif
+      __syncthreads();
+      xread(n0, 0, xA);
+      xw_mma(xB, w3);
+      wload(p, 1, w3);
+    };
+    const int npair = total >> 1;
+    int P = 0;
+    for (; P + 1 < npair; P += 2) {
+      pair(0);
+      pair(1);
+    }
+    if (P < npair) { pair(0); ++P; }
+    if (total & 1) {
+      xread(2 * (P & 1), 1, xB);
+      xw_mma(xA, w0);
+      xw_mma(xB, w1);
+    }
+    stamp(2);
   } else {
   gload(rsA);
   lstore(rsA, 0);
@@ -873,7 +1001,8 @@
 #pragma unroll
     for (int j = 0; j < TC; ++j) {
       const int n = m0 + clane + j * 32;
-      bv[j] = a.bias ? a.bias[n] : 0.0f;
+      if constexpr (WREG) bv[j] = bias_early;
+      else bv[j] = a.bias ? a.bias[n] : 0.0f;
       nok[j] = n < a.N;
     }
 #pragma unroll
@@ -1160,13 +1289,24 @@
   }
 }
 
-template <int BM, int BN, int WM, int WN, int KS = 1, int X16MODE = 0>
+template <int BM, int BN, int WM, int WN, int KS = 1, int X16MODE = 0, bool WR = false>
 inline void launch_cfg_x3(hipStream_t st, const GemmArgs& a, int epi, int npad, int n_utt, int max_rows, hipEvent_t e0 = nullptr, hipEvent_t e1 = nullptr) {
   dim3 grid(npad / BM, ceil_div(max_rows, BN), n_utt * (a.ksplit > 1 ? a.ksplit : 1)), block(WM * WN * 64 * KS);
   if (a.compact) grid = dim3(npad / BM, a.tiles_y, a.ksplit > 1 ? a.ksplit : 1);
   if constexpr (X16MODE != 0) {
     if (a.nseg == 1) STTS_LAUNCH_TIMED((conv_gemm_f32<BM, BN, WM, WN, EPI_STORE, KS, X16MODE == 2, PREC_X3, false, false, true>), grid, block, st, e0, e1, a);
     else STTS_LAUNCH_TIMED((conv_gemm_f32<BM, BN, WM, WN, EPI_STORE, KS, X16MODE == 2, PREC_X3, false, true, true>), grid, block, st, e0, e1, a);
+    return;
+  } else if constexpr (WR) {
+    if (a.xaff) {
+      if (a.nseg == 1 && a.xaff_scale_only) STTS_LAUNCH_TIMED((conv_gemm_f32<BM, BN, WM, WN, EPI_STORE, KS, false, PREC_X3, 2, false, false, true>), grid, block, st, e0, e1, a);
+      else if (a.nseg == 1) STTS_LAUNCH_TIMED((conv_gemm_f32<BM, BN, WM, WN, EPI_STORE, KS, false, PREC_X3, 1, false, false, true>), grid, block, st, e0, e1, a);
+      else STTS_LAUNCH_TIMED((conv_gemm_f32<BM, BN, WM, WN, EPI_STORE, KS, false, PREC_X3, 1, true, false, true>), grid, block, st, e0, e1, a);
+    } else if (a.nseg == 1) {
+      STTS_LAUNCH_TIMED((conv_gemm_f32<BM, BN, WM, WN, EPI_STORE, KS, false, PREC_X3, 0, false, false, true>), grid, block, st, e0, e1, a);
+    } else {
+      STTS_LAUNCH_TIMED((conv_gemm_f32<BM, BN, WM, WN, EPI_STORE, KS, false, PREC_X3, 0, true, false, true>), grid, block, st, e0, e1, a);
+    }
     return;
   } else
   if (epi == EPI_PRIOR) {
@@ -1190,7 +1330,7 @@
 inline void launch_tile_x3(hipStream_t st, const GemmArgs& as, int epi, int npad, int n_utt, int max_rows, hipEvent_t e0, hipEvent_t e1) {
   constexpr TileRow r = tile_row(T);
   static_assert((r.forms & FORM_X3) != 0, "not a split-fp32 tile");
-  launch_cfg_x3<r.BM, r.BN, r.WM, r.WN, r.KS, r.x16 != X16_MUST ? 0 : r.glds ? 2 : 1>(st, as, epi, npad, n_utt, max_rows, e0, e1);
+  launch_cfg_x3<r.BM, r.BN, r.WM, r.WN, r.KS, r.x16 != X16_MUST ? 0 : r.glds ? 2 : 1, r.wreg>(st, as, epi, npad, n_utt, max_rows, e0, e1);
 }
 #define STTS_TILE_CASE(T) case T: launch_tile<T, PR>(st, as, epi, npad, n_utt, max_rows, e0, e1); break;
 template <int PR>
@@ -1209,6 +1349,7 @@
     STTS_TILE_CASE(2) STTS_TILE_CASE(4) STTS_TILE_CASE(5) STTS_TILE_CASE(6) STTS_TILE_CASE(8)
     STTS_TILE_CASE(20) STTS_TILE_CASE(21) STTS_TILE_CASE(22)
     STTS_TILE_CASE(25) STTS_TILE_CASE(26) STTS_TILE_CASE(27) STTS_TILE_CASE(28)
+    STTS_TILE_CASE(30)
     default: launch_tile_x3<3>(st, as, epi, npad, n_utt, max_rows, e0, e1); break;
   }
 }
diff --git a/stylish_tts_amd/csrc/gemm_plan.hip.h b/stylish_tts_amd/csrc/gemm_plan.hip.h
--- a/stylish_tts_amd/csrc/gemm_plan.hip.h
+++ b/stylish_tts_amd/csrc/gemm_plan.hip.h
@@ -15,6 +15,7 @@
   bool paired;
   bool xaff;
   bool splitk;
+  bool wreg;
 };
 constexpr unsigned kAllForms = FORM_F32 | FORM_16 | FORM_X3;
 constexpr TileRow kTiles[] = {
@@ -38,6 +39,7 @@
     {26, 128, 64, 4, 2, 1, false, FORM_X3, X16_MUST, true, false, false, false},
     {27, 128, 128, 4, 2, 1, true, FORM_X3, X16_MUST, true, false, false, false},
     {28, 128, 64, 4, 2, 1, true, FORM_X3, X16_MUST, true, false, false, false},
+    {30, 128, 128, 4, 2, 1, false, FORM_X3, X16_NEVER, true, false, true, false, true},
 };
 constexpr const TileRow* find_tile(int id) {
   for (const TileRow& r : kTiles)
@@ -54,6 +56,7 @@
   static constexpr int kUnset = INT_MIN;
   bool no_x3;
   bool x3_rem;
+  bool x3_wreg;
   int x3_tile;
   bool x3p_glds;
   int tile16;
@@ -66,6 +69,7 @@
     GemmSwitches s;
     s.no_x3 = num("STTS_NO_X3", 0) != 0;
     s.x3_rem = num("STTS_X3_REM", 0) != 0;
+    s.x3_wreg = num("STTS_X3_WREG", 1) != 0;
     s.x3_tile = num("STTS_X3_TILE", GemmSwitches::kUnset);
     s.x3p_glds = num("STTS_X3P_GLDS", 1) != 0;
     s.tile16 = num("STTS_TILE16", GemmSwitches::kUnset);
@@ -118,6 +122,7 @@
 inline bool gemm16_will_run(const GemmArgs& a, int epi, int npad, int n_utt) { return gemm16_route(a, epi, npad, n_utt, 0, gemm_switches()); }
 
 constexpr int kCUs = 256;
+constexpr int kX3ShortK = 24;
 inline long gemm_row_tiles(const GemmArgs& a, int n_utt, int max_rows, int bn) {
   if (!a.seg_host) return (long)n_utt * ceil_div(max_rows, bn);
   long t = 0;
@@ -150,12 +155,17 @@
   p.cost *= bn * penalty;
   return p;
 }
+inline bool wreg_packed(const GemmArgs& a) {
+  for (int i = 0; i < a.nseg; ++i)
+    if (!a.seg[i].WF) return false;
+  return true;
+}
 inline bool tile_fits(GemmPlan& p, int tile, const GemmArgs& a, int epi, int npad, unsigned form) {
   const TileRow* r = find_tile(tile);
   const bool paired = epi != EPI_STORE && epi != EPI_SPLIT_ACC;
   if (!r) snprintf(p.err, sizeof(p.err), "conv_gemm: no tile %d", tile);
   else if (!(r->forms & form) || (a.x16 ? r->x16 == X16_NEVER || a.xaff : r->x16 == X16_MUST) || (a.xaff && !r->xaff) || (epi != EPI_STORE && r->store_only) ||
-           (paired && !r->paired) || npad % r->BM != 0)
+           (paired && !r->paired) || npad % r->BM != 0 || (r->wreg && !wreg_packed(a)))
     snprintf(p.err, sizeof(p.err), "conv_gemm: tile %d does not take this launch (operand form %u, 16-bit rows / pre-split planes %d, input affine %d, epilogue %d, cout padded to %d): see kTiles", tile, form,
               a.x16, a.xaff != nullptr, epi, npad);
   return p.ok();
@@ -201,7 +211,7 @@
       const RowPlan p5 = plan_rows(gemm_row_tiles(a, n_utt, max_rows, 128), mt, iters, may_split_rem, 128, 1.0);
       const RowPlan p6 = plan_rows(gemm_row_tiles(a, n_utt, max_rows, 64), mt, iters, may_split_rem, 64, 1.03);
       tile = p5.cost <= p6.cost ? 5 : 6;
-      if (x3 && iters <= 24 && !a.xaff) tile = 6;
+      if (x3 && iters <= kX3ShortK && !a.xaff) tile = 6;
       rows = tile == 5 ? p5 : p6;
       if (tile == 5 && blocks128 <= kCUs && a.prec == PREC_F32 && !x3) tile = 8;
     }
@@ -229,6 +239,7 @@
     tile = 22;
     rows = RowPlan();
   }
+  if (x3_large && tile == 5 && sw.x3_wreg && sw.x3_tile == GemmSwitches::kUnset && !sw.x3_rem && epi == EPI_STORE && blocks128 >= 128 && wreg_packed(a)) tile = 30;
   if (x3 && a.x16) {
     if (find_tile(tile)->x16 != X16_MUST) tile = presplit_tile(find_tile(tile)->BN, sw.x3p_glds);
     rows = RowPlan();
diff --git a/stylish_tts_amd/csrc/model.hip.h b/stylish_tts_amd/csrc/model.hip.h
--- a/stylish_tts_amd/csrc/model.hip.h
+++ b/stylish_tts_amd/csrc/model.hip.h
@@ -24,6 +24,7 @@
 #include "wn_fused_x3.hip.h"
 #include "wn_block_x3.hip.h"
 #include "winograd.hip.h"
+#include "x3_wreg_pack.h"
 
 namespace stts {
 
@@ -37,6 +38,7 @@
   float* W = nullptr;
   unsigned short* W16 = nullptr;
   long w16_plane = 0;
+  unsigned short* WF = nullptr;
   int prec = 0;
   float* bias = nullptr;
   int npad = 0, N = 0, kc = 0, ntaps = 1;
@@ -137,6 +139,7 @@
   bool x3;
   int kc_align;
   int tag;
+  bool wreg_all = false;
 };
 
 }
@@ -307,6 +310,10 @@
   return r;
 }
 
+inline size_t& x3_wreg_bytes() {
+  static size_t n = 0;
+  return n;
+}
 inline int pack_rows(stts_ctx* c, const HostTensor& w, const HostTensor* bias, const std::vector<int>& row_of, int cin_lo, int cin_n,
                      int kc, int N, PackedConv* out, float scale = 1.0f) {
   STTS_CHECK(c->pack.prec >= 0, "pack_rows outside a PackScope");
@@ -325,6 +332,7 @@
   STTS_TRY(dev_upload(c, pb, &out->bias));
   out->prec = prec;
   out->W16 = nullptr;
+  out->WF = nullptr;
   out->w16_plane = 0;
   if (prec != PREC_F32 || packs_x3(c)) {
     const bool split = prec == PREC_F32;
@@ -335,6 +343,11 @@
     } else
     for (size_t i = 0; i < pw.size(); ++i) h[i] = prec == PREC_BF16 ? f32_to_bf16(pw[i]) : f32_to_f16(pw[i]);
     STTS_TRY(dev_upload(c, h, &out->W16));
+    if (split && gemm_switches().x3_wreg && npad % 128 == 0 && kc % 32 == 0 && (c->pack.wreg_all || k * (kc / 32) > kX3ShortK)) {
+      const std::vector<unsigned short> hf = pack_x3_wreg(h.data(), pw.size(), npad, k, kc);
+      STTS_TRY(dev_upload(c, hf, &out->WF));
+      x3_wreg_bytes() += hf.size() * sizeof(unsigned short);
+    }
   }
   out->npad = npad;
   out->N = N;
@@ -832,6 +845,7 @@
   g.W = w.W;
   g.W16 = w.W16;
   g.w16_plane = w.w16_plane;
+  g.WF = w.WF;
   if (i == 0) a.prec = w.prec;
   g.w_utt_stride = 0;
   g.ldx = ldx;
@@ -856,7 +870,7 @@
 }
 template <int N>
 inline int run_winograd_n(hipStream_t st, const Seg& s, const float* X, int ldx, const WinoConv& wc, float* Y, int ldy, int act, const float* R, int ldr,
-                          float alpha, WinoScratch& scratch, const float* aff = nullptr, int ld_aff = 0, float* stat = nullptr, int ld_stat = 0) {
+                          float alpha, WinoScratch& scratch, const float* aff = nullptr, int ld_aff = 0, float* stat = nullptr, int ld_stat = 0, int force_tile = 0) {
   const int n = wc.mats.n, kc = wc.planes.kc, ldm = round_up(wc.planes.N, 32), ml = s.max_len();
   long pr = 0;
   for (int u = 0; u < s.n_utt; ++u) pr += ceil_div(s.host[u + 1] - s.host[u], kWinoM);
@@ -902,7 +916,7 @@
   }
   a.N = wc.planes.N; a.bias = nullptr; a.Y = Mp; a.ldy = ldm;
   {
-    const int rc = launch_conv_gemm(st, a, EPI_STORE, wc.planes.npad, n, (int)pr);
+    const int rc = launch_conv_gemm(st, a, EPI_STORE, wc.planes.npad, n, (int)pr, force_tile);
     if (rc) {
       prof.on = timed;
       return rc;
@@ -925,12 +939,12 @@
 }
 inline int wino_stat_chunks(const Seg& s) { return ceil_div(ceil_div(s.max_len(), kWinoM), 4); }
 inline int run_winograd(hipStream_t st, const Seg& s, const float* X, int ldx, const WinoConv& wc, float* Y, int ldy, int act, const float* R, int ldr,
-                        float alpha, WinoScratch& scratch, const float* aff = nullptr, int ld_aff = 0, float* stat = nullptr, int ld_stat = 0) {
+                        float alpha, WinoScratch& scratch, const float* aff = nullptr, int ld_aff = 0, float* stat = nullptr, int ld_stat = 0, int force_tile = 0) {
   STTS_CHECK(wc.ready && (wc.mats.n == 8 || wc.mats.n == 12), "winograd conv not packed");
   STTS_CHECK(ldx % 4 == 0 && ldy % 4 == 0 && (!R || ldr % 4 == 0), "winograd conv: leading dimensions must be multiples of 4");
   STTS_CHECK(!stat || (ld_stat % 4 == 0 && ld_stat >= round_up(wc.planes.N, 4)), "winograd conv: statistics rows of %d floats do not cover %d channels", ld_stat, wc.planes.N);
-  return wc.mats.n == 8 ? run_winograd_n<8>(st, s, X, ldx, wc, Y, ldy, act, R, ldr, alpha, scratch, aff, ld_aff, stat, ld_stat)
-                        : run_winograd_n<12>(st, s, X, ldx, wc, Y, ldy, act, R, ldr, alpha, scratch, aff, ld_aff, stat, ld_stat);
+  return wc.mats.n == 8 ? run_winograd_n<8>(st, s, X, ldx, wc, Y, ldy, act, R, ldr, alpha, scratch, aff, ld_aff, stat, ld_stat, force_tile)
+                        : run_winograd_n<12>(st, s, X, ldx, wc, Y, ldy, act, R, ldr, alpha, scratch, aff, ld_aff, stat, ld_stat, force_tile);
 }
 
 inline int run_style(hipStream_t st, const StyleTable& t, const float* style, int n_utt, float* out) {
@@ -1361,6 +1375,7 @@
     b.seg[0].W = w2u;
     b.seg[0].W16 = reinterpret_cast<const unsigned short*>(w2u);
     b.seg[0].w16_plane = 0;
+    b.seg[0].WF = nullptr;
     b.seg[0].w_utt_stride = (long)B.pw2.npad * B.pw2.kc;
   }
   b.x16 = p16 != 0;
diff --git a/stylish_tts_amd/csrc/phoneme_model.hip.h b/stylish_tts_amd/csrc/phoneme_model.hip.h
--- a/stylish_tts_amd/csrc/phoneme_model.hip.h
+++ b/stylish_tts_amd/csrc/phoneme_model.hip.h
@@ -384,6 +384,7 @@
     b.seg[0].W = w2u;
     b.seg[0].W16 = reinterpret_cast<const unsigned short*>(w2u);
     b.seg[0].w16_plane = 0;
+    b.seg[0].WF = nullptr;
     b.seg[0].w_utt_stride = (long)B.pw2.npad * B.pw2.kc;
     b.N = sd; b.bias = B.pw2.bias; b.Y = h2; b.ldy = sd; b.R = h; b.ldr = sd;
     STTS_TRY(launch_conv_gemm(st, b, EPI_STORE, B.pw2.npad, s.n_utt, ml));
diff --git a/stylish_tts_amd/csrc/x3_wreg_pack.h b/stylish_tts_amd/csrc/x3_wreg_pack.h
--- /dev/null
+++ b/stylish_tts_amd/csrc/x3_wreg_pack.h
@@ -0,0 +1,21 @@
+#pragma once
+#include <cstddef>
+#include <vector>
+
+namespace stts {
+
+inline size_t x3_wreg_index(int row, int tap, int ch, int pl, int ntaps, int kc) {
+  const int blk = row >> 5, lane = (row & 31) + 32 * ((ch >> 3) & 1), chunk = ch >> 5, step = (ch >> 4) & 1;
+  return ((((((size_t)blk * (kc / 32) + chunk) * ntaps + tap) * 2 + step) * 3 + pl) * 64 + lane) * 8 + (ch & 7);
+}
+
+inline std::vector<unsigned short> pack_x3_wreg(const unsigned short* w16, size_t plane, int rows, int ntaps, int kc) {
+  std::vector<unsigned short> out((size_t)3 * rows * ntaps * kc);
+  for (int pl = 0; pl < 3; ++pl)
+    for (int row = 0; row < rows; ++row)
+      for (int tap = 0; tap < ntaps; ++tap)
+        for (int ch = 0; ch < kc; ++ch) out[x3_wreg_index(row, tap, ch, pl, ntaps, kc)] = w16[pl * plane + ((size_t)row * ntaps + tap) * kc + ch];
+  return out;
+}
+
+}
diff --git a/stylish_tts_amd/runtime.py b/stylish_tts_amd/runtime.py
--- a/stylish_tts_amd/runtime.py
+++ b/stylish_tts_amd/runtime.py
@@ -223,6 +223,18 @@
                                               None if b is None else b.ctypes.data_as(C.c_void_p), cout, k, dil,
                                               None if a is None else a.ctypes.data_as(C.c_void_p), xaff_mode, slope, int(presplit), _ptr(y), ldy,
                                               force_tile, self.PRECISIONS[precision or self.precision]))
+        return y
+
+    def op_conv1d_wreg(self, seg: Segments, x, cins: Sequence[int], w: np.ndarray, bias: Optional[np.ndarray], wino=False, force_tile=0):
+        cout, _, k = w.shape
+        ldy = (cout + 31) // 32 * 32
+        y = torch.zeros(seg.rows, ldy, dtype=torch.float32, device=self.device)
+        w = np.ascontiguousarray(w, np.float32)
+        b = None if bias is None else np.ascontiguousarray(bias, np.float32)
+        ci = np.ascontiguousarray(cins, np.int32)
+        _lib.check(self.lib.stts_op_conv1d_wreg(_stream(), seg.n, seg.host_ptr, _ptr(seg.dev), int(seg.is_capacity), _ptr(x), x.shape[1],
+                                                ci.ctypes.data_as(C.c_void_p), len(ci), w.ctypes.data_as(C.c_void_p),
+                                                None if b is None else b.ctypes.data_as(C.c_void_p), cout, k, int(wino), _ptr(y), ldy, force_tile))
         return y
 
     def op_adain_block(self, prefix: str, seg: Segments, x, cin, cout, style):
```

Result: no change. 2456 (-0.4%).
